# zhouyifan233/light-transport

Measured on AMD Instinct MI355X. Metric: photon_steps_per_sec, higher is better.
Workload: dtype f64

## Files before the change

include/lt.h:

```cpp
#ifndef LT_H_
#define LT_H_

#include <stddef.h>
#include <stdint.h>

#ifdef __cplusplus
extern "C" {
#endif

#define LT_ABI_VERSION 3

#define LT_OK 0
#define LT_E_INVALID (-1)
#define LT_E_STATE (-2)
#define LT_E_HIP (-3)
#define LT_E_NOMEM (-4)
#define LT_E_UNSUPPORTED (-5)

#define LT_TALLY_F32 0
#define LT_TALLY_F64 1
#define LT_TALLY_U64FX 2
#define LT_FX_SCALE 1099511627776.0

#define LT_QUANTITY_ABSORBED 0
#define LT_QUANTITY_FLUENCE 1

#define LT_SRC_PENCIL 0
#define LT_SRC_COSINE_QUAD 1

#define LT_FLAG_F32_WALK 1u

typedef struct lt_medium {
    double mu_a;
    double mu_s;
    double g;
    double n;
} lt_medium;

typedef struct lt_bvh_node {
    double lo[3];
    double hi[3];
    int32_t offset;
    int32_t n_prims;
    int32_t axis;
    int32_t pad_;
} lt_bvh_node;

typedef struct lt_counters {
    uint64_t photons;
    uint64_t steps;
    double w_absorbed;
    double w_lost_outside_grid;
    double w_escaped_top;
    double w_escaped_bottom;
    double w_escaped_mesh;
    double w_specular;
    double w_roulette_net;
    double w_capped;
} lt_counters;

typedef struct lt_ctx lt_ctx;

int lt_abi_version(void);
int lt_create(lt_ctx** out, int device_id);
int lt_destroy(lt_ctx* ctx);
const char* lt_last_error(const lt_ctx* ctx);

int lt_set_media(lt_ctx* ctx, const lt_medium* media, int n);
int lt_set_layers(lt_ctx* ctx, const double* z_bounds, const int32_t* medium_idx,
                  int n, double n_above, double n_below);
int lt_set_mesh(lt_ctx* ctx, const double* verts, const int32_t* med_front,
                const int32_t* med_back, int n_tris, const lt_bvh_node* nodes,
                int n_nodes);
int lt_build_bvh(const double* verts, int n_tris, int split_method, int32_t* order_out, lt_bvh_node* nodes_out,
                 int max_nodes, int* n_nodes_out);
int lt_set_grid(lt_ctx* ctx, int nx, int ny, int nz, const double origin[3],
                const double voxel[3], int tally_dtype);
int lt_set_source(lt_ctx* ctx, int type, const double pos[3], const double dir[3],
                  const double* extra, int start_medium);
int lt_set_max_steps(lt_ctx* ctx, uint32_t max_steps);
int lt_set_tuning(lt_ctx* ctx, const char* key, int64_t value);
int lt_set_tally_quantity(lt_ctx* ctx, int quantity);
int lt_set_launch_config(lt_ctx* ctx, int blocks_per_cu, int threads_per_block);

#define LT_MODE_ATOMIC 0
#define LT_MODE_LOG 1
#define LT_MODE_AUTO 2
int lt_set_tally_mode(lt_ctx* ctx, int mode, uint64_t log_bytes);
int lt_reserve_log(lt_ctx* ctx, uint64_t n_photons);
int lt_set_overlap(lt_ctx* ctx, int lanes);

int lt_launch(lt_ctx* ctx, uint64_t n_photons, uint64_t photon_offset, uint64_t seed,
              const double* rng_table, uint64_t table_steps, uint32_t flags);
int lt_sync(lt_ctx* ctx);
int lt_last_kernel_ms(lt_ctx* ctx, double* ms);
int lt_zero_tally(lt_ctx* ctx);
int lt_last_log_stages(lt_ctx* ctx, double ms_out[4], uint64_t* records, uint64_t* batches);
int lt_last_log_info(lt_ctx* ctx, uint64_t* records, uint64_t* overflow_records, uint64_t* batches, int* lanes);
int lt_last_log_hot_tiles(lt_ctx* ctx, uint32_t* hot_tiles, uint32_t* threshold);

int lt_read_grid(lt_ctx* ctx, void* host_out, size_t bytes);
int lt_read_grid_f64(lt_ctx* ctx, double* host_out, size_t n_voxels);
int lt_read_counters(lt_ctx* ctx, lt_counters* out);
int lt_grid_device_ptr(lt_ctx* ctx, void** ptr, size_t* bytes);
int lt_counters_device_ptr(lt_ctx* ctx, void** ptr, size_t* bytes);
void* lt_stream(lt_ctx* ctx);
int lt_reduce_grid(lt_ctx* ctx, void* nccl_comm, int root);


int lt_intersect_rays(lt_ctx* ctx, const double* origins, const double* dirs,
                      const double* tmax, size_t n, int use_bvh, int32_t* prim_out,
                      double* t_out);
int lt_triangle_intersect(lt_ctx* ctx, const double* origins, const double* dirs,
                          const double* tris, size_t n, double* t_out);
int lt_intersect_bounds(lt_ctx* ctx, const double* origins, const double* dirs,
                        const double* tmax, const double* boxes, size_t n,
                        int32_t* hit_out);
#define LT_FN_HG_PDF 0
#define LT_FN_HG_SAMPLE 1
#define LT_FN_ONB 2
#define LT_FN_DISK 3
#define LT_FN_COSINE_HEMI 4
#define LT_FN_REFLECT 5
#define LT_FN_BOUNDARY 6
#define LT_FN_SPIN 7
#define LT_FN_WALK_MATH 8
#define LT_FN_WALK_MATH_RAW 9
int lt_eval(lt_ctx* ctx, int fn, const double* in, size_t n, double* out);
int lt_rng_raw(lt_ctx* ctx, uint64_t seed, uint64_t photon_id, uint32_t count,
               uint32_t* out);

typedef struct lt_surface_material {
    double diffuse[3];
    double emission;
    double ior;
    double transmission;
    int32_t is_diffuse, is_mirror, is_light, pad_;
} lt_surface_material;

typedef struct lt_point_light {
    double source[3];
    double normal[3];
    double radiance[3];
    double total_area;
} lt_point_light;

int lt_set_surface_materials(lt_ctx* ctx, const lt_surface_material* mats, int n_tris);
int lt_set_lights(lt_ctx* ctx, const lt_point_light* lights, int n);
int lt_render_surface(lt_ctx* ctx, int width, int height, int samples, int max_depth,
                      const double camera[3], double f_distance, const double* xs,
                      const double* ys, double* rand_0, const double* rand_1,
                      const int32_t* light_choice, double* image);
int lt_render_surface_old(lt_ctx* ctx, int width, int height, int samples, int max_depth,
                          const double camera[3], double f_distance, const double* xs,
                          const double* ys, double* rand_0, const double* rand_1,
                          const int32_t* light_choice, int choices_per_sample, double* image);

#define LT_VERTEX_LIGHT 5
#define LT_VERTEX_REFLECTIVE 3
#define LT_VERTEX_TRANSMISSIVE 4
#define LT_VERTEX_VOLUME 7
typedef struct lt_vertex {
    double point[3];
    double direction[3];
    double g_norm[3];
    double throughput;
    double pdf_pos;
    double pdf_dir;
    int32_t kind;
    int32_t medium;
    uint32_t step;
    uint32_t pad_;
} lt_vertex;
int lt_set_vertex_capture(lt_ctx* ctx, uint32_t max_vertices_per_photon);
int lt_read_vertices(lt_ctx* ctx, lt_vertex* vertices_out, uint32_t* counts_out, uint64_t n_photons);

int lt_mesh_accel_info(lt_ctx* ctx, int* kind, int march_dims[3], uint64_t* march_entries, int clearance_dims[3]);

int lt_device_info(lt_ctx* ctx, char* name, size_t name_len, int* n_cus,
                   int* clock_mhz, size_t* hbm_bytes);

#ifdef __cplusplus
}
#endif
#endif
```

light_transport_amd/_lib.py:

```python
import ctypes as C
import os
import subprocess

import numpy as np

_HERE = os.path.dirname(os.path.abspath(__file__))
LIB_PATH = os.environ.get("LT_HIP_LIBRARY") or os.path.join(_HERE, "liblt_hip.so")

TALLY = {"f32": 0, "f64": 1, "u64fx": 2}
TALLY_NP = {0: np.float32, 1: np.float64, 2: np.uint64}
FX_SCALE = 2.0 ** 40
SRC_PENCIL, SRC_COSINE_QUAD = 0, 1
FLAG_F32_WALK = 1
FN = dict(HG_PDF=0, HG_SAMPLE=1, ONB=2, DISK=3, COSINE_HEMI=4, REFLECT=5, BOUNDARY=6, SPIN=7, WALK_MATH=8, WALK_MATH_RAW=9)
_FN_SHAPE = {0: (2, 1), 1: (2, 1), 2: (3, 6), 3: (2, 2), 4: (8, 4), 5: (6, 3), 6: (8, 5), 7: (5, 3), 8: (1, 5), 9: (1, 3)}

SYMBOLS = [
    "lt_abi_version", "lt_create", "lt_destroy", "lt_last_error", "lt_set_media", "lt_set_layers", "lt_set_mesh",
    "lt_set_grid", "lt_set_source", "lt_set_max_steps", "lt_set_launch_config", "lt_launch", "lt_sync",
    "lt_last_kernel_ms", "lt_zero_tally", "lt_read_grid", "lt_read_grid_f64", "lt_read_counters",
    "lt_grid_device_ptr", "lt_counters_device_ptr", "lt_stream", "lt_reduce_grid", "lt_intersect_rays",
    "lt_triangle_intersect", "lt_intersect_bounds", "lt_eval", "lt_rng_raw", "lt_device_info",
    "lt_set_surface_materials", "lt_set_lights", "lt_render_surface", "lt_set_vertex_capture", "lt_read_vertices",
    "lt_set_tally_mode", "lt_last_log_stages", "lt_reserve_log", "lt_render_surface_old", "lt_set_overlap", "lt_last_log_hot_tiles",
    "lt_last_log_info", "lt_set_tally_quantity", "lt_set_tuning", "lt_mesh_accel_info", "lt_build_bvh",
]

VERTEX_DTYPE = np.dtype([("point", "<f8", 3), ("direction", "<f8", 3), ("g_norm", "<f8", 3), ("throughput", "<f8"),
                         ("pdf_pos", "<f8"), ("pdf_dir", "<f8"), ("kind", "<i4"), ("medium", "<i4"), ("step", "<u4"),
                         ("pad_", "<u4")])
VERTEX_LIGHT, VERTEX_REFLECTIVE, VERTEX_TRANSMISSIVE, VERTEX_VOLUME = 5, 3, 4, 7


class LtError(RuntimeError):
    pass


NODE_DTYPE = np.dtype([("lo", "<f8", 3), ("hi", "<f8", 3), ("offset", "<i4"), ("n_prims", "<i4"), ("axis", "<i4"), ("pad_", "<i4")])


def build_bvh_arrays(verts, split_method=1):
    v = _f64(verts).reshape(-1, 3, 3)
    T = v.shape[0]
    order = np.empty(T, dtype=np.int32)
    nodes = np.zeros(max(2 * T, 1), dtype=NODE_DTYPE)
    nn = C.c_int(0)
    rc = lib().lt_build_bvh(_dp(v), C.c_int(T), C.c_int(int(split_method)), _ip(order), nodes.ctypes.data_as(C.c_void_p),
                            C.c_int(len(nodes)), C.byref(nn))
    if rc:
        raise LtError("lt_build_bvh failed (%d): needs >= 1 triangle with finite vertices and split_method 0 or 1" % rc)
    return order, nodes[:nn.value]


class Medium(C.Structure):
    _fields_ = [("mu_a", C.c_double), ("mu_s", C.c_double), ("g", C.c_double), ("n", C.c_double)]


class BvhNode(C.Structure):
    _fields_ = [("lo", C.c_double * 3), ("hi", C.c_double * 3), ("offset", C.c_int32),
                ("n_prims", C.c_int32), ("axis", C.c_int32), ("pad_", C.c_int32)]


class Counters(C.Structure):
    _fields_ = [("photons", C.c_uint64), ("steps", C.c_uint64)] + [
        (k, C.c_double) for k in ("w_absorbed", "w_lost_outside_grid", "w_escaped_top", "w_escaped_bottom",
                                  "w_escaped_mesh", "w_specular", "w_roulette_net", "w_capped")]

    def as_dict(self):
        return {k: getattr(self, k) for k, _ in self._fields_}


class SurfaceMaterial(C.Structure):
    _fields_ = [("diffuse", C.c_double * 3), ("emission", C.c_double), ("ior", C.c_double),
                ("transmission", C.c_double), ("is_diffuse", C.c_int32), ("is_mirror", C.c_int32),
                ("is_light", C.c_int32), ("pad_", C.c_int32)]


class PointLight(C.Structure):
    _fields_ = [("source", C.c_double * 3), ("normal", C.c_double * 3), ("radiance", C.c_double * 3),
                ("total_area", C.c_double)]


def pack_surface_materials(primitives):
    arr = (SurfaceMaterial * max(len(primitives), 1))()
    for i, p in enumerate(primitives):
        m = p.material
        arr[i].diffuse[:] = [float(x) for x in m.color.diffuse[:3]]
        arr[i].emission, arr[i].ior, arr[i].transmission = float(m.emission), float(m.ior), float(m.transmission)
        arr[i].is_diffuse, arr[i].is_mirror, arr[i].is_light = int(m.is_diffuse), int(m.is_mirror), int(p.is_light)
    return arr


def pack_lights(lights):
    arr = (PointLight * max(len(lights), 1))()
    for i, l in enumerate(lights):
        arr[i].source[:] = [float(x) for x in l.source[:3]]
        arr[i].normal[:] = [float(x) for x in l.normal[:3]]
        arr[i].radiance[:] = [float(l.material.emission * x) for x in l.material.color.diffuse[:3]]
        arr[i].total_area = float(l.total_area)
    return arr


_lib = None


def build(verbose=False):
    cmd = ["make", "-C", os.path.join(_HERE, "csrc")]
    if not verbose:
        cmd.append("-s")
    subprocess.check_call(cmd)
    return LIB_PATH


def lib():
    global _lib
    if _lib is None:
        if not os.path.exists(LIB_PATH):
            raise LtError("liblt_hip.so is not built (run light_transport_amd.build() or "
                          "`make -C light_transport_amd/csrc`); there is no CPU fallback")
        L = C.CDLL(LIB_PATH)
        L.lt_last_error.restype = C.c_char_p
        L.lt_last_error.argtypes = [C.c_void_p]
        L.lt_stream.restype = C.c_void_p
        L.lt_stream.argtypes = [C.c_void_p]
        _lib = L
    return _lib


def _dp(a):
    return a.ctypes.data_as(C.POINTER(C.c_double)) if a is not None else None


def _ip(a):
    return a.ctypes.data_as(C.POINTER(C.c_int32)) if a is not None else None


def _f64(a, shape=None):
    a = np.ascontiguousarray(a, dtype=np.float64)
    return a.reshape(shape) if shape is not None else a


class Context:

    def __init__(self, device_id=0):
        self._h = C.c_void_p()
        rc = lib().lt_create(C.byref(self._h), C.c_int(device_id))
        if rc != 0:
            msg = lib().lt_last_error(None)
            raise LtError("lt_create failed (%d): %s" % (rc, msg.decode() if msg else "?"))
        self.device_id = device_id
        self._grid_shape = None
        self._tally = None

    def _ck(self, rc, what):
        if rc != 0:
            msg = lib().lt_last_error(self._h)
            raise LtError("%s failed (%d): %s" % (what, rc, msg.decode() if msg else "?"))

    def close(self):
        if getattr(self, "_h", None) is not None and self._h.value:
            lib().lt_destroy(self._h)
            self._h = C.c_void_p()

    def __del__(self):
        try:
            self.close()
        except Exception:
            pass

    def __enter__(self):
        return self

    def __exit__(self, *a):
        self.close()

    def set_media(self, media):
        arr = (Medium * len(media))(*[Medium(*map(float, m)) for m in media])
        self._ck(lib().lt_set_media(self._h, arr, C.c_int(len(media))), "lt_set_media")

    def set_layers(self, z_bounds, medium_idx, n_above=1.0, n_below=1.0):
        zb = _f64(z_bounds)
        mi = np.ascontiguousarray(medium_idx, dtype=np.int32)
        if zb.size != mi.size + 1:
            raise LtError("set_layers: need len(z_bounds) == len(medium_idx) + 1")
        self._ck(lib().lt_set_layers(self._h, _dp(zb), _ip(mi), C.c_int(mi.size), C.c_double(n_above),
                                     C.c_double(n_below)), "lt_set_layers")

    def set_mesh(self, verts, med_front, med_back, nodes):
        v = _f64(verts).reshape(-1, 3, 3)
        mf = np.ascontiguousarray(med_front, dtype=np.int32)
        mb = np.ascontiguousarray(med_back, dtype=np.int32)
        if isinstance(nodes, np.ndarray) and nodes.dtype == NODE_DTYPE:
            arr = np.ascontiguousarray(nodes)
        else:
            n_ = len(nodes["offset"])
            arr = np.zeros(n_, dtype=NODE_DTYPE)
            arr["lo"] = np.asarray(nodes["lo"], dtype=np.float64).reshape(n_, 3); arr["hi"] = np.asarray(nodes["hi"], dtype=np.float64).reshape(n_, 3)
            arr["offset"] = nodes["offset"]; arr["n_prims"] = nodes["n_prims"]; arr["axis"] = nodes["axis"]
        n = len(arr)
        if mf.size != v.shape[0] or mb.size != v.shape[0]:
            raise LtError("set_mesh: medium arrays must have one entry per triangle")
        self._ck(lib().lt_set_mesh(self._h, _dp(v), _ip(mf), _ip(mb), C.c_int(v.shape[0]), arr.ctypes.data_as(C.c_void_p), C.c_int(n)),
                 "lt_set_mesh")

# ... 231 lines not shown
```

light_transport_amd/csrc/lt_api.cpp:

```cpp
#include <hip/hip_runtime_api.h>

#include <dlfcn.h>

#include <algorithm>
#include <cmath>
#include <cctype>
#include <cstdarg>
#include <cstdio>
#include <cstdlib>
#include <cstring>
#include <limits>
#include <mutex>
#include <new>
#include <string>
#include <vector>

#include "lt_internal.hpp"

using namespace ltk;

static const size_t kMeshLdsBudget = 64 * 1024;

namespace {

thread_local std::string g_create_error;

struct DevBuf {
    void* p = nullptr;
    size_t bytes = 0;
    void release() { if (p) { (void)hipFree(p); p = nullptr; bytes = 0; } }
    hipError_t ensure(size_t n)
    {
        if (n <= bytes && p) return hipSuccess;
        release();
        hipError_t e = hipMalloc(&p, n ? n : 16);
        if (e == hipSuccess) bytes = n ? n : 16;
        return e;
    }
};

}

constexpr int kMaxLanes = 3;
constexpr int kAutoLanes = 2;

struct LogLane {
    hipStream_t stream = nullptr;
    hipStream_t tail_stream = nullptr;
    hipEvent_t ev_bulk = nullptr, ev_tail = nullptr;
    hipEvent_t ev_done = nullptr;
    std::vector<hipEvent_t> evs;
    size_t ev_used = 0;
    DevBuf log_idx, log_val, tmp_idx, tmp_val, log_fill, meta, hist1, hist_unused, hist, bin_base, bin_cnt, tile_base, tile_cnt, cursor1,
        cursor2, items2, items_c, items_r, itab, head, pool, pool_n;
    size_t alloc_records = 0;
    int alloc_elem = 0;
    void release_log() { log_idx.release(); log_val.release(); tmp_idx.release(); tmp_val.release(); log_fill.release(); alloc_records = 0; }
    void release_all()
    {
        release_log(); meta.release(); hist1.release(); hist_unused.release(); hist.release(); bin_base.release(); bin_cnt.release(); tile_base.release();
        tile_cnt.release(); cursor1.release(); itab.release();
        cursor2.release(); items2.release(); items_c.release(); items_r.release(); head.release(); pool.release(); pool_n.release();
    }
};

struct lt_ctx {
    int device = 0;
    hipStream_t stream = nullptr;
    hipEvent_t ev0 = nullptr, ev1 = nullptr, ev_fork = nullptr;
    bool stages_valid = false;
    uint64_t last_records = 0, last_overflow = 0, last_batches = 0;
    int last_lanes = 1;
    bool log_stats_pending = false;
    uint64_t pending_photons = 0;
    std::string err;
    hipDeviceProp_t prop;

    std::vector<lt_medium> media;
    std::vector<double> z_bounds;
    std::vector<int32_t> layer_medium;
    double n_above = 1.0, n_below = 1.0;
    std::vector<double> verts;
    std::vector<int32_t> med_front, med_back;
    std::vector<lt_bvh_node> nodes;
    std::vector<lt_surface_material> surf_mats;
    std::vector<lt_point_light> lights;
    bool have_layers = false, have_mesh = false, have_grid = false, have_source = false;
    int nx = 0, ny = 0, nz = 0, tally = LT_TALLY_F32;
    double origin[3] = {0, 0, 0}, voxel[3] = {1, 1, 1};
    int src_type = LT_SRC_PENCIL, start_medium = 0;
    double src_pos[3] = {0, 0, 0}, src_dir[3] = {0, 0, 1}, src_extra[6] = {0, 0, 0, 0, 0, 0};
    uint32_t max_steps = 1000000;
    int quantity = LT_QUANTITY_ABSORBED;
    uint32_t max_vertices = 0, captured_max_vertices = 0;
    int tally_mode = 2;
    size_t log_budget = (size_t)16 << 30, default_log_budget = (size_t)16 << 30;
    double rec_per_photon = 0.0;
    int overlap_mode = 0;
    double auto_ms_per_photon[kMaxLanes] = {0.0, 0.0, 0.0};
    uint64_t auto_photons[kMaxLanes] = {0, 0, 0};
    int auto_pending = -1;
    uint64_t captured_photons = 0;
    int blocks_per_cu = 0, threads_per_block = 0;

    DevBuf d_media[2], d_zb[2], d_if[2], d_lm, d_tris[2], d_nodes[2];
    DevBuf d_grid, d_counters, d_head, d_table, d_scratch_in, d_scratch_out, d_scratch_aux;
    DevBuf d_mats, d_lights, d_r0, d_r1, d_lc, d_img, d_xy, d_vtx, d_vcnt, d_clear, d_job, d_gridx[kMaxLanes - 1];
    int cn[3] = {0, 0, 0};
    double corg[3] = {0, 0, 0}, ccell[3] = {1, 1, 1};
    bool have_clear = false;
    DevBuf d_mcell, d_mlist, d_mcoarse, d_links;
    MarchGrid mgrid;
    bool have_march = false, have_links = false;
    size_t march_entries = 0;
    LogLane lanes[kMaxLanes];
    DevBuf d_dmap, d_dmeta;
    bool dmap_valid = false, tile_cnt_ready = false, last_hot = false;
    uint32_t dmap_tiles = 0, dmap_bits2 = 0;
    bool tables_dirty = true, media_dirty = false;
    struct Knobs {
        long query_min = -1, log_bits2 = -1, log_hot = -1, overlap_walk_bpc = -1, diag_no_tally = -1, log_timing = -1,
             march_cells = -1, march_scale_milli = -1, no_march = -1, no_clearance = -1, no_near_lists = -1,
             clearance_cells = -1, march_info = -1, force_march = -1, tail_split = -1, part_alone = -1, serial_walks = -1, part_lds = -1,
             render_lds_tables = -1;
        std::string overlap_pattern;
    } knob;
    long* knob_by_name(const char* key)
    {
        static const struct { const char* k; long Knobs::*m; } tab[] = {
            {"query_min", &Knobs::query_min}, {"log_bits2", &Knobs::log_bits2}, {"log_hot", &Knobs::log_hot},
            {"overlap_walk_bpc", &Knobs::overlap_walk_bpc}, {"diag_no_tally", &Knobs::diag_no_tally}, {"log_timing", &Knobs::log_timing},
            {"march_cells", &Knobs::march_cells}, {"march_scale_milli", &Knobs::march_scale_milli}, {"no_march", &Knobs::no_march},
            {"no_clearance", &Knobs::no_clearance}, {"no_near_lists", &Knobs::no_near_lists}, {"clearance_cells", &Knobs::clearance_cells},
            {"march_info", &Knobs::march_info}, {"force_march", &Knobs::force_march}, {"tail_split", &Knobs::tail_split}, {"part_alone", &Knobs::part_alone}, {"serial_walks", &Knobs::serial_walks}, {"part_lds", &Knobs::part_lds},
            {"render_lds_tables", &Knobs::render_lds_tables}};
        for (const auto& t : tab) if (std::strcmp(key, t.k) == 0) return &(knob.*(t.m));
        return nullptr;
    }
    bool on(long v) const { return v > 0; }
    bool timed = false;

    int fail(int code, const char* fmt, ...)
    {
        char buf[512];
        va_list ap;
        va_start(ap, fmt);
        vsnprintf(buf, sizeof buf, fmt, ap);
        va_end(ap);
        err = buf;
        return code;
    }
    int hip(hipError_t e, const char* what)
    {
        if (e == hipSuccess) return LT_OK;
        return fail(LT_E_HIP, "%s: %s", what, hipGetErrorString(e));
    }
    size_t grid_elem() const { return tally == LT_TALLY_F32 ? 4 : 8; }
    size_t n_vox() const { return (size_t)nx * (size_t)ny * (size_t)nz; }
    void scene_changed() { rec_per_photon = 0.0; for (double& a : auto_ms_per_photon) a = 0.0; for (uint64_t& a : auto_photons) a = 0; auto_pending = -1; dmap_valid = tile_cnt_ready = false; }
};

static bool bvh_octant_links(const std::vector<lt_bvh_node>& nd, std::vector<int16_t>& out)
{
    const int n = (int)nd.size();
    if (n <= 0 || n > 32767) return false;
    out.assign((size_t)16 * n, (int16_t)n);
    for (int oct = 0; oct < 8; oct++) {
        int16_t* first = &out[(size_t)oct * 2 * n]; int16_t* after = first + n;
        std::vector<std::pair<int, int>> todo{{0, n}};
        while (!todo.empty()) {
            const auto [i, a] = todo.back(); todo.pop_back();
            after[i] = (int16_t)a;
            if (nd[(size_t)i].n_prims > 0) continue;
            const int c0 = i + 1, c1 = nd[(size_t)i].offset;
            const bool neg = (oct >> nd[(size_t)i].axis) & 1;
            const int near_ = neg ? c1 : c0, far_ = neg ? c0 : c1;
            first[i] = (int16_t)near_;
            todo.emplace_back(near_, far_); todo.emplace_back(far_, a);
        }
    }
    return true;
}

#define CHECK_CTX(c) do { if (!(c)) return LT_E_INVALID; } while (0)
#define HIP_TRY(c, call) do { hipError_t e_ = (call); if (e_ != hipSuccess) return (c)->hip(e_, #call); } while (0)
#define BIND(c) HIP_TRY(c, hipSetDevice((c)->device))

namespace {

template <typename R>
void fill_media(const std::vector<lt_medium>& in, int quantity, std::vector<MedD<R>>& out)
{
    out.resize(in.size());
    for (size_t i = 0; i < in.size(); i++) {
        const double mu_t = in[i].mu_a + in[i].mu_s;
        MedD<R>& m = out[i];
        m.mu_t = (R)mu_t;
        m.inv_mu_t = (R)(mu_t > 0 ? 1.0 / mu_t : 0.0);
        m.absorb = (R)(mu_t > 0 ? in[i].mu_a / mu_t : 0.0);
        m.g = (R)in[i].g;
        m.n = (R)in[i].n;
        const R g = m.g;
        m.one_m_g2 = (R)1 - g * g;
        m.one_p_g2 = (R)1 + g * g;
        m.inv_2g = g != 0 ? (R)1 / ((R)2 * g) : (R)0;
        m.dep = quantity == LT_QUANTITY_FLUENCE ? m.inv_mu_t : m.absorb;
        m.one_m_g = (R)1 - g; m.two_g = (R)2 * g;
        m.pad_ = 0;
    }
}

template <typename R>
void fill_tris(const std::vector<double>& v, const std::vector<int32_t>& mf, const std::vector<int32_t>& mb,
               std::vector<TriD<R>>& out)
{
    const size_t n = v.size() / 9;
    out.resize(n);
    for (size_t i = 0; i < n; i++) {
        const double* a = &v[9 * i];
        const double* b = a + 3;
        const double* c = a + 6;
        double e1[3], e2[3], nn[3];
        for (int k = 0; k < 3; k++) { e1[k] = b[k] - a[k]; e2[k] = c[k] - a[k]; }
        nn[0] = e1[1] * e2[2] - e1[2] * e2[1];
        nn[1] = e1[2] * e2[0] - e1[0] * e2[2];
        nn[2] = e1[0] * e2[1] - e1[1] * e2[0];
        const double l = std::sqrt(nn[0] * nn[0] + nn[1] * nn[1] + nn[2] * nn[2]);
        for (int k = 0; k < 3; k++) {
            out[i].a[k] = (R)a[k]; out[i].ab[k] = (R)e1[k]; out[i].ac[k] = (R)e2[k]; out[i].n[k] = (R)(nn[k] / l);
        }
        out[i].med_front = mf[i];
        out[i].med_back = mb[i];
    }
}

template <typename R>
void fill_nodes(const std::vector<lt_bvh_node>& in, std::vector<NodeD<R>>& out)
{
    out.resize(in.size());
    for (size_t i = 0; i < in.size(); i++) {
        for (int k = 0; k < 3; k++) {
            R lo = (R)in[i].lo[k], hi = (R)in[i].hi[k];
            if ((double)lo > in[i].lo[k]) lo = std::nextafter(lo, -std::numeric_limits<R>::infinity());
            if ((double)hi < in[i].hi[k]) hi = std::nextafter(hi, std::numeric_limits<R>::infinity());
            out[i].lo[k] = lo; out[i].hi[k] = hi;
        }
        out[i].offset = in[i].offset;
        out[i].n_prims = in[i].n_prims;
        out[i].axis = in[i].axis;
        out[i].skip = (int32_t)in.size();
    }
    for (size_t i = 0; i < in.size(); i++) {
        if (in[i].n_prims > 0) continue;
        out[i + 1].skip = in[i].offset;
        out[(size_t)in[i].offset].skip = out[i].skip;
    }
}

template <typename R>
void fill_ifaces(const lt_ctx* c, std::vector<IfD<R>>& out)
{
    const int n = (int)c->layer_medium.size();
    out.resize((size_t)n + 1);
    for (int k = 0; k <= n; k++) {
        auto index_of = [&](int layer) {
            const int32_t m = c->layer_medium[(size_t)layer];
            return m >= 0 && (size_t)m < c->media.size() ? c->media[(size_t)m].n : 1.0;
        };
        const R up = (R)(k == 0 ? c->n_above : index_of(k - 1));
        const R dn = (R)(k == n ? c->n_below : index_of(k));
        out[(size_t)k].n_up = up; out[(size_t)k].n_dn = dn;
        out[(size_t)k].nr_down = up / dn; out[(size_t)k].nr_up = dn / up;
    }
}

template <typename T>
int upload(lt_ctx* c, DevBuf& b, const std::vector<T>& h)
{
    HIP_TRY(c, b.ensure(h.size() * sizeof(T)));
    if (!h.empty()) HIP_TRY(c, hipMemcpyAsync(b.p, h.data(), h.size() * sizeof(T), hipMemcpyHostToDevice, c->stream));
    return LT_OK;
}

bool tri_box_overlap(const double bc[3], const double bh[3], const double* tri)
{
    double v[3][3];
    for (int i = 0; i < 3; i++) for (int k = 0; k < 3; k++) v[i][k] = tri[3 * i + k] - bc[k];
    for (int k = 0; k < 3; k++) {
        const double lo = std::min(v[0][k], std::min(v[1][k], v[2][k])), hi = std::max(v[0][k], std::max(v[1][k], v[2][k]));
        if (lo > bh[k] || hi < -bh[k]) return false;
    }
    const double e[3][3] = {{v[1][0] - v[0][0], v[1][1] - v[0][1], v[1][2] - v[0][2]},
                            {v[2][0] - v[1][0], v[2][1] - v[1][1], v[2][2] - v[1][2]},
                            {v[0][0] - v[2][0], v[0][1] - v[2][1], v[0][2] - v[2][2]}};
    for (int j = 0; j < 3; j++)
        for (int i = 0; i < 3; i++) {
            const int a = (i + 1) % 3, b = (i + 2) % 3;
            const double ax = -e[j][b], bx = e[j][a];
            const double p0 = ax * v[0][a] + bx * v[0][b], p1 = ax * v[1][a] + bx * v[1][b], p2 = ax * v[2][a] + bx * v[2][b];
            const double r = bh[a] * std::fabs(ax) + bh[b] * std::fabs(bx);
            if (std::min(p0, std::min(p1, p2)) > r || std::max(p0, std::max(p1, p2)) < -r) return false;
        }
    const double n[3] = {e[0][1] * e[1][2] - e[0][2] * e[1][1], e[0][2] * e[1][0] - e[0][0] * e[1][2], e[0][0] * e[1][1] - e[0][1] * e[1][0]};
    const double dn = n[0] * v[0][0] + n[1] * v[0][1] + n[2] * v[0][2];
    const double r = bh[0] * std::fabs(n[0]) + bh[1] * std::fabs(n[1]) + bh[2] * std::fabs(n[2]);
    return !(dn > r || dn < -r);
}

int build_march_grid(lt_ctx* c)
{
    c->have_march = false;
    const size_t nt = c->verts.size() / 9;
    double ext[3], longest = 0;
    for (int k = 0; k < 3; k++) { ext[k] = c->nodes[0].hi[k] - c->nodes[0].lo[k]; if (ext[k] > longest) longest = ext[k]; }
    if (!(longest > 0) || !std::isfinite(longest) || nt == 0) return LT_OK;
    std::vector<double> size(nt);
    for (size_t i = 0; i < nt; i++) {
        const double* a = &c->verts[9 * i];
        const double e1[3] = {a[3] - a[0], a[4] - a[1], a[5] - a[2]}, e2[3] = {a[6] - a[0], a[7] - a[1], a[8] - a[2]};
        const double nn[3] = {e1[1] * e2[2] - e1[2] * e2[1], e1[2] * e2[0] - e1[0] * e2[2], e1[0] * e2[1] - e1[1] * e2[0]};
        size[i] = std::sqrt(std::sqrt(nn[0] * nn[0] + nn[1] * nn[1] + nn[2] * nn[2]));
    }
    std::nth_element(size.begin(), size.begin() + nt / 2, size.end());
    double h = size[nt / 2];
    if (c->knob.march_scale_milli > 10 && c->knob.march_scale_milli < 100000) h *= 1e-3 * (double)c->knob.march_scale_milli;
    int per_axis = h > 0 ? (int)std::lround(longest / h) : 256;
    per_axis = per_axis < 32 ? 32 : (per_axis > 256 ? 256 : per_axis);
    if (c->knob.march_cells >= 4 && c->knob.march_cells <= 512) per_axis = (int)c->knob.march_cells;
    h = longest / (double)per_axis;
    MarchGrid& G = c->mgrid;
    int n[3];
    for (int k = 0; k < 3; k++) {
        n[k] = (int)std::ceil(ext[k] / h); if (n[k] < 1) n[k] = 1;
        G.h[k] = ext[k] > 0 ? ext[k] / n[k] : h;
        n[k] += 2;
        G.org[k] = c->nodes[0].lo[k] - G.h[k]; G.inv[k] = 1.0 / G.h[k];
    }
    G.nx = n[0]; G.ny = n[1]; G.nz = n[2];
    for (int k = 0; k < 3; k++) {
        G.fn[k] = (double)n[k]; G.fn32[k] = (float)n[k];
        G.org32[k] = (float)G.org[k]; G.inv32[k] = (float)G.inv[k]; G.h32[k] = (float)G.h[k];
    }
    const size_t cells = (size_t)n[0] * n[1] * n[2];
    const double hmin = std::min(G.h[0], std::min(G.h[1], G.h[2]));
    const double margin = std::max(1e-4 * hmin, 3e-5 * longest);
    G.nudge64 = 1e-9 * hmin; G.nudge32 = 4e-6 * longest;
    std::vector<uint32_t> count(cells, 0u);
    std::vector<std::pair<uint32_t, uint32_t>> pairs;
    pairs.reserve(nt * 8);
    for (size_t i = 0; i < nt; i++) {
        const double* a = &c->verts[9 * i];
        int lo[3], hi[3];
        for (int k = 0; k < 3; k++) {
            const double mn = std::min(a[k], std::min(a[3 + k], a[6 + k])) - margin, mx = std::max(a[k], std::max(a[3 + k], a[6 + k])) + margin;
            lo[k] = (int)std::floor((mn - G.org[k]) * G.inv[k]); hi[k] = (int)std::floor((mx - G.org[k]) * G.inv[k]);
            lo[k] = lo[k] < 0 ? 0 : lo[k]; hi[k] = hi[k] >= n[k] ? n[k] - 1 : hi[k];
        }
        const double bh[3] = {0.5 * G.h[0] + margin, 0.5 * G.h[1] + margin, 0.5 * G.h[2] + margin};
        for (int z = lo[2]; z <= hi[2]; z++)
            for (int y = lo[1]; y <= hi[1]; y++)
                for (int x = lo[0]; x <= hi[0]; x++) {
                    const double bc[3] = {G.org[0] + (x + 0.5) * G.h[0], G.org[1] + (y + 0.5) * G.h[1], G.org[2] + (z + 0.5) * G.h[2]};
                    if (!tri_box_overlap(bc, bh, a)) continue;
                    const uint32_t ci = (uint32_t)(((size_t)z * n[1] + y) * n[0] + x);
                    count[ci]++;
                    pairs.emplace_back(ci, (uint32_t)i);
                }
    }
    std::vector<uint2> rec(cells);
    size_t total = 0;
    for (size_t i = 0; i < cells; i++) {
        rec[i].x = count[i] < kMarchCountMask ? count[i] : kMarchCountMask;
        rec[i].y = (uint32_t)total;
        total += count[i];
    }
    if (total >= (1u << 26)) return LT_OK;
    std::vector<uint32_t> list(total ? total : 1, 0u), fill(cells, 0u);
    for (const auto& pr : pairs) list[rec[pr.first].y + fill[pr.first]++] = pr.second;
    c->march_entries = pairs.size();
    HIP_TRY(c, c->d_mcell.ensure(cells * sizeof(uint2)));
    HIP_TRY(c, c->d_mlist.ensure(list.size() * 4));
    const size_t nc = (size_t)((n[0] + 7) / 8) * ((n[1] + 7) / 8) * ((n[2] + 7) / 8);
    HIP_TRY(c, c->d_mcoarse.ensure(nc * sizeof(double)));
    HIP_TRY(c, hipMemcpyAsync(c->d_mcell.p, rec.data(), cells * sizeof(uint2), hipMemcpyHostToDevice, c->stream));
    HIP_TRY(c, hipMemcpyAsync(c->d_mlist.p, list.data(), list.size() * 4, hipMemcpyHostToDevice, c->stream));
    G.cell = (const uint2*)c->d_mcell.p; G.list = (const uint32_t*)c->d_mlist.p;
    HIP_TRY(c, launch_march_clearance(c->d_tris[0].p, c->d_nodes[0].p, (int)c->nodes.size(), G, (uint2*)c->d_mcell.p,
                                      (double*)c->d_mcoarse.p, c->stream));
    HIP_TRY(c, hipStreamSynchronize(c->stream));
    c->have_march = true;
    if (c->on(c->knob.march_info))
        std::fprintf(stderr, "[lt march] %zu triangles, grid %d x %d x %d (cell %.4g), %zu list entries (%.2f per triangle), %zu cells listed\n",
                     nt, n[0], n[1], n[2], h, pairs.size(), (double)pairs.size() / (double)nt,
                     (size_t)std::count_if(count.begin(), count.end(), [](uint32_t v) { return v != 0; }));
    return LT_OK;
}

int upload_tables(lt_ctx* c)
{
    if (!c->tables_dirty && !c->media_dirty) return LT_OK;
    int rc;
    std::vector<MedD<double>> m64; std::vector<MedD<float>> m32;
    std::vector<double> z64; std::vector<float> z32;
    std::vector<IfD<double>> i64; std::vector<IfD<float>> i32;
    std::vector<TriD<double>> t64; std::vector<TriD<float>> t32;
    std::vector<NodeD<double>> n64; std::vector<NodeD<float>> n32;
    std::vector<int16_t> links16;
    fill_media(c->media, c->quantity, m64); fill_media(c->media, c->quantity, m32);
    if ((rc = upload(c, c->d_media[0], m64))) return rc;
    if ((rc = upload(c, c->d_media[1], m32))) return rc;
    if (c->have_layers) {
        fill_ifaces(c, i64); fill_ifaces(c, i32);
        if ((rc = upload(c, c->d_if[0], i64))) return rc;
        if ((rc = upload(c, c->d_if[1], i32))) return rc;
    }
    if (!c->tables_dirty) {
        HIP_TRY(c, hipStreamSynchronize(c->stream));
        c->media_dirty = false;
        return LT_OK;
    }
    if (c->have_layers) {
        z64 = c->z_bounds;
        z32.assign(z64.begin(), z64.end());
        if ((rc = upload(c, c->d_zb[0], z64))) return rc;
        if ((rc = upload(c, c->d_zb[1], z32))) return rc;
        if ((rc = upload(c, c->d_lm, c->layer_medium))) return rc;
    }
    if (c->have_mesh) {
        fill_tris(c->verts, c->med_front, c->med_back, t64);
        fill_tris(c->verts, c->med_front, c->med_back, t32);
        fill_nodes(c->nodes, n64); fill_nodes(c->nodes, n32);
        if ((rc = upload(c, c->d_tris[0], t64))) return rc;
        if ((rc = upload(c, c->d_tris[1], t32))) return rc;
        if ((rc = upload(c, c->d_nodes[0], n64))) return rc;
        if ((rc = upload(c, c->d_nodes[1], n32))) return rc;
        c->have_links = bvh_octant_links(c->nodes, links16);
        if (c->have_links && (rc = upload(c, c->d_links, links16))) return rc;
        Variant vq; std::memset(&vq, 0, sizeof vq); vq.mesh = 1;
        const int nm = (int)c->media.size(), ntr = (int)t64.size(), nno = (int)n64.size();
        const bool lds64 = walk_lds_bytes(vq, nm, 0, ntr, nno) <= kMeshLdsBudget;
        vq.f32 = 1;
        const bool lds32 = walk_lds_bytes(vq, nm, 0, ntr, nno) <= kMeshLdsBudget;
        c->have_march = false;
        if ((!lds64 || c->on(c->knob.force_march)) && !c->on(c->knob.no_clearance) && !c->on(c->knob.no_march)) { if ((rc = build_march_grid(c))) return rc; }
        c->have_clear = false;
        if (!c->on(c->knob.no_clearance) && lds32) {
            if (t64.size() > 0xffff) return c->fail(LT_E_UNSUPPORTED, "lt_set_mesh: %zu triangles within the LDS budget cannot be (near-triangle ids are 16 bits)", t64.size());
            double ext[3], longest = 0;
            for (int k = 0; k < 3; k++) { ext[k] = c->nodes[0].hi[k] - c->nodes[0].lo[k]; if (ext[k] > longest) longest = ext[k]; }
            if (longest > 0 && std::isfinite(longest)) {
                int per_axis = (int)std::cbrt(2.0e9 / (double)(t64.empty() ? 1 : t64.size()));
                per_axis = per_axis < 32 ? 32 : (per_axis > 128 ? 128 : per_axis);
                if (c->knob.clearance_cells >= 8 && c->knob.clearance_cells <= 512) per_axis = (int)c->knob.clearance_cells;
                const double h = longest / (double)per_axis;
                for (int k = 0; k < 3; k++) {
                    c->cn[k] = (int)std::ceil(ext[k] / h); if (c->cn[k] < 1) c->cn[k] = 1;
                    c->ccell[k] = ext[k] > 0 ? ext[k] / c->cn[k] : h; c->corg[k] = c->nodes[0].lo[k];
                }
                const size_t cells = (size_t)c->cn[0] * c->cn[1] * c->cn[2];
                HIP_TRY(c, c->d_clear.ensure(cells * 16));
                HIP_TRY(c, launch_build_clearance(c->d_tris[0].p, (int)t64.size(), c->on(c->knob.no_near_lists) ? 0 : 1, c->d_clear.p,
                                                  c->cn[0], c->cn[1], c->cn[2], c->corg, c->ccell, c->stream));
                c->have_clear = true;
            }
        }
    }
    HIP_TRY(c, hipStreamSynchronize(c->stream));
    c->tables_dirty = false; c->media_dirty = false;
    return LT_OK;
}

int collect_log_stats(lt_ctx* c)
{
    if (!c->log_stats_pending) return LT_OK;
    unsigned long long h[2] = {0, 0};
    HIP_TRY(c, hipMemcpyAsync(h, c->d_job.p, sizeof h, hipMemcpyDeviceToHost, c->stream));
    HIP_TRY(c, hipStreamSynchronize(c->stream));
    c->log_stats_pending = false;
    c->last_records = h[0]; c->last_overflow = h[1];
    if (c->pending_photons > 0) c->rec_per_photon = (double)(h[0] + h[1]) / (double)c->pending_photons;
    if (c->auto_pending >= 0) {
        float f = 0;
        if (hipEventElapsedTime(&f, c->ev0, c->ev1) == hipSuccess && c->pending_photons > 0)
        {
            c->auto_ms_per_photon[c->auto_pending] = (double)f / (double)c->pending_photons;
            c->auto_photons[c->auto_pending] = c->pending_photons;
        }
        c->auto_pending = -1;
    }
    return LT_OK;
}

constexpr uint32_t kMaxLogTiles = 65536;
constexpr uint64_t kPilotPhotons = 16384;
constexpr uint64_t kOverlapMinPhotons = 1ull << 21;
constexpr uint64_t kTailSplitMinPerWave = 512;

struct LogGeom { uint32_t ntx, nty, ntz, n_tiles, bits2, nb1; };

LogGeom log_geom(const lt_ctx* c)
{
    LogGeom g;
    g.ntx = ((uint32_t)c->nx + 31u) >> kTileBX; g.nty = ((uint32_t)c->ny + 31u) >> kTileBY; g.ntz = ((uint32_t)c->nz + 15u) >> kTileBZ;
    g.n_tiles = g.ntx * g.nty * g.ntz;
    uint32_t b = 0;
    if (g.n_tiles > 1024) { b = 1; while ((1u << (2 * b)) < g.n_tiles && b < 7) b++; }
    if (c->knob.log_bits2 >= 0) b = c->knob.log_bits2 > 7 ? 7u : (uint32_t)c->knob.log_bits2;
    while ((g.n_tiles >> b) > 1024 && b < 7) b++;
    g.bits2 = b;
    g.nb1 = b ? (g.n_tiles + (1u << b) - 1) >> b : g.n_tiles;
    return g;
}

size_t log_slack_records() { return (size_t)kTileAlign * kMaxLogTiles + (size_t)kBinAlign * 1024 + 2 * (size_t)log_part_item(); }

struct LogPlan {
    int lanes = 1;
    uint32_t cap_chunks[kMaxLanes] = {0, 0, 0};
    std::vector<std::pair<int, uint64_t>> batches;
};

hipError_t ensure_lane(lt_ctx* c, LogLane& ln, size_t want, size_t limit, const LogGeom& G)
{
    hipError_t e;
    const size_t elem = c->grid_elem();
    if (ln.alloc_elem != (int)elem) { ln.release_log(); ln.alloc_elem = (int)elem; }
    if (want > ln.alloc_records) {
        size_t grown = want + want / 8;
        if (grown > limit) grown = limit;
        grown = (grown / kLogChunk) * kLogChunk;
        ln.release_log();
        const size_t n = grown + log_slack_records();
        if ((e = ln.log_idx.ensure(n * 4)) != hipSuccess) return e;
        if ((e = ln.tmp_idx.ensure(n * 4)) != hipSuccess) return e;
        if ((e = ln.log_val.ensure(n * elem)) != hipSuccess) return e;
        if ((e = ln.tmp_val.ensure(n * elem)) != hipSuccess) return e;
        if ((e = ln.log_fill.ensure((grown / kLogChunk) * 4)) != hipSuccess) return e;
        if ((e = ln.itab.ensure((grown / log_part_item() + 1024 + 16) * 16)) != hipSuccess) return e;
        ln.alloc_records = grown;
    }
    const size_t nt = G.n_tiles, nd = G.bits2 ? (size_t)log_max_digits() : G.n_tiles;
    if ((e = ln.meta.ensure(LM_WORDS * 4)) != hipSuccess) return e;
    if ((e = ln.head.ensure(sizeof(unsigned long long))) != hipSuccess) return e;
    if ((e = ln.hist.ensure(nt * kLogGroups * 4)) != hipSuccess) return e;
    if ((e = ln.hist1.ensure(nd * kLogGroups * 4)) != hipSuccess) return e;
    if (G.bits2 && (e = ln.hist_unused.ensure(nd * kLogGroups * 4)) != hipSuccess) return e;
    if ((e = ln.bin_base.ensure((nd + 1) * 4)) != hipSuccess) return e;
    if ((e = ln.bin_cnt.ensure((nd + 1) * 4)) != hipSuccess) return e;
    if ((e = ln.tile_base.ensure((nt + 1) * 4)) != hipSuccess) return e;
    if ((e = ln.tile_cnt.ensure((nt + 1) * 4)) != hipSuccess) return e;
    if ((e = ln.cursor1.ensure(nd * kLogGroups * 4)) != hipSuccess) return e;
    if ((e = ln.cursor2.ensure(nt * kLogGroups2 * 4)) != hipSuccess) return e;
    if ((e = ln.items2.ensure((nd + 1) * 4)) != hipSuccess) return e;
    if ((e = ln.items_c.ensure((nd + 1) * 4)) != hipSuccess) return e;
    return ln.items_r.ensure((nt + 1) * 4);
}

int plan_log(lt_ctx* c, uint64_t n, int lanes, LogPlan* plan)
{
    const LogGeom G = log_geom(c);
    const size_t rec_bytes = 4 + c->grid_elem();
    size_t per_lane = c->log_budget / (2 * rec_bytes) / (size_t)lanes;
    if (per_lane > 0xFF000000ull) per_lane = 0xFF000000ull;
    per_lane = (per_lane / kLogChunk) * kLogChunk;
    if (per_lane < 16 * (size_t)kLogChunk) {
        if (lanes > 1) return LT_E_NOMEM;
        return c->fail(LT_E_INVALID, "lt_launch: log budget too small (%zu bytes)", c->log_budget);
    }
    for (int l = 1; l < lanes; l++)
        if (c->d_gridx[l - 1].ensure(c->n_vox() * c->grid_elem()) != hipSuccess) { (void)hipGetLastError(); return LT_E_NOMEM; }
    const double rate = c->rec_per_photon > 0.0 ? c->rec_per_photon : 400.0;
    const uint64_t tail = lanes == 1 ? 0 : n / (uint64_t)(2 * lanes + 1);
    const uint64_t b_target = lanes == 1 ? n : (n - tail + (uint64_t)lanes - 1) / (uint64_t)lanes;
    double waves = 20.0 * (double)c->prop.multiProcessorCount / (double)lanes;
    const double launched = 4.0 * (double)((b_target + 255) / 256);
    if (launched < waves) waves = launched;
    const double wave_slack = (double)kLogChunk * waves;
    const double groups_used = launched / 4.0 < (double)kLogGroups ? (launched / 4.0 < 1.0 ? 1.0 : launched / 4.0) : (double)kLogGroups;
    const double need = (1.25 * rate * (double)b_target + 1048576.0) * ((double)kLogGroups / groups_used) + wave_slack;
    size_t want = need < (double)per_lane ? (size_t)need : per_lane;
    want = ((want + kLogChunk - 1) / kLogChunk) * kLogChunk;
    size_t cap_use = per_lane;
    for (int l = 0; l < lanes; l++) {
        if (ensure_lane(c, c->lanes[l], want, per_lane, G) != hipSuccess) {
            (void)hipGetLastError();
            for (int k = 0; k < kMaxLanes; k++) c->lanes[k].release_log();
            return LT_E_NOMEM;
        }
        const size_t use = c->lanes[l].alloc_records < per_lane ? c->lanes[l].alloc_records : per_lane;
        plan->cap_chunks[l] = (uint32_t)(use / kLogChunk);
        if (use < cap_use) cap_use = use;
    }
    double fit = 0.8 * ((double)cap_use - wave_slack) / rate;
    if (fit < 4096.0) fit = 4096.0;
    plan->lanes = lanes;
    plan->batches.clear();
    uint64_t left = n;
    if (lanes == 1) {
        while (left > 0) { const uint64_t b = (double)left > fit ? (uint64_t)fit : left; plan->batches.emplace_back(0, b); left -= b; }
    } else {
        int l = 0;
        if (const char* e = c->knob.overlap_pattern.empty() ? nullptr : c->knob.overlap_pattern.c_str()) {
            std::vector<double> wts; double sum = 0.0;
            for (const char* q = e; *q;) { char* end = nullptr; const double v_ = std::strtod(q, &end); if (end == q) break; if (v_ > 0) { wts.push_back(v_); sum += v_; } q = *end ? end + 1 : end; }
            for (size_t k = 0; k < wts.size() && left > 0 && sum > 0; k++) {
                uint64_t take = k + 1 == wts.size() ? left : (uint64_t)((double)n * wts[k] / sum);
                if (take < 1) take = 1;
                if (take > left) take = left;
                if ((double)take > fit) take = (uint64_t)fit;
                plan->batches.emplace_back(l, take);
                left -= take; l = (l + 1) % lanes;
            }
        }
        const uint64_t body = left > tail ? left - tail : left;
        const uint64_t cap_b = (double)b_target > fit ? (uint64_t)fit : b_target;
        uint64_t rounds = (body + cap_b * (uint64_t)lanes - 1) / (cap_b * (uint64_t)lanes);
        if (rounds < 1) rounds = 1;
        const uint64_t full = (body + rounds * (uint64_t)lanes - 1) / (rounds * (uint64_t)lanes);
        for (uint64_t k = 0, done_b = 0; k < rounds * (uint64_t)lanes && done_b < body; k++) {
            const uint64_t take = full < body - done_b ? full : body - done_b;
            plan->batches.emplace_back(l, take);
            done_b += take; left -= take; l = (l + 1) % lanes;
        }
        while (left > 0) {
            const uint64_t take = (double)left > fit ? (uint64_t)fit : left;
            plan->batches.emplace_back(l, take);
            left -= take; l = (l + 1) % lanes;
        }
    }
    return LT_OK;
}

int choose_lanes(lt_ctx* c, uint64_t n)
{
    c->auto_pending = -1;
    if (c->overlap_mode == 1) return 1;
    if (c->overlap_mode >= 2) return n >= 8192 ? c->overlap_mode : 1;
    if (c->blocks_per_cu > 0 || n < kOverlapMinPhotons) return 1;
    for (int k = kAutoLanes - 1; k >= 0; k--) {
        const bool stale = c->auto_photons[k] != 0 && (n > 2 * c->auto_photons[k] || c->auto_photons[k] > 2 * n);
        if (c->auto_ms_per_photon[k] <= 0.0 || stale) { c->auto_pending = k; return k + 1; }
    }
    int best = 0;
    for (int k = 1; k < kAutoLanes; k++) if (c->auto_ms_per_photon[k] < c->auto_ms_per_photon[best]) best = k;
    return best + 1;
}

struct LogRun {
    lt_ctx* c; WalkParams P; Variant v; LaunchCfg cfg; LogGeom G;
};

struct WalkGate {
    std::mutex mu;
    hipEvent_t ring[64] = {};
    unsigned next = 0;
    hipEvent_t last = nullptr;
};
WalkGate& walk_gate(int device)
{
    static WalkGate gates[16];
    return gates[device & 15];
}

hipError_t lane_event(LogLane& ln, hipStream_t s)
{
    if (ln.ev_used == ln.evs.size()) {
        hipEvent_t ev;
        hipError_t e = hipEventCreate(&ev);
        if (e != hipSuccess) return e;
        ln.evs.push_back(ev);
    }
    return hipEventRecord(ln.evs[ln.ev_used++], s);
}

int run_log_plan(LogRun& R, const LogPlan& plan, uint64_t offset, int* n_batches)
{
    lt_ctx* c = R.c;
    const LogGeom& G = R.G;
    const bool hot = G.bits2 != 0 && c->dmap_valid;
    const uint32_t n_hist = G.bits2 ? G.nb1 : G.n_tiles;
    LaunchCfg cfg = R.cfg;
    cfg.lds_bytes = walk_lds_bytes(R.v, R.P.n_media, R.P.n_layers, R.P.n_tris, R.P.n_nodes, n_hist);
    const int resident = walk_max_blocks_per_cu(R.v, cfg.threads, cfg.lds_bytes);
    if (resident <= 0) return c->fail(LT_E_HIP, "lt_launch: log-mode kernel not resident");
    int per_cu = c->blocks_per_cu > 0 ? c->blocks_per_cu : (plan.lanes >= 2 ? (resident + 1) / 2 : resident);
    if (plan.lanes >= 2 && c->knob.overlap_walk_bpc >= 1 && c->knob.overlap_walk_bpc <= 8) per_cu = (int)c->knob.overlap_walk_bpc;
    const unsigned long long cap = (unsigned long long)per_cu * (unsigned long long)c->prop.multiProcessorCount;
    if (plan.lanes >= 2) {
        const size_t gb = c->n_vox() * c->grid_elem();
        HIP_TRY(c, hipEventRecord(c->ev_fork, c->stream));
        for (int l = 1; l < plan.lanes; l++) {
            if (!c->lanes[l].stream) HIP_TRY(c, hipStreamCreateWithFlags(&c->lanes[l].stream, hipStreamNonBlocking));
            HIP_TRY(c, hipStreamWaitEvent(c->lanes[l].stream, c->ev_fork, 0));
            HIP_TRY(c, hipMemsetAsync(c->d_gridx[l - 1].p, 0, gb, c->lanes[l].stream));
        }
    }
    for (const auto& bt : plan.batches) {
        LogLane& ln = c->lanes[bt.first];
        hipStream_t s = ln.stream;
        uint32_t* meta = (uint32_t*)ln.meta.p;
        WalkParams P = R.P;
        P.n_photons = bt.second; P.photon_offset = offset;
        if (bt.first >= 1) P.grid = c->d_gridx[bt.first - 1].p;
        P.head = (unsigned long long*)ln.head.p;
        P.log_idx = (uint32_t*)ln.log_idx.p; P.log_val = ln.log_val.p; P.log_fill = (uint32_t*)ln.log_fill.p;
        P.log_next = meta + LM_NEXT; P.log_overflow = meta + LM_OVERFLOW; P.log_cap_chunks = plan.cap_chunks[bt.first];
        P.log_hist = (uint32_t*)(hot ? ln.hist_unused.p : (G.bits2 ? ln.hist1.p : ln.hist.p)); P.log_n_hist = n_hist; P.log_hist_shift = kTileShift + G.bits2;
        P.log_ntx = G.ntx; P.log_nty = G.nty;
        const unsigned long long want = (bt.second + (unsigned long long)cfg.threads - 1) / (unsigned long long)cfg.threads;
        cfg.blocks = (int)(want < cap ? want : cap);
        if (cfg.blocks < 1) cfg.blocks = 1;

        LogReduceParams L;
        std::memset(&L, 0, sizeof L);
        L.log_idx = P.log_idx; L.log_val = P.log_val; L.log_fill = P.log_fill;
        L.tmp_idx = (uint32_t*)ln.tmp_idx.p; L.tmp_val = ln.tmp_val.p;
        L.hist1 = (uint32_t*)ln.hist1.p; L.hist = (uint32_t*)ln.hist.p;
        L.bin_base = (uint32_t*)ln.bin_base.p; L.bin_cnt = (uint32_t*)ln.bin_cnt.p;
        L.tile_base = (uint32_t*)ln.tile_base.p; L.tile_cnt = (uint32_t*)ln.tile_cnt.p;
        L.cursor1 = (uint32_t*)ln.cursor1.p; L.cursor2 = (uint32_t*)ln.cursor2.p;
        L.items2 = (uint32_t*)ln.items2.p; L.items_c = (uint32_t*)ln.items_c.p; L.items_r = (uint32_t*)ln.items_r.p;
        L.itab = (uint32_t*)ln.itab.p;
        L.meta = meta; L.job = (unsigned long long*)c->d_job.p; L.cap_chunks = P.log_cap_chunks;
        L.n_tiles = G.n_tiles; L.bits2 = G.bits2;
        L.grid = bt.first >= 1 ? c->d_gridx[bt.first - 1].p : c->d_grid.p; L.n_vox = c->n_vox(); L.tally = c->tally;
        L.nx = (uint32_t)c->nx; L.ny = (uint32_t)c->ny; L.nz = (uint32_t)c->nz; L.ntx = G.ntx; L.nty = G.nty;
        L.flush_atomic = 0;
        if (hot) { L.dmap = (const uint16_t*)c->d_dmap.p; L.dmeta = (const uint32_t*)c->d_dmeta.p; }

        HIP_TRY(c, hipMemsetAsync(ln.head.p, 0, sizeof(unsigned long long), s));
        HIP_TRY(c, hipMemsetAsync(meta, 0, LM_WORDS * 4, s));
        HIP_TRY(c, hipMemsetAsync(ln.hist.p, 0, (size_t)G.n_tiles * (G.bits2 ? kLogGroups2 : kLogGroups) * 4, s));
        HIP_TRY(c, hipMemsetAsync(ln.log_fill.p, 0, (size_t)P.log_cap_chunks * 4, s));
        if (G.bits2) HIP_TRY(c, hipMemsetAsync(ln.hist1.p, 0, (size_t)(hot ? log_max_digits() : G.nb1) * kLogGroups * 4, s));
        const bool last_batch = &bt == &plan.batches.back();
        const uint64_t waves_launched = (uint64_t)cfg.blocks * (uint64_t)(cfg.threads / 64);
        const bool big_enough = c->knob.tail_split >= 2 || bt.second >= kTailSplitMinPerWave * waves_launched;
        const bool split = R.v.mesh <= 1 && !R.v.table && !R.v.capture && c->knob.tail_split != 0 && big_enough &&
                           ((plan.lanes == 1 && (c->blocks_per_cu == 0 || c->knob.serial_walks > 0) && (!R.v.f32 || c->knob.tail_split >= 2)) ||
                            (plan.lanes > 1 && last_batch));
        L.alone = (plan.lanes == 1 && c->blocks_per_cu == 0 && !split) ? 1 : 0;
        if (c->knob.part_alone == 0 || c->knob.part_alone == 1) L.alone = (int)c->knob.part_alone;
        L.lds_part = c->knob.part_lds > 0 ? (int)(c->knob.part_lds & 7) : 0;
        Variant vw = R.v;
        if (split) {
            const size_t cap = (size_t)cfg.blocks * (size_t)(cfg.threads / 64) * kDumpPoolLanes;
            P.dump_max = c->knob.tail_split > 1 ? (uint32_t)std::min<long>(c->knob.tail_split, (long)kDumpPoolLanes) : kDumpMaxLanes;
            HIP_TRY(c, ln.pool.ensure(cap * (R.v.f32 ? sizeof(SurvD<float>) : sizeof(SurvD<double>))));
            HIP_TRY(c, ln.pool_n.ensure(4));
            if (!ln.tail_stream) HIP_TRY(c, hipStreamCreateWithFlags(&ln.tail_stream, hipStreamNonBlocking));
            if (!ln.ev_bulk) HIP_TRY(c, hipEventCreateWithFlags(&ln.ev_bulk, hipEventDisableTiming));
            if (!ln.ev_tail) HIP_TRY(c, hipEventCreateWithFlags(&ln.ev_tail, hipEventDisableTiming));
            HIP_TRY(c, hipMemsetAsync(ln.pool_n.p, 0, 4, s));
            P.pool = ln.pool.p; P.pool_n = (uint32_t*)ln.pool_n.p; P.pool_cap = (uint32_t)cap;
            vw.phase = 1;
        }
        const bool train = c->knob.serial_walks > 0;
        if (train) {
            WalkGate& g = walk_gate(c->device);
            std::lock_guard<std::mutex> lk(g.mu);
            if (g.last) HIP_TRY(c, hipStreamWaitEvent(s, g.last, 0));
        }
        HIP_TRY(c, lane_event(ln, s));
        HIP_TRY(c, launch_walk(P, vw, cfg, s));
        HIP_TRY(c, lane_event(ln, s));
        if (split) {
            HIP_TRY(c, hipEventRecord(ln.ev_bulk, s));
            HIP_TRY(c, hipStreamWaitEvent(ln.tail_stream, ln.ev_bulk, 0));
            WalkParams Pt = P;
            Pt.log_idx = nullptr; Pt.log_val = nullptr; Pt.log_n_hist = 0;
            Variant vt = R.v; vt.phase = 2;
            LaunchCfg ct = cfg;
            ct.lds_bytes = walk_lds_bytes(vt, P.n_media, P.n_layers, P.n_tris, P.n_nodes, 0);
            ct.blocks = (int)((P.pool_cap / 64u + (unsigned)(cfg.threads / 64) - 1) / (unsigned)(cfg.threads / 64));
            if (ct.blocks < 1) ct.blocks = 1;
            HIP_TRY(c, launch_walk(Pt, vt, ct, ln.tail_stream));
            HIP_TRY(c, hipEventRecord(ln.ev_tail, ln.tail_stream));
        }
        if (hot) HIP_TRY(c, launch_log_count1(L, s));
        HIP_TRY(c, G.bits2 ? launch_log_scan_bins(L, s) : launch_log_scan_tiles(L, s));
        if (train) {
            WalkGate& g = walk_gate(c->device);
            std::lock_guard<std::mutex> lk(g.mu);
            hipEvent_t& ev = g.ring[g.next++ & 63u];
            if (!ev) HIP_TRY(c, hipEventCreateWithFlags(&ev, hipEventDisableTiming));
            HIP_TRY(c, hipEventRecord(ev, s));
            g.last = ev;
        }
        HIP_TRY(c, lane_event(ln, s));
        HIP_TRY(c, launch_log_part1(L, s));
        LogReduceParams Lr = L;
        if (G.bits2 == 0) { Lr.log_idx = L.tmp_idx; Lr.log_val = L.tmp_val; }
        else HIP_TRY(c, launch_log_part2(L, s));
        HIP_TRY(c, lane_event(ln, s));
        if (split) Lr.flush_atomic = 1;
        HIP_TRY(c, launch_log_reduce(Lr, s));
        HIP_TRY(c, lane_event(ln, s));
        if (split) HIP_TRY(c, hipStreamWaitEvent(s, ln.ev_tail, 0));
        if (bt.first == 0 && G.bits2) c->tile_cnt_ready = true;
        offset += bt.second;
        (*n_batches)++;
    }
    for (int l = 1; l < plan.lanes; l++) {
        HIP_TRY(c, hipEventRecord(c->lanes[l].ev_done, c->lanes[l].stream));
        HIP_TRY(c, hipStreamWaitEvent(c->stream, c->lanes[l].ev_done, 0));
        HIP_TRY(c, launch_grid_add(c->d_grid.p, c->d_gridx[l - 1].p, c->tally, c->n_vox(), c->stream));
    }
    return LT_OK;
}

bool bvh_is_valid(const std::vector<lt_bvh_node>& n, int n_tris, int* max_depth)
{
    std::vector<std::pair<int, int>> todo{{0, 0}};
    std::vector<char> seen(n.size(), 0);
    size_t visited = 0;
    *max_depth = 0;
    while (!todo.empty()) {
        const auto [idx, depth] = todo.back(); todo.pop_back();
        if (idx < 0 || idx >= (int)n.size() || seen[idx]) return false;
        seen[idx] = 1; visited++;
        if (depth > *max_depth) *max_depth = depth;
        const lt_bvh_node& nd = n[idx];
        if (nd.n_prims > 0) { if (nd.offset < 0 || nd.offset + nd.n_prims > n_tris) return false; continue; }
        if (nd.axis < 0 || nd.axis > 2 || nd.offset <= idx + 1) return false;
        todo.emplace_back(nd.offset, depth + 1); todo.emplace_back(idx + 1, depth + 1);
    }
    return visited == n.size();
}

}

extern "C" {

int lt_abi_version(void) { return LT_ABI_VERSION; }

const char* lt_last_error(const lt_ctx* ctx) { return ctx ? ctx->err.c_str() : g_create_error.c_str(); }

int lt_create(lt_ctx** out, int device_id)
{
    if (!out) return LT_E_INVALID;
    *out = nullptr;
    int n_dev = 0;
    hipError_t e = hipGetDeviceCount(&n_dev);
    if (e != hipSuccess || n_dev <= 0) {
        g_create_error = std::string("no HIP device available (") + (e != hipSuccess ? hipGetErrorString(e) : "0 devices") +
                         "); this library has no CPU fallback";
        return LT_E_HIP;
    }
    if (device_id < 0 || device_id >= n_dev) { g_create_error = "device_id out of range"; return LT_E_INVALID; }
    lt_ctx* c = new (std::nothrow) lt_ctx();
    if (!c) { g_create_error = "out of host memory"; return LT_E_NOMEM; }
    c->device = device_id;
    {
        static const char* const names[] = {"query_min", "log_bits2", "log_hot", "overlap_walk_bpc", "diag_no_tally", "log_timing", "march_cells",
                                            "march_scale_milli", "no_march", "no_clearance", "no_near_lists", "clearance_cells", "march_info", "force_march", "tail_split", "part_alone", "serial_walks", "part_lds",
                                            "render_lds_tables"};
        for (const char* k : names) {
            std::string name = "LT_";
            for (const char* q = k; *q; q++) name += (char)std::toupper((unsigned char)*q);
            if (const char* v = std::getenv(name.c_str())) *c->knob_by_name(k) = std::atol(v);
        }
        if (const char* v = std::getenv("LT_OVERLAP_PATTERN")) c->knob.overlap_pattern = v;
    }
    e = hipSetDevice(device_id);
    if (e == hipSuccess) e = hipGetDeviceProperties(&c->prop, device_id);
    if (e == hipSuccess && std::strncmp(c->prop.gcnArchName, "gfx950", 6) != 0) {
        g_create_error = std::string("device arch ") + c->prop.gcnArchName + " is not gfx950: kernels are built for MI355X only";
        delete c;
        return LT_E_UNSUPPORTED;
    }
    if (e == hipSuccess) {
        size_t quarter = c->prop.totalGlobalMem / 4;
        c->log_budget = c->default_log_budget = quarter < ((size_t)64 << 30) ? quarter : ((size_t)64 << 30);
    }
    if (e == hipSuccess) e = hipStreamCreateWithFlags(&c->stream, hipStreamNonBlocking);
    c->lanes[0].stream = c->stream;
    if (e == hipSuccess) e = hipEventCreate(&c->ev0);
    if (e == hipSuccess) e = hipEventCreate(&c->ev1);
    if (e == hipSuccess) e = hipEventCreateWithFlags(&c->ev_fork, hipEventDisableTiming);
    for (int k = 0; k < kMaxLanes && e == hipSuccess; k++) e = hipEventCreateWithFlags(&c->lanes[k].ev_done, hipEventDisableTiming);
    if (e == hipSuccess) e = c->d_job.ensure(2 * sizeof(unsigned long long));
    if (e == hipSuccess) e = c->d_counters.ensure(sizeof(DevCounters));
    if (e == hipSuccess) e = c->d_head.ensure(sizeof(unsigned long long));
    if (e == hipSuccess) e = hipMemsetAsync(c->d_counters.p, 0, sizeof(DevCounters), c->stream);
    if (e != hipSuccess) {
        g_create_error = std::string("lt_create: ") + hipGetErrorString(e);
        delete c;
        return LT_E_HIP;
    }
    *out = c;
    return LT_OK;
}

int lt_destroy(lt_ctx* c)
{
    if (!c) return LT_OK;
    (void)hipSetDevice(c->device);
    if (c->stream) (void)hipStreamSynchronize(c->stream);
    for (int i = 0; i < 2; i++) { c->d_media[i].release(); c->d_zb[i].release(); c->d_if[i].release(); c->d_tris[i].release(); c->d_nodes[i].release(); }
    c->d_lm.release(); c->d_grid.release(); c->d_counters.release(); c->d_head.release(); c->d_table.release();
    c->d_scratch_in.release(); c->d_scratch_out.release(); c->d_scratch_aux.release();
    c->d_mats.release(); c->d_lights.release(); c->d_r0.release(); c->d_r1.release(); c->d_lc.release();
    c->d_img.release(); c->d_xy.release(); c->d_vtx.release(); c->d_vcnt.release(); c->d_clear.release();
    c->d_job.release(); c->d_dmap.release(); c->d_dmeta.release();
    c->d_mcell.release(); c->d_mlist.release(); c->d_mcoarse.release(); c->d_links.release();
    for (int k = 1; k < kMaxLanes; k++) { c->d_gridx[k - 1].release(); if (c->lanes[k].stream) (void)hipStreamSynchronize(c->lanes[k].stream); }
    for (int k = 0; k < kMaxLanes; k++) {
        c->lanes[k].release_all();
        for (hipEvent_t ev : c->lanes[k].evs) (void)hipEventDestroy(ev);
        if (c->lanes[k].ev_done) (void)hipEventDestroy(c->lanes[k].ev_done);
    }
    if (c->ev0) (void)hipEventDestroy(c->ev0);
    if (c->ev1) (void)hipEventDestroy(c->ev1);
    if (c->ev_fork) (void)hipEventDestroy(c->ev_fork);
    for (int k = 0; k < kMaxLanes; k++) {
        if (c->lanes[k].tail_stream) { (void)hipStreamSynchronize(c->lanes[k].tail_stream); (void)hipStreamDestroy(c->lanes[k].tail_stream); }
        if (c->lanes[k].ev_bulk) (void)hipEventDestroy(c->lanes[k].ev_bulk);
        if (c->lanes[k].ev_tail) (void)hipEventDestroy(c->lanes[k].ev_tail);
    }
    for (int k = 1; k < kMaxLanes; k++) if (c->lanes[k].stream) (void)hipStreamDestroy(c->lanes[k].stream);
    if (c->stream) (void)hipStreamDestroy(c->stream);
    delete c;
    return LT_OK;
}

int lt_set_media(lt_ctx* c, const lt_medium* media, int n)
{
    CHECK_CTX(c);
    if (!media || n <= 0 || n > kMaxMedia) return c->fail(LT_E_INVALID, "lt_set_media: need 1..%d media", kMaxMedia);
    for (int i = 0; i < n; i++) {
        const lt_medium& m = media[i];
        if (!(m.mu_a >= 0) || !(m.mu_s >= 0) || !(m.g > -1 && m.g < 1) || !(m.n > 0) || !std::isfinite(m.mu_a + m.mu_s))
            return c->fail(LT_E_INVALID, "lt_set_media: medium %d out of range (mu_a,mu_s >= 0, |g| < 1, n > 0)", i);
    }
    c->media.assign(media, media + n);
    c->scene_changed();
    c->tables_dirty = true;
    return LT_OK;
}

int lt_set_layers(lt_ctx* c, const double* z_bounds, const int32_t* medium_idx, int n, double n_above, double n_below)
{
    CHECK_CTX(c);
    if (!z_bounds || !medium_idx || n <= 0 || n > kMaxLayers)
        return c->fail(LT_E_INVALID, "lt_set_layers: need 1..%d layers", kMaxLayers);
    if (!std::isfinite(z_bounds[0])) return c->fail(LT_E_INVALID, "lt_set_layers: z_bounds[0] must be finite");
    for (int i = 0; i < n; i++) {
        if (!(z_bounds[i + 1] > z_bounds[i])) return c->fail(LT_E_INVALID, "lt_set_layers: z_bounds must ascend");
        if (medium_idx[i] < 0) return c->fail(LT_E_INVALID, "lt_set_layers: negative medium index");
    }
    if (!(n_above > 0) || !(n_below > 0)) return c->fail(LT_E_INVALID, "lt_set_layers: ambient indices must be > 0");
    c->z_bounds.assign(z_bounds, z_bounds + n + 1);
    c->layer_medium.assign(medium_idx, medium_idx + n);
    c->n_above = n_above; c->n_below = n_below;
    c->have_layers = true; c->have_mesh = false;
    c->scene_changed();
    c->tables_dirty = true;
    return LT_OK;
}

int lt_set_mesh(lt_ctx* c, const double* verts, const int32_t* med_front, const int32_t* med_back, int n_tris,
                const lt_bvh_node* nodes, int n_nodes)
{
    CHECK_CTX(c);
    if (!verts || !med_front || !med_back || n_tris <= 0 || !nodes || n_nodes <= 0)
        return c->fail(LT_E_INVALID, "lt_set_mesh: empty mesh or BVH");
    for (size_t i = 0; i < (size_t)n_tris * 9; i++)
        if (!std::isfinite(verts[i])) return c->fail(LT_E_INVALID, "lt_set_mesh: non-finite vertex");
    std::vector<lt_bvh_node> nn(nodes, nodes + n_nodes);
    int depth = 0;
    if (!bvh_is_valid(nn, n_tris, &depth))
        return c->fail(LT_E_INVALID, "lt_set_mesh: BVH is not a valid pre-order tree over %d triangles", n_tris);
    size_t covered = 0;
    for (const auto& nd : nn) if (nd.n_prims > 0) covered += (size_t)nd.n_prims;
    if (covered != (size_t)n_tris) return c->fail(LT_E_INVALID, "lt_set_mesh: leaves cover %zu of %d triangles", covered, n_tris);
    c->verts.assign(verts, verts + (size_t)n_tris * 9);
    c->med_front.assign(med_front, med_front + n_tris);
    c->med_back.assign(med_back, med_back + n_tris);
    c->nodes.swap(nn);
    c->have_mesh = true; c->have_layers = false;
    c->surf_mats.clear();
    c->scene_changed();
    c->tables_dirty = true;
    return LT_OK;
}

int lt_set_grid(lt_ctx* c, int nx, int ny, int nz, const double origin[3], const double voxel[3], int tally_dtype)
{
    CHECK_CTX(c);
    if (nx <= 0 || ny <= 0 || nz <= 0 || !origin || !voxel) return c->fail(LT_E_INVALID, "lt_set_grid: bad shape");
    if (tally_dtype < LT_TALLY_F32 || tally_dtype > LT_TALLY_U64FX) return c->fail(LT_E_INVALID, "lt_set_grid: bad tally dtype");
    for (int k = 0; k < 3; k++)
        if (!(voxel[k] > 0) || !std::isfinite(origin[k])) return c->fail(LT_E_INVALID, "lt_set_grid: bad origin/voxel");
    if ((double)nx * ny * nz > 2147483647.0) return c->fail(LT_E_UNSUPPORTED, "lt_set_grid: more than 2^31-1 voxels");
    BIND(c);
    c->nx = nx; c->ny = ny; c->nz = nz; c->tally = tally_dtype;
    for (int k = 0; k < 3; k++) { c->origin[k] = origin[k]; c->voxel[k] = voxel[k]; }
    HIP_TRY(c, c->d_grid.ensure(c->n_vox() * c->grid_elem()));
    c->have_grid = true;
    c->scene_changed();
    return lt_zero_tally(c);
}

int lt_set_source(lt_ctx* c, int type, const double pos[3], const double dir[3], const double* extra, int start_medium)
{
    CHECK_CTX(c);
    if (!pos || !dir || (type != LT_SRC_PENCIL && type != LT_SRC_COSINE_QUAD)) return c->fail(LT_E_INVALID, "lt_set_source: bad arguments");
    const double l = std::sqrt(dir[0] * dir[0] + dir[1] * dir[1] + dir[2] * dir[2]);
    if (!(l > 0) || !std::isfinite(l)) return c->fail(LT_E_INVALID, "lt_set_source: zero direction");
    if (type == LT_SRC_COSINE_QUAD && !extra) return c->fail(LT_E_INVALID, "lt_set_source: quad source needs extra[6]");
    c->src_type = type; c->start_medium = start_medium;
    for (int k = 0; k < 3; k++) { c->src_pos[k] = pos[k]; c->src_dir[k] = dir[k] / l; }
    for (int k = 0; k < 6; k++) c->src_extra[k] = extra ? extra[k] : 0.0;
    c->have_source = true;
    c->scene_changed();
    return LT_OK;
}

int lt_set_max_steps(lt_ctx* c, uint32_t max_steps)
{
    CHECK_CTX(c);
    if (max_steps == 0) return c->fail(LT_E_INVALID, "lt_set_max_steps: must be > 0");
    c->max_steps = max_steps;
    return LT_OK;
}

int lt_set_tuning(lt_ctx* c, const char* key, int64_t value)
{
    CHECK_CTX(c);
    long* k = key ? c->knob_by_name(key) : nullptr;
    if (!k) return c->fail(LT_E_INVALID, "lt_set_tuning: unknown key '%s'", key ? key : "(null)");
    *k = value < 0 ? -1 : (long)value;
    if (!std::strcmp(key, "log_hot") || !std::strcmp(key, "log_bits2")) { c->dmap_valid = false; }
    return LT_OK;
}

int lt_set_tally_quantity(lt_ctx* c, int quantity)
{
    CHECK_CTX(c);
    if (quantity != LT_QUANTITY_ABSORBED && quantity != LT_QUANTITY_FLUENCE)
        return c->fail(LT_E_INVALID, "lt_set_tally_quantity: LT_QUANTITY_ABSORBED or LT_QUANTITY_FLUENCE");
    if (quantity != c->quantity) { c->quantity = quantity; c->media_dirty = true; }
    return LT_OK;
}

int lt_set_launch_config(lt_ctx* c, int blocks_per_cu, int threads_per_block)
{
    CHECK_CTX(c);
    if (blocks_per_cu < 0 || threads_per_block < 0 || threads_per_block > 256 || (threads_per_block % 64) != 0)
        return c->fail(LT_E_INVALID, "lt_set_launch_config: threads must be a multiple of 64, <= 256");
    c->blocks_per_cu = blocks_per_cu; c->threads_per_block = threads_per_block;
    return LT_OK;
}

int lt_zero_tally(lt_ctx* c)
{
    CHECK_CTX(c);
    BIND(c);
    if (c->have_grid) HIP_TRY(c, hipMemsetAsync(c->d_grid.p, 0, c->n_vox() * c->grid_elem(), c->stream));
    HIP_TRY(c, hipMemsetAsync(c->d_counters.p, 0, sizeof(DevCounters), c->stream));
    return LT_OK;
}

int lt_launch(lt_ctx* c, uint64_t n_photons, uint64_t photon_offset, uint64_t seed, const double* rng_table,
              uint64_t table_steps, uint32_t flags)
{
    CHECK_CTX(c);
    if (c->media.empty()) return c->fail(LT_E_STATE, "lt_launch: lt_set_media first");
    if (!c->have_layers && !c->have_mesh) return c->fail(LT_E_STATE, "lt_launch: lt_set_layers or lt_set_mesh first");
    if (!c->have_grid) return c->fail(LT_E_STATE, "lt_launch: lt_set_grid first");
    if (!c->have_source) return c->fail(LT_E_STATE, "lt_launch: lt_set_source first");
    const int n_media = (int)c->media.size();
    if (c->have_layers) {
        for (int32_t m : c->layer_medium) if (m >= n_media) return c->fail(LT_E_INVALID, "lt_launch: layer medium index %d >= %d media", m, n_media);
    } else {
        for (size_t i = 0; i < c->med_front.size(); i++)
            if (c->med_front[i] >= n_media || c->med_back[i] >= n_media || c->med_front[i] < -1 || c->med_back[i] < -1)
                return c->fail(LT_E_INVALID, "lt_launch: triangle %zu medium index out of range", i);
        if (c->start_medium < 0 || c->start_medium >= n_media) return c->fail(LT_E_INVALID, "lt_launch: start_medium out of range");
    }
    Variant v;
    v.f32 = (flags & LT_FLAG_F32_WALK) ? 1 : 0;
    v.mesh = c->have_mesh ? 1 : 0;
    v.table = rng_table ? 1 : 0;
    v.tally = c->tally;
    v.capture = c->max_vertices > 0 ? 1 : 0;
    v.phase = 0;
    if (v.capture && (v.f32 || v.table)) return c->fail(LT_E_UNSUPPORTED, "lt_launch: vertex capture runs the f64 walk with the XORWOW generator");
    if (c->on(c->knob.diag_no_tally)) v.tally = 3;
    if (v.table && v.f32) return c->fail(LT_E_UNSUPPORTED, "lt_launch: table RNG runs the f64 walk only");
    if (v.table && v.tally == LT_TALLY_F32) return c->fail(LT_E_UNSUPPORTED, "lt_launch: table RNG needs an f64 or u64fx tally");
    if (v.table && table_steps == 0) return c->fail(LT_E_INVALID, "lt_launch: table_steps == 0");
    BIND(c);
    int rc = upload_tables(c);
    if (rc) return rc;
    if (n_photons == 0) { c->timed = false; return LT_OK; }

    if (v.table) {
        const size_t bytes = (size_t)n_photons * (size_t)table_steps * 4 * sizeof(double);
        HIP_TRY(c, c->d_table.ensure(bytes));
        HIP_TRY(c, hipMemcpyAsync(c->d_table.p, rng_table, bytes, hipMemcpyHostToDevice, c->stream));
        HIP_TRY(c, hipStreamSynchronize(c->stream));
    }

    WalkParams P;
    std::memset(&P, 0, sizeof P);
    P.head = (unsigned long long*)c->d_head.p;
    P.n_photons = n_photons; P.photon_offset = photon_offset; P.seed = seed;
    const int pi = v.f32 ? 1 : 0;
    P.media = c->d_media[pi].p; P.zb = c->d_zb[pi].p; P.ifaces = c->d_if[pi].p; P.layer_medium = (const int32_t*)c->d_lm.p;
    P.tris = c->d_tris[pi].p; P.nodes = c->d_nodes[pi].p; P.links = c->have_mesh && c->have_links ? (const int16_t*)c->d_links.p : nullptr;
    P.n_media = n_media;
    P.n_layers = c->have_layers ? (int)c->layer_medium.size() : 0;
    P.n_tris = c->have_mesh ? (int)c->med_front.size() : 0;
    P.n_nodes = c->have_mesh ? (int)c->nodes.size() : 0;
    P.n_above = c->n_above; P.n_below = c->n_below;
    P.grid = c->d_grid.p; P.nx = c->nx; P.ny = c->ny; P.nz = c->nz; P.tally = c->tally;
    for (int k = 0; k < 3; k++) {
        P.origin[k] = c->origin[k]; P.inv_voxel[k] = 1.0 / c->voxel[k];
        P.src_pos[k] = c->src_pos[k]; P.src_dir[k] = c->src_dir[k];
        P.src_e1[k] = c->src_extra[k]; P.src_e2[k] = c->src_extra[3 + k];
    }
    P.fdim[0] = (double)c->nx; P.fdim[1] = (double)c->ny; P.fdim[2] = (double)c->nz;
    for (int k = 0; k < 3; k++) { P.f32.origin[k] = (float)P.origin[k]; P.f32.inv_voxel[k] = (float)P.inv_voxel[k]; P.f32.fdim[k] = (float)P.fdim[k]; }
    P.src_type = c->src_type; P.start_medium = c->start_medium;
    P.table = (const double*)c->d_table.p; P.table_steps = table_steps;
    P.max_steps = c->max_steps;
    P.counters = (DevCounters*)c->d_counters.p;
    if (c->knob.query_min >= 1 && c->knob.query_min <= 64) P.query_min = (unsigned)c->knob.query_min;
    if (c->have_mesh && c->have_clear) {
        P.clear = (const uint4*)c->d_clear.p; P.cnx = c->cn[0]; P.cny = c->cn[1]; P.cnz = c->cn[2];
        for (int k = 0; k < 3; k++) {
            P.corg[k] = c->corg[k]; P.cinv[k] = 1.0 / c->ccell[k]; P.cdim[k] = (double)c->cn[k];
            P.f32.corg[k] = (float)P.corg[k]; P.f32.cinv[k] = (float)P.cinv[k]; P.f32.cdim[k] = (float)P.cdim[k];
        }
    }
    if (c->have_mesh && c->have_march) P.mg = c->mgrid;
    c->captured_photons = 0;
    if (c->max_vertices > 0) {
        const size_t vb = (size_t)n_photons * c->max_vertices * sizeof(lt_vertex);
        if (vb > ((size_t)64 << 30)) return c->fail(LT_E_NOMEM, "lt_launch: vertex capture needs %zu bytes (> 64 GiB)", vb);
        HIP_TRY(c, c->d_vtx.ensure(vb));
        HIP_TRY(c, c->d_vcnt.ensure((size_t)n_photons * sizeof(uint32_t)));
        HIP_TRY(c, hipMemsetAsync(c->d_vcnt.p, 0, (size_t)n_photons * sizeof(uint32_t), c->stream));
        P.vertices = (lt_vertex*)c->d_vtx.p; P.vertex_counts = (uint32_t*)c->d_vcnt.p; P.max_vertices = c->max_vertices;
        c->captured_photons = n_photons; c->captured_max_vertices = c->max_vertices;
    }

    LaunchCfg cfg;
    cfg.threads = c->threads_per_block > 0 ? c->threads_per_block : 256;
    cfg.lds_bytes = walk_lds_bytes(v, P.n_media, P.n_layers, P.n_tris, P.n_nodes);
    if (v.mesh && (cfg.lds_bytes > kMeshLdsBudget || (c->on(c->knob.force_march) && c->have_march && !v.table))) {
        if (v.table) return c->fail(LT_E_UNSUPPORTED, "lt_launch: table RNG with a mesh beyond the LDS budget");
        v.mesh = c->have_march ? 3 : 2;
        cfg.lds_bytes = walk_lds_bytes(v, P.n_media, P.n_layers, P.n_tris, P.n_nodes);
    }
    int resident = walk_max_blocks_per_cu(v, cfg.threads, cfg.lds_bytes);
    if (resident <= 0) return c->fail(LT_E_HIP, "lt_launch: kernel variant not resident (occupancy query returned %d)", resident);
    int per_cu = c->blocks_per_cu > 0 ? c->blocks_per_cu : resident;
    unsigned long long want = (n_photons + (unsigned long long)cfg.threads - 1) / (unsigned long long)cfg.threads;
    unsigned long long cap = (unsigned long long)per_cu * (unsigned long long)c->prop.multiProcessorCount;
    cfg.blocks = (int)(want < cap ? want : cap);
    if (cfg.blocks < 1) cfg.blocks = 1;

    const int mode = c->tally_mode == 2 ? 1 : c->tally_mode;
    { int rc3 = collect_log_stats(c); if (rc3) return rc3; }
    LogGeom G = log_geom(c);
    bool use_log = mode == 1 && !v.table && c->max_vertices == 0 && G.n_tiles <= kMaxLogTiles && !c->on(c->knob.diag_no_tally);
    if (use_log) {
        LogRun R;
        R.c = c; R.P = P; R.v = v; R.cfg = cfg; R.G = G;
        if (c->dmap_valid && (c->dmap_tiles != G.n_tiles || c->dmap_bits2 != G.bits2)) c->dmap_valid = c->tile_cnt_ready = false;
        c->stages_valid = false;
        for (LogLane& ln : c->lanes) ln.ev_used = 0;
        HIP_TRY(c, hipMemsetAsync(c->d_job.p, 0, 2 * sizeof(unsigned long long), c->stream));
        uint64_t done = 0;
        int n_batches = 0;
        if (c->rec_per_photon <= 0.0 && n_photons > kPilotPhotons) {
            LogPlan pilot;
            rc = plan_log(c, kPilotPhotons, 1, &pilot);
            if (rc == LT_OK) rc = run_log_plan(R, pilot, photon_offset, &n_batches);
            if (rc == LT_E_NOMEM) { use_log = false; rc = LT_OK; }
            else if (rc) return rc;
            else {
                c->log_stats_pending = true; c->pending_photons = kPilotPhotons; c->auto_pending = -1;
                if ((rc = collect_log_stats(c))) return rc;
                done = kPilotPhotons;
            }
        }
        if (use_log && G.bits2 && !c->dmap_valid && c->tile_cnt_ready && G.n_tiles <= kMaxHotTiles && G.nb1 < log_max_digits()) {
            uint32_t max_hot = log_max_digits() - G.nb1;
            if (c->knob.log_hot >= 0 && (uint32_t)c->knob.log_hot < max_hot) max_hot = (uint32_t)c->knob.log_hot;
            if (max_hot > 0) {
                HIP_TRY(c, c->d_dmap.ensure(((size_t)G.n_tiles + 2) * sizeof(uint16_t)));
                HIP_TRY(c, c->d_dmeta.ensure(4 * sizeof(uint32_t)));
                HIP_TRY(c, launch_log_plan((const uint32_t*)c->lanes[0].tile_cnt.p, G.n_tiles, G.bits2, max_hot, (uint16_t*)c->d_dmap.p,
                                           (uint32_t*)c->d_dmeta.p, c->stream));
                c->dmap_valid = true; c->dmap_tiles = G.n_tiles; c->dmap_bits2 = G.bits2;
            }
        }
        if (use_log) {
            int lanes = choose_lanes(c, n_photons - done);
            LogPlan plan;
            rc = plan_log(c, n_photons - done, lanes, &plan);
            while (rc == LT_E_NOMEM && lanes > 1) {
                lanes--; rc = plan_log(c, n_photons - done, lanes, &plan);
                if (c->auto_pending >= 0) c->auto_pending = lanes - 1;
            }
            if (rc == LT_E_NOMEM) { use_log = false; rc = LT_OK; }
            else if (rc) return rc;
            else {
                HIP_TRY(c, hipEventRecord(c->ev0, c->stream));
                if ((rc = run_log_plan(R, plan, photon_offset + done, &n_batches))) return rc;
                HIP_TRY(c, hipEventRecord(c->ev1, c->stream));
                c->stages_valid = true; c->last_batches = (uint64_t)n_batches; c->last_lanes = plan.lanes;
                c->last_hot = G.bits2 != 0 && c->dmap_valid;
                c->log_stats_pending = true; c->pending_photons = n_photons;
                if (c->auto_pending >= 0 && done > 0) c->auto_pending = -1;
                c->timed = true;
                if (c->on(c->knob.log_timing)) {
                    double ms[4]; uint64_t rec = 0, bat = 0;
                    if (lt_last_log_stages(c, ms, &rec, &bat) == LT_OK)
                        std::fprintf(stderr, "[lt log] %llu photons, %d lane(s), %llu batches, %llu records (%.1f / photon), %llu to atomics; "
                                     "stage sums ms: walk %.2f scan %.2f partition %.2f reduce %.2f\n", (unsigned long long)n_photons,
                                     plan.lanes, (unsigned long long)bat, (unsigned long long)rec, (double)rec / (double)n_photons,
                                     (unsigned long long)c->last_overflow, ms[0], ms[1], ms[2], ms[3]);
                }
                return LT_OK;
            }
        }
        P.n_photons = n_photons - done; P.photon_offset = photon_offset + done;
        want = (P.n_photons + (unsigned long long)cfg.threads - 1) / (unsigned long long)cfg.threads;
        cfg.blocks = (int)(want < cap ? want : cap);
        if (cfg.blocks < 1) cfg.blocks = 1;
    }

    c->stages_valid = false;
    HIP_TRY(c, hipMemsetAsync(c->d_head.p, 0, sizeof(unsigned long long), c->stream));
    HIP_TRY(c, hipEventRecord(c->ev0, c->stream));
    HIP_TRY(c, launch_walk(P, v, cfg, c->stream));
    HIP_TRY(c, hipEventRecord(c->ev1, c->stream));
    c->timed = true;
    return LT_OK;
}

int lt_reserve_log(lt_ctx* c, uint64_t n_photons)
{
    CHECK_CTX(c);
    if (!c->have_grid) return c->fail(LT_E_STATE, "lt_reserve_log: lt_set_grid first");
    BIND(c);
    LogPlan plan;
    int lanes = c->overlap_mode == 1 ? 1 : (c->overlap_mode >= 2 ? c->overlap_mode : ((c->blocks_per_cu == 0 && n_photons >= kOverlapMinPhotons) ? kAutoLanes : 1));
    int rc = plan_log(c, n_photons, lanes, &plan);
    if (rc == LT_E_NOMEM) return c->fail(LT_E_NOMEM, "lt_reserve_log: not enough device memory for the deposit log");
    return rc;
}

int lt_set_tally_mode(lt_ctx* c, int mode, uint64_t log_bytes)
{
    CHECK_CTX(c);
    if (mode < 0 || mode > 2) return c->fail(LT_E_INVALID, "lt_set_tally_mode: mode must be LT_MODE_ATOMIC, LT_MODE_LOG or LT_MODE_AUTO");
    c->tally_mode = mode;
    c->log_budget = log_bytes ? (size_t)log_bytes : c->default_log_budget;
// ... 459 lines not shown
```

light_transport_amd/csrc/lt_internal.hpp:

```cpp
#pragma once
#include <hip/hip_runtime_api.h>
#include <stdint.h>

#include "../../include/lt.h"

namespace ltk {

template <typename R>
struct MedD {
    R mu_t, inv_mu_t, absorb, g;
    R n, one_m_g2, one_p_g2, inv_2g;
    R dep;
    R one_m_g, two_g;
    R pad_;
};

template <typename R>
struct IfD {
    R n_up, n_dn;
    R nr_down, nr_up;
};

template <typename R>
struct TriD {
    R a[3], ab[3], ac[3], n[3];
    int32_t med_front, med_back;
};

template <typename R>
struct NodeD {
    R lo[3], hi[3];
    int32_t offset, n_prims, axis;
    int32_t skip;
};

struct DevCounters {
    unsigned long long photons, steps;
    double w[8];
};
enum { CW_ABSORBED = 0, CW_LOST, CW_ESC_TOP, CW_ESC_BOT, CW_ESC_MESH, CW_SPECULAR, CW_ROULETTE, CW_CAPPED };

constexpr int kMaxMedia = 32;
constexpr uint32_t kLogChunk = 8192;
constexpr uint32_t kTileShift = 14;
constexpr uint32_t kTileSize = 1u << kTileShift;
constexpr uint32_t kTileBX = 5, kTileBY = 5, kTileBZ = 4;
constexpr uint32_t kLogGroups = 16;
constexpr uint32_t kLogGroups2 = 8;
constexpr int kMaxLayers = 64;

constexpr uint32_t kMarchCountMask = 63u;
struct MarchGrid {
    const uint2* cell;
    const uint32_t* list;
    int nx, ny, nz;
    double org[3], inv[3], h[3];
    double fn[3];
    float org32[3], inv32[3], h32[3], fn32[3];
    double nudge64, nudge32;
};

template <typename R>
struct SurvD {
    R p[3], u[3], w, sleft;
    unsigned long long pid;
    int32_t cur;
    uint32_t step;
    uint32_t rng[6];
    uint32_t held[3];
    uint32_t q_pend;
};
constexpr uint32_t kDumpMaxLanes = 32;
constexpr uint32_t kDumpPoolLanes = 48;

struct WalkParams {
    unsigned long long* head;
    unsigned long long n_photons, photon_offset, seed;
    const void* media;
    const void* zb;
    const void* ifaces;
    const int32_t* layer_medium;
    const void* tris;
    const void* nodes;
    const int16_t* links;
    int n_media, n_layers, n_tris, n_nodes;
    double n_above, n_below;
    void* grid;
    int nx, ny, nz, tally;
    double origin[3], inv_voxel[3];
    double fdim[3];
    double cdim[3];
    struct { float origin[3], inv_voxel[3], fdim[3], corg[3], cinv[3], cdim[3]; } f32;
    int src_type, start_medium;
    double src_pos[3], src_dir[3], src_e1[3], src_e2[3];
    const double* table;
    unsigned long long table_steps;
    unsigned max_steps;
    unsigned query_min;
    DevCounters* counters;
    uint32_t* log_idx;
    void* log_val;
    uint32_t* log_fill;
    uint32_t* log_next;
    uint32_t log_cap_chunks;
    uint32_t* log_hist;
    uint32_t log_n_hist, log_hist_shift, log_ntx, log_nty;
    uint32_t* log_overflow;
    const uint4* clear;
    int cnx, cny, cnz;
    double corg[3], cinv[3];
    MarchGrid mg;
    void* pool;
    uint32_t* pool_n;
    uint32_t pool_cap;
    uint32_t dump_max;
    lt_vertex* vertices;
    uint32_t* vertex_counts;
    unsigned max_vertices;
};

struct LaunchCfg {
    int blocks, threads;
    size_t lds_bytes;
};

struct Variant {
    int f32;
    int mesh;
    int table;
    int tally;
    int capture;
    int phase;
};

hipError_t launch_walk(const WalkParams& P, const Variant& v, const LaunchCfg& cfg, hipStream_t s);
size_t walk_lds_bytes(const Variant& v, int n_media, int n_layers, int n_tris, int n_nodes, unsigned n_hist = 0);
int walk_max_blocks_per_cu(const Variant& v, int threads, size_t lds_bytes);

struct RenderParams {
    const void* tris;
    const void* nodes;
    const lt_surface_material* mats;
    const lt_point_light* lights;
    const int16_t* links;
    int n_tris, n_nodes, n_lights;
    int W, H, S, D;
    double cam[3], f_distance;
    const double* xs;
    const double* ys;
    double* rand_0;
    const double* rand_1;
    const int32_t* light_choice;
    double* image;
    int variant;
    int choices;
    int lds_tables;
};
constexpr int kRenderOldMaxDepth = 24;
hipError_t launch_march_clearance(const void* tris_f64, const void* nodes_f64, int n_nodes, const MarchGrid& G, uint2* cells,
                                  double* coarse, hipStream_t s);
hipError_t launch_build_clearance(const void* tris_f64, int n_tris, int near_lists, void* clear_records, int nx, int ny, int nz,
                                  const double org[3], const double cell[3], hipStream_t s);
hipError_t launch_render_surface(const RenderParams& P, hipStream_t s);

enum { LM_NEXT = 0,
       LM_OVERFLOW = 16,
       LM_RECORDS,
       LM_ITEMS2,
       LM_ITEMS_R,
       LM_SLICE,
       LM_ITEMS_C,
       LM_WORK,
       LM_WORDS = 24 };
static_assert(kLogGroups == 16, "LM_NEXT holds one counter per group");
constexpr uint32_t kTileAlign = 8, kBinAlign = 8;

struct LogReduceParams {
    const uint32_t* log_idx; const void* log_val; const uint32_t* log_fill;
    uint32_t* tmp_idx; void* tmp_val;
    uint32_t* hist1;
    uint32_t* hist;
    uint32_t* bin_base; uint32_t* bin_cnt;
    uint32_t* tile_base; uint32_t* tile_cnt;
    uint32_t* cursor1;
    uint32_t* cursor2;
    uint32_t* items2;
    uint32_t* items_c;
    uint32_t* itab;
    uint32_t* items_r;
    uint32_t* meta;
    unsigned long long* job;
    uint32_t cap_chunks;
    uint32_t n_tiles, bits2;
    void* grid; size_t n_vox; int tally;
    uint32_t nx, ny, nz, ntx, nty;
    const uint16_t* dmap; const uint32_t* dmeta;
    int alone;
    int flush_atomic;
    int lds_part;
};
hipError_t launch_log_scan_bins(const LogReduceParams& L, hipStream_t s);
hipError_t launch_log_count1(const LogReduceParams& L, hipStream_t s);
hipError_t launch_log_plan(const uint32_t* tile_cnt, uint32_t n_tiles, uint32_t bits2, uint32_t max_hot, uint16_t* dmap,
                           uint32_t* dmeta, hipStream_t s);
uint32_t log_max_digits();
constexpr uint32_t kMaxHotTiles = 8192;
hipError_t launch_log_scan_tiles(const LogReduceParams& L, hipStream_t s);
hipError_t launch_log_part1(const LogReduceParams& L, hipStream_t s);
hipError_t launch_log_part2(const LogReduceParams& L, hipStream_t s);
hipError_t launch_log_reduce(const LogReduceParams& L, hipStream_t s);
uint32_t log_part_item();

hipError_t launch_intersect_rays(const void* tris, const void* nodes, int n_tris, int n_nodes,
                                 const double* o, const double* d, const double* tmax, size_t n,
                                 int use_bvh, const MarchGrid* G, const int16_t* links, int32_t* prim, double* t, hipStream_t s);
hipError_t launch_triangle_intersect(const double* o, const double* d, const double* tris, size_t n,
                                     double* t, hipStream_t s);
hipError_t launch_intersect_bounds(const double* o, const double* d, const double* tmax,
                                   const double* boxes, size_t n, int32_t* hit, hipStream_t s);
hipError_t launch_eval(int fn, const double* in, size_t n, double* out, hipStream_t s);
hipError_t launch_rng_raw(unsigned long long seed, unsigned long long photon_id, unsigned count,
                          uint32_t* out, hipStream_t s);
hipError_t launch_grid_to_f64(const void* grid, int tally, size_t n, double* out, hipStream_t s);
hipError_t launch_grid_add(void* dst, const void* src, int tally, size_t n, hipStream_t s);

}
```

light_transport_amd/csrc/lt_kernels.hip:

```cpp
#include <hip/hip_runtime.h>

#define ROCRAND_DETAIL_BM_NOT_IN_STATE
#include <rocrand/rocrand_xorwow.h>
#include <rocrand/rocrand_uniform.h>

#include "lt_internal.hpp"

static_assert(sizeof(rocrand_state_xorwow) == 6 * sizeof(uint32_t), "rocrand_state_xorwow is not {d, x[5]}: SurvD::rng and the tail-split hand-over assume it");

namespace ltk {

#define LT_DEV __device__ __forceinline__
#define LT_PV(name, k) (sizeof(R) == 8 ? (R)P.name[k] : (R)P.f32.name[k])
#define LT_GV(name, k) (sizeof(R) == 8 ? (R)G.name[k] : (R)G.name##32[k])

#ifdef LT_K_IN_SGPR
LT_DEV double fma_k(double a, double b, double k) { double r; asm("v_fma_f64 %0, %1, %2, %3" : "=v"(r) : "v"(a), "v"(b), "s"(k)); return r; }
LT_DEV double fma_mk(double a, double k, double c) { return __builtin_fma(a, k, c); }
LT_DEV double mul_k(double a, double k) { return a * k; }
LT_DEV double fma_kk(double x, double k) { double r; asm("v_fma_f64 %0, %1, %2, %2" : "=v"(r) : "v"(x), "s"(k)); return r; }
#else
template <unsigned long long BITS> LT_DEV double fma_kb(double a, double b)
{
    double r;
// ... 31 lines not shown
{
    double r = __builtin_amdgcn_rcp(b);
    r = __builtin_fma(__builtin_fma(-b, r, 1.0), r, r);
    const double q = a * r;
    return __builtin_fma(__builtin_fma(-b, q, a), r, q);
}
LT_DEV double sqrt_core(double x, double y)
{
    double g = x * y, h = 0.5 * y;
    const double r = __builtin_fma(-h, g, 0.5);
    g = __builtin_fma(g, r, g); h = __builtin_fma(h, r, h);
    const double d = __builtin_fma(-g, g, x);
    return __builtin_fma(d, h, g);
}
LT_DEV double sqrt01(double x)
{
    const double xc = __builtin_fmax(x, 0.0);
    return sqrt_core(xc, __builtin_amdgcn_rsq(__builtin_fmax(xc, 1e-300)));
}
LT_DEV double sqrt_pos(double x) { return sqrt_core(x, __builtin_amdgcn_rsq(x)); }
LT_DEV double rsqrt_pos(double x)
{
    double y = __builtin_amdgcn_rsq(x);
    double e = __builtin_fma(-(x * y), y, 1.0);
    y = __builtin_fma(0.5 * y, e, y);
    e = __builtin_fma(-(x * y), y, 1.0);
    return __builtin_fma(0.5 * y, e, y);
}
__device__ const double kWalkMathTab[(97 + 64) * 2] = {
    0x1.5555555555555p-7, -0x1.269621134db92p-2, 0x1.51d07eae2f815p-7, -0x1.1bf99635a6b95p-2, 0x1.4e5e0a72f0539p-7, -0x1.1178e8227e47cp-2,
    0x1.4afd6a052bf5bp-7, -0x1.07138604d5862p-2, 0x1.47ae147ae147bp-7, -0x1.f991c6cb3b379p-3, 0x1.446f86562d9fbp-7, -0x1.e530effe71012p-3,
    0x1.4141414141414p-7, -0x1.d1037f2655e7bp-3, 0x1.3e22cbce4a902p-7, -0x1.bd087383bd8adp-3, 0x1.3b13b13b13b14p-7, -0x1.a93ed3c8ad9e3p-3,
    0x1.3813813813814p-7, -0x1.95a5adcf7017fp-3, 0x1.3521cfb2b78c1p-7, -0x1.823c16551a3c2p-3, 0x1.323e34a2b10bfp-7, -0x1.6f0128b756abcp-3,
    0x1.2f684bda12f68p-7, -0x1.5bf406b543db2p-3, 0x1.2c9fb4d812ca0p-7, -0x1.4913d8333b561p-3, 0x1.29e4129e4129ep-7, -0x1.365fcb0159016p-3,
    0x1.27350b8812735p-7, -0x1.23d712a49c202p-3, 0x1.2492492492492p-7, -0x1.1178e8227e47cp-3, 0x1.21fb78121fb78p-7, -0x1.fe89139dbd566p-4,
    0x1.1f7047dc11f70p-7, -0x1.da727638446a2p-4, 0x1.1cf06ada2811dp-7, -0x1.b6ac88dad5b1cp-4, 0x1.1a7b9611a7b96p-7, -0x1.9335e5d594989p-4,
    0x1.1811811811812p-7, -0x1.700d30aeac0e1p-4, 0x1.15b1e5f75270dp-7, -0x1.4d3115d207eacp-4, 0x1.135c81135c811p-7, -0x1.2aa04a44717a5p-4,
    0x1.1111111111111p-7, -0x1.08598b59e3a07p-4, 0x1.0ecf56be69c90p-7, -0x1.ccb73cdddb2ccp-5, 0x1.0c9714fbcda3bp-7, -0x1.894aa149fb343p-5,
    0x1.0a6810a6810a7p-7, -0x1.466aed42de3eap-5, 0x1.0842108421084p-7, -0x1.0415d89e74444p-5, 0x1.0624dd2f1a9fcp-7, -0x1.8492528c8cabfp-6,
    0x1.0410410410410p-7, -0x1.0205658935847p-6, 0x1.0204081020408p-7, -0x1.010157588de71p-7, 0x1.0000000000000p-7, 0x0.0p+0,
    0x1.fc07f01fc07f0p-8, 0x1.fe02a6b106789p-8, 0x1.f81f81f81f820p-8, 0x1.fc0a8b0fc03e4p-7, 0x1.f44659e4a4271p-8, 0x1.7b91b07d5b11bp-6,
    0x1.f07c1f07c1f08p-8, 0x1.f829b0e783300p-6, 0x1.ecc07b301ecc0p-8, 0x1.39e87b9febd60p-5, 0x1.e9131abf0b767p-8, 0x1.77458f632dcfcp-5,
    0x1.e573ac901e574p-8, 0x1.b42dd711971bfp-5, 0x1.e1e1e1e1e1e1ep-8, 0x1.f0a30c01162a6p-5, 0x1.de5d6e3f8868ap-8, 0x1.16536eea37ae1p-4,
    0x1.dae6076b981dbp-8, 0x1.341d7961bd1d1p-4, 0x1.d77b654b82c34p-8, 0x1.51b073f06183fp-4, 0x1.d41d41d41d41dp-8, 0x1.6f0d28ae56b4cp-4,
    0x1.d0cb58f6ec074p-8, 0x1.8c345d6319b21p-4, 0x1.cd85689039b0bp-8, 0x1.a926d3a4ad563p-4, 0x1.ca4b3055ee191p-8, 0x1.c5e548f5bc743p-4,
    0x1.c71c71c71c71cp-8, 0x1.e27076e2af2e6p-4, 0x1.c3f8f01c3f8f0p-8, 0x1.fec9131dbeabbp-4, 0x1.c0e070381c0e0p-8, 0x1.0d77e7cd08e59p-3,
    0x1.bdd2b899406f7p-8, 0x1.1b72ad52f67a0p-3, 0x1.bacf914c1bad0p-8, 0x1.29552f81ff523p-3, 0x1.b7d6c3dda338bp-8, 0x1.371fc201e8f74p-3,
    0x1.b4e81b4e81b4fp-8, 0x1.44d2b6ccb7d1ep-3, 0x1.b2036406c80d9p-8, 0x1.526e5e3a1b438p-3, 0x1.af286bca1af28p-8, 0x1.5ff3070a793d4p-3,
    0x1.ac5701ac5701bp-8, 0x1.6d60fe719d21dp-3, 0x1.a98ef606a63bep-8, 0x1.7ab890210d909p-3, 0x1.a6d01a6d01a6dp-8, 0x1.87fa06520c911p-3,
    0x1.a41a41a41a41ap-8, 0x1.9525a9cf456b4p-3, 0x1.a16d3f97a4b02p-8, 0x1.a23bc1fe2b563p-3, 0x1.9ec8e951033d9p-8, 0x1.af3c94e80bff3p-3,
    0x1.9c2d14ee4a102p-8, 0x1.bc286742d8cd6p-3, 0x1.999999999999ap-8, 0x1.c8ff7c79a9a22p-3, 0x1.970e4f80cb872p-8, 0x1.d5c216b4fbb91p-3,
    0x1.948b0fcd6e9e0p-8, 0x1.e27076e2af2e6p-3, 0x1.920fb49d0e229p-8, 0x1.ef0adcbdc5936p-3, 0x1.8f9c18f9c18fap-8, 0x1.fb9186d5e3e2bp-3,
    0x1.8d3018d3018d3p-8, 0x1.0402594b4d041p-2, 0x1.8acb90f6bf3aap-8, 0x1.0a324e27390e3p-2, 0x1.886e5f0abb04ap-8, 0x1.1058bf9ae4ad5p-2,
    0x1.8618618618618p-8, 0x1.1675cababa60ep-2, 0x1.83c977ab2beddp-8, 0x1.1c898c16999fbp-2, 0x1.8181818181818p-8, 0x1.22941fbcf7966p-2,
    0x1.7f405fd017f40p-8, 0x1.2895a13de86a3p-2, 0x1.7d05f417d05f4p-8, 0x1.2e8e2bae11d31p-2, 0x1.7ad2208e0ecc3p-8, 0x1.347dd9a987d55p-2,
    0x1.78a4c8178a4c8p-8, 0x1.3a64c556945eap-2, 0x1.767dce434a9b1p-8, 0x1.404308686a7e4p-2, 0x1.745d1745d1746p-8, 0x1.4618bc21c5ec2p-2,
    0x1.724287f46debcp-8, 0x1.4be5f957778a1p-2, 0x1.702e05c0b8170p-8, 0x1.51aad872df82dp-2, 0x1.6e1f76b4337c7p-8, 0x1.5767717455a6cp-2,
    0x1.6c16c16c16c17p-8, 0x1.5d1bdbf5809cap-2, 0x1.6a13cd1537290p-8, 0x1.62c82f2b9c795p-2, 0x1.6816816816817p-8, 0x1.686c81e9b14afp-2,
    0x1.661ec6a5122f9p-8, 0x1.6e08eaa2ba1e4p-2, 0x1.642c8590b2164p-8, 0x1.739d7f6bbd007p-2, 0x1.623fa77016240p-8, 0x1.792a55fdd47a2p-2,
    0x1.6058160581606p-8, 0x1.7eaf83b82afc3p-2, 0x1.5e75bb8d015e7p-8, 0x1.842d1da1e8b17p-2, 0x1.5c9882b931057p-8, 0x1.89a3386c1425bp-2,
    0x1.5ac056b015ac0p-8, 0x1.8f11e873662c7p-2, 0x1.58ed2308158edp-8, 0x1.947941c2116fbp-2, 0x1.571ed3c506b3ap-8, 0x1.99d958117e08bp-2,
    0x1.5555555555555p-8, 0x1.9f323ecbf984cp-2,
    0x0.0p+0, 0x1.0000000000000p+0, 0x1.917a6bc29b42cp-4, 0x1.fd88da3d12526p-1, 0x1.8f8b83c69a60bp-3, 0x1.f6297cff75cb0p-1,
    0x1.294062ed59f06p-2, 0x1.e9f4156c62ddap-1, 0x1.87de2a6aea963p-2, 0x1.d906bcf328d46p-1, 0x1.e2b5d3806f63bp-2, 0x1.c38b2f180bdb1p-1,
    0x1.1c73b39ae68c8p-1, 0x1.a9b66290ea1a3p-1, 0x1.44cf325091dd6p-1, 0x1.8bc806b151741p-1, 0x1.6a09e667f3bcdp-1, 0x1.6a09e667f3bcdp-1,
    0x1.8bc806b151741p-1, 0x1.44cf325091dd6p-1, 0x1.a9b66290ea1a3p-1, 0x1.1c73b39ae68c8p-1, 0x1.c38b2f180bdb1p-1, 0x1.e2b5d3806f63bp-2,
    0x1.d906bcf328d46p-1, 0x1.87de2a6aea963p-2, 0x1.e9f4156c62ddap-1, 0x1.294062ed59f06p-2, 0x1.f6297cff75cb0p-1, 0x1.8f8b83c69a60bp-3,
    0x1.fd88da3d12526p-1, 0x1.917a6bc29b42cp-4, 0x1.0000000000000p+0, 0x0.0p+0, 0x1.fd88da3d12526p-1, -0x1.917a6bc29b42cp-4,
    0x1.f6297cff75cb0p-1, -0x1.8f8b83c69a60bp-3, 0x1.e9f4156c62ddap-1, -0x1.294062ed59f06p-2, 0x1.d906bcf328d46p-1, -0x1.87de2a6aea963p-2,
    0x1.c38b2f180bdb1p-1, -0x1.e2b5d3806f63bp-2, 0x1.a9b66290ea1a3p-1, -0x1.1c73b39ae68c8p-1, 0x1.8bc806b151741p-1, -0x1.44cf325091dd6p-1,
    0x1.6a09e667f3bcdp-1, -0x1.6a09e667f3bcdp-1, 0x1.44cf325091dd6p-1, -0x1.8bc806b151741p-1, 0x1.1c73b39ae68c8p-1, -0x1.a9b66290ea1a3p-1,
    0x1.e2b5d3806f63bp-2, -0x1.c38b2f180bdb1p-1, 0x1.87de2a6aea963p-2, -0x1.d906bcf328d46p-1, 0x1.294062ed59f06p-2, -0x1.e9f4156c62ddap-1,
    0x1.8f8b83c69a60bp-3, -0x1.f6297cff75cb0p-1, 0x1.917a6bc29b42cp-4, -0x1.fd88da3d12526p-1, 0x0.0p+0, -0x1.0000000000000p+0,
    -0x1.917a6bc29b42cp-4, -0x1.fd88da3d12526p-1, -0x1.8f8b83c69a60bp-3, -0x1.f6297cff75cb0p-1, -0x1.294062ed59f06p-2, -0x1.e9f4156c62ddap-1,
    -0x1.87de2a6aea963p-2, -0x1.d906bcf328d46p-1, -0x1.e2b5d3806f63bp-2, -0x1.c38b2f180bdb1p-1, -0x1.1c73b39ae68c8p-1, -0x1.a9b66290ea1a3p-1,
    -0x1.44cf325091dd6p-1, -0x1.8bc806b151741p-1, -0x1.6a09e667f3bcdp-1, -0x1.6a09e667f3bcdp-1, -0x1.8bc806b151741p-1, -0x1.44cf325091dd6p-1,
    -0x1.a9b66290ea1a3p-1, -0x1.1c73b39ae68c8p-1, -0x1.c38b2f180bdb1p-1, -0x1.e2b5d3806f63bp-2, -0x1.d906bcf328d46p-1, -0x1.87de2a6aea963p-2,
    -0x1.e9f4156c62ddap-1, -0x1.294062ed59f06p-2, -0x1.f6297cff75cb0p-1, -0x1.8f8b83c69a60bp-3, -0x1.fd88da3d12526p-1, -0x1.917a6bc29b42cp-4,
    -0x1.0000000000000p+0, 0x0.0p+0, -0x1.fd88da3d12526p-1, 0x1.917a6bc29b42cp-4, -0x1.f6297cff75cb0p-1, 0x1.8f8b83c69a60bp-3,
    -0x1.e9f4156c62ddap-1, 0x1.294062ed59f06p-2, -0x1.d906bcf328d46p-1, 0x1.87de2a6aea963p-2, -0x1.c38b2f180bdb1p-1, 0x1.e2b5d3806f63bp-2,
    -0x1.a9b66290ea1a3p-1, 0x1.1c73b39ae68c8p-1, -0x1.8bc806b151741p-1, 0x1.44cf325091dd6p-1, -0x1.6a09e667f3bcdp-1, 0x1.6a09e667f3bcdp-1,
    -0x1.44cf325091dd6p-1, 0x1.8bc806b151741p-1, -0x1.1c73b39ae68c8p-1, 0x1.a9b66290ea1a3p-1, -0x1.e2b5d3806f63bp-2, 0x1.c38b2f180bdb1p-1,
    -0x1.87de2a6aea963p-2, 0x1.d906bcf328d46p-1, -0x1.294062ed59f06p-2, 0x1.e9f4156c62ddap-1, -0x1.8f8b83c69a60bp-3, 0x1.f6297cff75cb0p-1,
    -0x1.917a6bc29b42cp-4, 0x1.fd88da3d12526p-1
};
constexpr int kLnTabEntries = 97, kScTabEntries = 64;
constexpr size_t kWalkMathTabBytes = sizeof(double) * 2 * (kLnTabEntries + kScTabEntries);
LT_DEV double neg_log_tab(double x, const double* T)
{
    int e = __builtin_amdgcn_frexp_exp(x);
    double m = __builtin_amdgcn_frexp_mant(x);
    if (m < 0.75) { m += m; e -= 1; }
    const double t = m * 128.0;
    const double qf = __builtin_rint(t);
    const double d = t - qf;
    const double2 Tj = *reinterpret_cast<const double2*>(T + 2 * ((int)qf - 96));
    const double r = d * Tj.x;
    double p = 1.0 / 7.0;
    p = fma_k(p, r, -1.0 / 6.0); p = fma_k(p, r, 1.0 / 5.0); p = fma_k(p, r, -0.25); p = fma_k(p, r, 1.0 / 3.0);
    p = __builtin_fma(p, r, -0.5);
    const double lnm = Tj.y + __builtin_fma(r * r, p, r);
    const double de = (double)e;
    return -fma_mk(de, 6.93147180369123816490e-01, fma_mk(de, 1.90821492927058770002e-10, lnm));
}
LT_DEV void sincos_turn_tab(double xi, const double* T, double* sn, double* cs)
{
    const double t = 64.0 * xi;
    const double qf = __builtin_rint(t);
    const double a = mul_k(t - qf, 9.8174770424681038702e-02);
    const double z = a * a;
    double ps = -1.9841269841269841270e-04;
    ps = fma_k(ps, z, 8.3333333333333333333e-03);
    ps = fma_k(ps, z, -1.6666666666666666667e-01);
    const double sd = __builtin_fma(a * z, ps, a);
    double pc = 2.4801587301587301587e-05;
    pc = fma_k(pc, z, -1.3888888888888888889e-03);
    pc = fma_k(pc, z, 4.1666666666666666667e-02);
    pc = __builtin_fma(pc, z, -0.5);
    const double cd = __builtin_fma(pc, z, 1.0);
    const double2 Ti = *reinterpret_cast<const double2*>(T + 2 * (kLnTabEntries + ((int)qf & (kScTabEntries - 1))));
    *sn = __builtin_fma(Ti.x, cd, Ti.y * sd);
    *cs = __builtin_fma(Ti.y, cd, -(Ti.x * sd));
}

LT_DEV void sincos_small_f64(double x, double* sn, double* cs)
{
    const double kf = __builtin_rint(x * 0.63661977236758134308);
    double a = __builtin_fma(-kf, 1.57079632679489655800e+00, x);
    a = __builtin_fma(-kf, 6.12323399573676603587e-17, a);
    const double z = a * a;
    double ps = -7.6471637318198164759e-13;
    ps = fma_k(ps, z, 1.6059043836821614599e-10);
    ps = fma_k(ps, z, -2.5052108385441718775e-08);
    ps = fma_k(ps, z, 2.7557319223985890653e-06);
    ps = fma_k(ps, z, -1.9841269841269841270e-04);
    ps = fma_k(ps, z, 8.3333333333333333333e-03);
    ps = fma_k(ps, z, -1.6666666666666666667e-01);
    const double s = __builtin_fma(a * z, ps, a);
    double pc = 4.7794773323873852974e-14;
    pc = fma_k(pc, z, -1.1470745597729724714e-11);
    pc = fma_k(pc, z, 2.0876756987868098979e-09);
    pc = fma_k(pc, z, -2.7557319223985890653e-07);
    pc = fma_k(pc, z, 2.4801587301587301587e-05);
    pc = fma_k(pc, z, -1.3888888888888888889e-03);
    pc = fma_k(pc, z, 4.1666666666666666667e-02);
    pc = __builtin_fma(pc, z, -0.5);
    const double c = __builtin_fma(pc, z, 1.0);
    const int q = (int)kf & 3;
    const double s1 = (q & 1) ? c : s, c1 = (q & 1) ? s : c;
    *sn = (q & 2) ? -s1 : s1;
    *cs = ((q + 1) & 2) ? -c1 : c1;
}

LT_DEV double neg_log_raw(unsigned k, const double* T)
{
    const unsigned n = k + 1u;
    const int lz = __clz((int)n);
    const unsigned nm = n << (lz & 31);
    const unsigned hi = nm >= 0xC0000000u ? 1u : 0u;
    const unsigned sh = 24u + hi;
    const unsigned j = ((nm >> (sh - 1u)) + 1u) >> 1;
    const int dint = (int)(nm - (j << sh));
    const double d = __builtin_ldexp((double)dint, -(int)sh);
    const double2 Tj = *reinterpret_cast<const double2*>(T + 2 * ((int)j - 96));
    const double r = d * Tj.x;
    double p = 1.0 / 7.0;
    p = fma_k(p, r, -1.0 / 6.0); p = fma_k(p, r, 1.0 / 5.0); p = fma_k(p, r, -0.25); p = fma_k(p, r, 1.0 / 3.0);
    p = __builtin_fma(p, r, -0.5);
    const double lnm = Tj.y + __builtin_fma(r * r, p, r);
    const double de = (double)((int)hi - 1 - lz);
    const double v = -fma_mk(de, 6.93147180369123816490e-01, fma_mk(de, 1.90821492927058770002e-10, lnm));
    return n == 0u ? 0.0 : v;
}
LT_DEV void sincos_turn_raw(unsigned k, const double* T, double* sn, double* cs)
{
    const unsigned n = k + 1u;
    const unsigned iq = ((n >> 25) + 1u) >> 1;
    const int drem = (int)(n - (iq << 26));
    const double a = mul_k((double)drem, 1.4629180792671596e-09);
    const double z = a * a;
    double ps = -1.9841269841269841270e-04;
    ps = fma_k(ps, z, 8.3333333333333333333e-03);
    ps = fma_k(ps, z, -1.6666666666666666667e-01);
    const double sd = __builtin_fma(a * z, ps, a);
    double pc = 2.4801587301587301587e-05;
    pc = fma_k(pc, z, -1.3888888888888888889e-03);
    pc = fma_k(pc, z, 4.1666666666666666667e-02);
    pc = __builtin_fma(pc, z, -0.5);
    const double cd = __builtin_fma(pc, z, 1.0);
    const double2 Ti = *reinterpret_cast<const double2*>(T + 2 * (kLnTabEntries + (int)(iq & (unsigned)(kScTabEntries - 1))));
    *sn = __builtin_fma(Ti.x, cd, Ti.y * sd);
    *cs = __builtin_fma(Ti.y, cd, -(Ti.x * sd));
}
template <typename R> struct Mx;
template <> struct Mx<double> {
    static LT_DEV double log(double x) { return ::log(x); }
    static LT_DEV double sqrt(double x) { return ::sqrt(x); }
    static LT_DEV double abs(double x) { return ::fabs(x); }
    static LT_DEV double clamp_unit(double c) { return __builtin_fmax(__builtin_fmin(c, 1.0), -1.0); }
    static LT_DEV double sin(double x) { return ::sin(x); }
    static LT_DEV double cos(double x) { return ::cos(x); }
    static LT_DEV double neg_log(double xi, const double* T) { return neg_log_tab(xi, T); }
    static LT_DEV double sqrt_unit(double x) { return sqrt01(x); }
    static LT_DEV double max0(double x) { return __builtin_fmax(x, 0.0); }
    static LT_DEV unsigned sign_word(double x) { return (unsigned)__double2hiint(x); }
    static LT_DEV double max_tiny(double x) { return __builtin_fmax(x, 1e-300); }
    static LT_DEV double sqrt_pos(double x) { return ltk::sqrt_pos(x); }
    static LT_DEV double rsqrt_pos(double x) { return ltk::rsqrt_pos(x); }
    static LT_DEV double quot(double a, double b) { return fast_div(a, b); }
    static LT_DEV double rcp48(double d) { double r = __builtin_amdgcn_rcp(d); return __builtin_fma(__builtin_fma(-d, r, 1.0), r, r); }
    static LT_DEV void sincos_turn(double xi, const double* T, double* s, double* c) { sincos_turn_tab(xi, T, s, c); }
    static LT_DEV double inf() { return __builtin_huge_val(); }
    static LT_DEV double uniform(rocrand_state_xorwow* st)
    {
        const unsigned v1 = rocrand(st), v2 = rocrand(st);
        return fma_kk((double)(((unsigned long long)(v2 >> 11) << 32) | v1), 1.1102230246251565404e-16);
    }
    static LT_DEV double uniform32(rocrand_state_xorwow* st) { return fma_kk((double)rocrand(st), 2.3283064365386962891e-10); }
};
template <> struct Mx<float> {
    static LT_DEV float log(float x) { return ::logf(x); }
    static LT_DEV float sqrt(float x) { return ::sqrtf(x); }
    static LT_DEV float abs(float x) { return ::fabsf(x); }
    static LT_DEV float clamp_unit(float c) { return __builtin_fmaxf(__builtin_fminf(c, 1.0f), -1.0f); }
    static LT_DEV float sin(float x) { return ::sinf(x); }
    static LT_DEV float cos(float x) { return ::cosf(x); }
    static LT_DEV float neg_log(float xi, const double*) { return -::logf(xi); }
    static LT_DEV float sqrt_unit(float x) { return ::sqrtf(__builtin_fmaxf(x, 0.0f)); }
    static LT_DEV float max0(float x) { return __builtin_fmaxf(x, 0.0f); }
    static LT_DEV unsigned sign_word(float x) { return __float_as_uint(x); }
    static LT_DEV float max_tiny(float x) { return __builtin_fmaxf(x, 1e-30f); }
    static LT_DEV float sqrt_pos(float x) { return ::sqrtf(x); }
    static LT_DEV float rsqrt_pos(float x) { return 1.0f / ::sqrtf(x); }
    static LT_DEV float quot(float a, float b) { return a / b; }
    static LT_DEV float rcp48(float d) { return 1.0f / d; }
    static LT_DEV void sincos_turn(float xi, const double*, float* s, float* c) { ::sincospif(2.0f * xi, s, c); }
    static LT_DEV float inf() { return __builtin_huge_valf(); }
    static LT_DEV float uniform(rocrand_state_xorwow* st) { return rocrand_uniform(st); }
    static LT_DEV float uniform32(rocrand_state_xorwow* st) { return rocrand_uniform(st); }
};

template <typename R> LT_DEV R dot3(const R* a, const R* b) { return a[0] * b[0] + a[1] * b[1] + a[2] * b[2]; }
template <typename R> LT_DEV void cross3(const R* a, const R* b, R* o)
{
    o[0] = a[1] * b[2] - a[2] * b[1];
    o[1] = a[2] * b[0] - a[0] * b[2];
    o[2] = a[0] * b[1] - a[1] * b[0];
}
template <typename R> LT_DEV void normalize3(R* v)
{
    R l = Mx<R>::sqrt(v[0] * v[0] + v[1] * v[1] + v[2] * v[2]);
    v[0] /= l; v[1] /= l; v[2] /= l;
}

template <typename R>
LT_DEV R tri_hit(const R* o, const R* d, const TriD<R>* T)
{
    const R eps = (R)1e-7;
    const R nan = (R)__builtin_nanf("");
    R n[3] = {T->n[0], T->n[1], T->n[2]};
    R ddn = dot3(d, n);
    if (Mx<R>::abs(ddn) <= eps) return nan;
    R ab[3] = {T->ab[0], T->ab[1], T->ab[2]};
    R ac[3] = {T->ac[0], T->ac[1], T->ac[2]};
    R pvec[3], qvec[3], tvec[3];
    cross3(d, ac, pvec);
    R det = dot3(ab, pvec);
    if (-eps < det && det < eps) return nan;
    R inv_det = (R)1 / det;
    tvec[0] = o[0] - T->a[0]; tvec[1] = o[1] - T->a[1]; tvec[2] = o[2] - T->a[2];
    R u = dot3(tvec, pvec) * inv_det;
    if (u < 0 || u > 1) return nan;
    cross3(tvec, ab, qvec);
    R v = dot3(d, qvec) * inv_det;
    if (v < 0 || u + v > 1) return nan;
    R t = dot3(ac, qvec) * inv_det;
    return (t > eps) ? t : nan;
}

template <typename R> LT_DEV R box_widen()
{
    const R eps = (R)5.9604644775390625e-08;
    return (R)1 + (R)2 * (((R)3 * eps) / ((R)1 - (R)3 * eps));
}

template <typename R>
LT_DEV bool box_hit(const R* lo, const R* hi, const R* o, const R* inv_d, R tmax)
{
    R t0 = 0, t1 = tmax;
    const R widen = box_widen<R>();
#pragma unroll
    for (int i = 0; i < 3; i++) {
        R tn = (lo[i] - o[i]) * inv_d[i];
        R tf = (hi[i] - o[i]) * inv_d[i];
        if (tn > tf) { R s = tn; tn = tf; tf = s; }
        tf *= widen;
        t0 = tn > t0 ? tn : t0;
        t1 = tf < t1 ? tf : t1;
        if (t0 > t1) return false;
    }
    return true;
}

template <typename R>
LT_DEV void consider(const TriD<R>* tris, int i, const R* o, const R* d, int& bi, R& bt)
{
    R t = tri_hit(o, d, &tris[i]);
    if (t == t && t > (R)1e-6) {
        if (t < bt || (t == bt && bi >= 0 && i < bi)) { bt = t; bi = i; }
    }
}

template <typename R>
LT_DEV void nearest_bvh(const TriD<R>* tris, const NodeD<R>* nodes, int n_nodes, const R* o,
                        const R* d, R tmax, int& prim, R& t_out)
{
    int bi = -1; R bt = tmax;
    const R inv_d[3] = {(R)1 / d[0], (R)1 / d[1], (R)1 / d[2]};
    const R slack = box_widen<R>();
    int cur = 0;
    while (cur < n_nodes) {
        const NodeD<R>* nd = &nodes[cur];
        const R lo[3] = {nd->lo[0], nd->lo[1], nd->lo[2]};
        const R hi[3] = {nd->hi[0], nd->hi[1], nd->hi[2]};
        const int np = nd->n_prims, off = nd->offset, skip = nd->skip;
        if (box_hit(lo, hi, o, inv_d, bt * slack)) {
            if (np > 0) {
                for (int k = 0; k < np; k++) consider(tris, off + k, o, d, bi, bt);
                cur = skip;
            } else {
                cur = cur + 1;
            }
        } else {
            cur = skip;
        }
    }
    prim = bi; t_out = bi >= 0 ? bt : Mx<R>::inf();
}

template <typename R>
LT_DEV void nearest_bvh_ordered(const TriD<R>* tris, const NodeD<R>* nodes, int n_nodes, const int16_t* links, const R* o,
                                const R* d, R tmax, int& prim, R& t_out, bool ANY = false)
{
    int bi = -1; R bt = tmax;
    const R inv_d[3] = {(R)1 / d[0], (R)1 / d[1], (R)1 / d[2]};
    const R slack = box_widen<R>();
// ... 230 lines not shown
    const R inf = Mx<R>::inf(), tol = (R)1e-4;
    const R hx = LT_GV(h, 0), hy = LT_GV(h, 1), hz = LT_GV(h, 2);
    const R nudge = sizeof(R) == 8 ? (R)G.nudge64 : (R)G.nudge32;
    unsigned n = 0, lst = 0;
    R tex = inf, bt = inf; float clr = 0.0f;
    bool m = marching;
    if (m) {
        bt = march_unbits(W->slot_t[lane]);
        if (!(tcur < bt)) m = false;
    }
    if (m) {
        const R px = W->ray[0][lane], py = W->ray[1][lane], pz = W->ray[2][lane];
        const R ux = W->ray[3][lane], uy = W->ray[4][lane], uz = W->ray[5][lane];
        const R fx = (px + tcur * ux - LT_GV(org, 0)) * LT_GV(inv, 0), fy = (py + tcur * uy - LT_GV(org, 1)) * LT_GV(inv, 1),
                fz = (pz + tcur * uz - LT_GV(org, 2)) * LT_GV(inv, 2);
        if (!(fx >= -tol && fx <= LT_GV(fn, 0) + tol && fy >= -tol && fy <= LT_GV(fn, 1) + tol && fz >= -tol && fz <= LT_GV(fn, 2) + tol) ||
            (ux > 0 ? fx >= LT_GV(fn, 0) : (ux < 0 && fx <= 0)) || (uy > 0 ? fy >= LT_GV(fn, 1) : (uy < 0 && fy <= 0)) ||
            (uz > 0 ? fz >= LT_GV(fn, 2) : (uz < 0 && fz <= 0))) m = false;
        else {
            int cx = (int)__builtin_floor(fx), cy = (int)__builtin_floor(fy), cz = (int)__builtin_floor(fz);
            cx = cx < 0 ? 0 : (cx >= G.nx ? G.nx - 1 : cx);
            cy = cy < 0 ? 0 : (cy >= G.ny ? G.ny - 1 : cy);
            cz = cz < 0 ? 0 : (cz >= G.nz ? G.nz - 1 : cz);
            const uint2 rec = G.cell[((size_t)cz * G.ny + cy) * G.nx + cx];
            n = rec.x & kMarchCountMask; lst = rec.y; clr = __uint_as_float(rec.x & ~kMarchCountMask);
            if (n == kMarchCountMask) { heavy = true; m = false; n = 0; }
            const R ix = W->ray[6][lane], iy = W->ray[7][lane], iz = W->ray[8][lane];
            const R ex = ix < inf && ix > -inf ? (LT_GV(org, 0) + (R)(cx + (ux > 0 ? 1 : 0)) * hx - px) * ix : inf;
            const R ey = iy < inf && iy > -inf ? (LT_GV(org, 1) + (R)(cy + (uy > 0 ? 1 : 0)) * hy - py) * iy : inf;
            const R ez = iz < inf && iz > -inf ? (LT_GV(org, 2) + (R)(cz + (uz > 0 ? 1 : 0)) * hz - pz) * iz : inf;
            tex = ex < ey ? (ex < ez ? ex : ez) : (ey < ez ? ey : ez);
        }
    }
    if (!m) marching = false;
    unsigned excl = 0, total_ = 0;
#pragma unroll
    for (unsigned b = 0; b < 6; b++) {
        const unsigned long long mb = __ballot((n >> b) & 1u);
        excl += __builtin_amdgcn_mbcnt_hi((unsigned)(mb >> 32), __builtin_amdgcn_mbcnt_lo((unsigned)mb, 0u)) << b;
        total_ += (unsigned)__popcll(mb) << b;
    }
    const unsigned incl = excl + n, cap = kMarchQ - qn;
    const bool blocked = incl > cap;
    const unsigned long long bm = __ballot(blocked);
    const unsigned pushed = bm ? (unsigned)__builtin_amdgcn_readlane((int)excl, __ffsll((long long)bm) - 1) : total_;
    if (!blocked) for (unsigned k = 0; k < n; k++) W->q_item[qn + excl + k] = (lane << 26) | (lst + k);
    qn += pushed;
    if (m && !blocked) {
        if (n) dirty = true;
        const R jump_min = (R)1.5 * (hx < hy ? (hx < hz ? hx : hz) : (hy < hz ? hy : hz));
        if (!(tex < bt)) marching = false;
        else {
            R tn = (R)clr > jump_min ? tex + (R)clr : tex + nudge;
            const R floor_ = tcur + nudge;
            tcur = tn > floor_ ? tn : floor_;
            if (!(tcur < bt)) marching = false;
        }
    }
    return bm != 0ull;
}

template <typename R>
LT_DEV void march_drain(const TriD<R>* tris, const MarchGrid& G, MarchWave<R>* W, unsigned& qn)
{
    typedef typename MarchBits<R>::type UB;
    const unsigned lane = threadIdx.x & 63u;
    __builtin_amdgcn_fence(__ATOMIC_RELEASE, "wavefront");
    for (unsigned j0 = 0; j0 < qn; j0 += 64u) {
        const unsigned j = j0 + lane;
        UB tb = ~(UB)0;
        if (j < qn) {
            const unsigned item = W->q_item[j], src = item >> 26;
            const int id = (int)G.list[item & 0x3ffffffu];
            const R o[3] = {W->ray[0][src], W->ray[1][src], W->ray[2][src]};
            const R d[3] = {W->ray[3][src], W->ray[4][src], W->ray[5][src]};
            const R t = tri_hit(o, d, &tris[id]);
            if (t == t && t > (R)1e-6) {
                tb = march_bits(t);
                const UB old = __hip_atomic_fetch_min(&W->slot_t[src], tb, __ATOMIC_RELAXED, __HIP_MEMORY_SCOPE_WORKGROUP);
                if (tb < old) W->slot_i[src] = kMarchNone;
            }
        }
        W->q_t[j] = tb;
    }
    __builtin_amdgcn_fence(__ATOMIC_ACQ_REL, "wavefront");
    for (unsigned j0 = 0; j0 < qn; j0 += 64u) {
        const unsigned j = j0 + lane;
        if (j < qn) {
            const UB tb = W->q_t[j];
            const unsigned item = W->q_item[j], src = item >> 26;
            if (tb != ~(UB)0 && tb == W->slot_t[src])
                (void)__hip_atomic_fetch_min(&W->slot_i[src], G.list[item & 0x3ffffffu], __ATOMIC_RELAXED, __HIP_MEMORY_SCOPE_WORKGROUP);
        }
    }
    __builtin_amdgcn_fence(__ATOMIC_ACQ_REL, "wavefront");
    qn = 0;
}

template <typename R>
LT_DEV void march_result(const TriD<R>* tris, const NodeD<R>* nodes, int n_nodes, const int16_t* links, MarchWave<R>* W, bool use_bvh, R px, R py, R pz,
                         R ux, R uy, R uz, R tmax, int& prim, R& t_out)
{
    const unsigned lane = threadIdx.x & 63u;
    prim = -1; t_out = Mx<R>::inf();
    if (use_bvh) {
        const R o[3] = {px, py, pz}, d[3] = {ux, uy, uz};
        nearest_bvh_walk(tris, nodes, n_nodes, links, o, d, tmax, prim, t_out);
    } else {
        const typename MarchBits<R>::type b = W->slot_t[lane];
        if (b < march_bits(tmax)) { prim = (int)W->slot_i[lane]; t_out = march_unbits(b); }
    }
}

template <typename R>
LT_DEV void march_service(const TriD<R>* tris, const NodeD<R>* nodes, int n_nodes, const MarchGrid& G, MarchWave<R>* W,
                          bool want, R px, R py, R pz, R ux, R uy, R uz, R tmax, R t0, int& prim, R& t_out)
{
    bool marching = false, heavy = false, dirty = false, outside = false;
    R tcur = t0 > 0 ? t0 : (R)0;
    if (want) { outside = !march_enter(G, W, px, py, pz, ux, uy, uz, tmax); marching = !outside; }
    unsigned qn = 0;
    while (__any(marching) || qn > 0) {
        bool full = false;
        if (__any(marching)) full = march_round(G, W, marching, heavy, dirty, tcur, qn);
        if (qn > 0 && (full || qn >= 64u || !__any(marching))) march_drain(tris, G, W, qn);
    }
    if (want) march_result(tris, nodes, n_nodes, (const int16_t*)nullptr, W, outside || heavy, px, py, pz, ux, uy, uz, tmax, prim, t_out);
    else { prim = -1; t_out = Mx<R>::inf(); }
}

template <typename R> LT_DEV R hg_pdf(R cos_t, R g)
{
    R denom = (R)1 + g * g + (R)2 * g * cos_t;
    return (R)0.07957747154594767 * ((R)1 - g * g) / (denom * Mx<R>::sqrt(denom));
}

template <typename R> LT_DEV R hg_sample(R xi, R g, R one_m_g2, R one_p_g2, R inv_2g)
{
    R c;
    if (g == 0) c = (R)2 * xi - (R)1;
    else {
        R t = Mx<R>::quot(one_m_g2, (R)1 - g + (R)2 * g * xi);
        c = (one_p_g2 - t * t) * inv_2g;
    }
    return Mx<R>::clamp_unit(c);
}

template <typename R> LT_DEV R hg_sample_walk(R xi, const MedD<R>* M)
{
    if (M->g == 0) return (R)2 * xi - (R)1;
    const R t = Mx<R>::quot(M->one_m_g2, M->two_g * xi + M->one_m_g);
    return (M->one_p_g2 - t * t) * M->inv_2g;
}

template <typename R> LT_DEV void onb(const R* n, R* v2, R* v3)
{
    if (Mx<R>::abs(n[0]) > Mx<R>::abs(n[1])) {
        R l = Mx<R>::sqrt(n[0] * n[0] + n[2] * n[2]);
        v2[0] = -n[2] / l; v2[1] = 0; v2[2] = n[0] / l;
    } else {
        R l = Mx<R>::sqrt(n[1] * n[1] + n[2] * n[2]);
        v2[0] = 0; v2[1] = n[2] / l; v2[2] = -n[1] / l;
    }
    cross3(n, v2, v3);
}

template <typename R, bool LEAN = false> LT_DEV void disk(R u0, R u1, R* d)
{
    R ox = (R)2 * u0 - (R)1, oy = (R)2 * u1 - (R)1;
    if (ox == 0 && oy == 0) { d[0] = 0; d[1] = 0; return; }
    R r, theta;
    if (Mx<R>::abs(ox) > Mx<R>::abs(oy)) { r = ox; theta = (R)0.7853981633974483 * (oy / ox); }
    else { r = oy; theta = (R)1.5707963267948966 - (R)0.7853981633974483 * (ox / oy); }
    if constexpr (LEAN && sizeof(R) == 8) {
        double sn, cs;
        sincos_small_f64(theta, &sn, &cs);
        d[0] = r * cs; d[1] = r * sn;
    } else {
        d[0] = r * Mx<R>::cos(theta); d[1] = r * Mx<R>::sin(theta);
    }
}

template <typename R> LT_DEV void cosine_hemi_frame(const R* n, const R* v2, const R* v3, const R* wi_in, R u0, R u1, R* out)
{
    R wiz = -wi_in[2];
    R d[2]; disk(u0, u1, d);
    R zz = (R)1 - d[0] * d[0] - d[1] * d[1];
    R z = Mx<R>::sqrt(zz > 0 ? zz : (R)0);
    R oz = z;
    if (wiz < 0) oz = -oz;
    R pdf = (wiz * oz > 0) ? Mx<R>::abs(z) * (R)0.3183098861837907 : (R)0;
#pragma unroll
    for (int k = 0; k < 3; k++) out[k] = d[0] * v2[k] + d[1] * v3[k] + oz * n[k];
    out[3] = pdf;
}
template <typename R, bool LEAN = false> LT_DEV void cosine_hemi(const R* n, const R* wi_in, R u0, R u1, R* out)
{
    R wiz = -wi_in[2];
    R d[2]; disk<R, LEAN>(u0, u1, d);
    R zz = (R)1 - d[0] * d[0] - d[1] * d[1];
    R z = Mx<R>::sqrt(zz > 0 ? zz : (R)0);
    R oz = z;
    R v2[3], v3[3]; onb(n, v2, v3);
    if (wiz < 0) oz = -oz;
    R pdf = (wiz * oz > 0) ? Mx<R>::abs(z) * (R)0.3183098861837907 : (R)0;
#pragma unroll
    for (int k = 0; k < 3; k++) out[k] = d[0] * v2[k] + d[1] * v3[k] + oz * n[k];
    out[3] = pdf;
}

template <typename R> LT_DEV void reflect(const R* v, const R* n, R* o)
{
    R k = (R)2 * dot3(v, n);
    o[0] = v[0] - k * n[0]; o[1] = v[1] - k * n[1]; o[2] = v[2] - k * n[2];
    normalize3(o);
}

template <typename R> LT_DEV void reflect_walk(const R* v, const R* n, R* o)
{
    R k = (R)2 * dot3(v, n);
    o[0] = v[0] - k * n[0]; o[1] = v[1] - k * n[1]; o[2] = v[2] - k * n[2];
    const R inv = Mx<R>::rsqrt_pos(o[0] * o[0] + o[1] * o[1] + o[2] * o[2]);
    o[0] *= inv; o[1] *= inv; o[2] *= inv;
}

template <typename R> LT_DEV R boundary(const R* d, const R* nf, R n1, R n2, R* cos_t_out, R* refr)
{
    R cos_i = -dot3(d, nf);
    if (n1 == n2) {
        *cos_t_out = cos_i; refr[0] = d[0]; refr[1] = d[1]; refr[2] = d[2];
        return 0;
    }
    R Nr = Mx<R>::quot(n1, n2);
    R rad = (R)1 - Nr * Nr * ((R)1 - cos_i * cos_i);
    if (rad <= 0) { *cos_t_out = 0; refr[0] = refr[1] = refr[2] = 0; return 1; }
    R cos_t = Mx<R>::sqrt_pos(rad);
    R a = n1 * cos_i, b = n2 * cos_t, c = n1 * cos_t, e = n2 * cos_i;
    const R sab = a + b, sce = c + e;
    const R rr = Mx<R>::rcp48(sab * sce);
    R rs = (a - b) * sce * rr, rp = (c - e) * sab * rr;
    R k = Nr * cos_i - cos_t;
    refr[0] = d[0] * Nr + nf[0] * k;
    refr[1] = d[1] * Nr + nf[1] * k;
    refr[2] = d[2] * Nr + nf[2] * k;
    const R inv = Mx<R>::rsqrt_pos(refr[0] * refr[0] + refr[1] * refr[1] + refr[2] * refr[2]);
    refr[0] *= inv; refr[1] *= inv; refr[2] *= inv;
    *cos_t_out = cos_t;
    return (R)0.5 * (rs * rs + rp * rp);
}

template <typename R> LT_DEV R boundary_planar(R uz, R n1, R n2, R Nr, R* cos_t_out)
{
    const R cos_i = Mx<R>::abs(uz);
    if (n1 == n2) { *cos_t_out = cos_i; return 0; }
    const R rad = (R)1 - Nr * Nr * ((R)1 - cos_i * cos_i);
    if (rad <= 0) { *cos_t_out = 0; return 1; }
    const R cos_t = Mx<R>::sqrt_pos(rad);
    const R a = n1 * cos_i, b = n2 * cos_t, c = n1 * cos_t, e = n2 * cos_i;
    const R sab = a + b, sce = c + e;
    const R r = Mx<R>::rcp48(sab * sce);
    const R rs = (a - b) * sce * r, rp = (c - e) * sab * r;
    *cos_t_out = cos_t;
    return (R)0.5 * (rs * rs + rp * rp);
}

template <typename R, bool TABLE> LT_DEV void spin(R* u, R ct, typename HeldU<R, TABLE>::type xi_phi, const double* T)
{
    const R st2 = Mx<R>::max0((R)1 - ct * ct);
    R sp, cp; HeldU<R, TABLE>::sincos_turn(xi_phi, T, &sp, &cp);
    R ux = u[0], uy = u[1], uz = u[2];
    if (Mx<R>::abs(uz) > (R)0.99999) {
        const R st = Mx<R>::sqrt_unit(st2);
        u[0] = st * cp; u[1] = st * sp; u[2] = uz >= 0 ? ct : -ct;
    } else {
        const R t2 = (R)1 - uz * uz;
        const R a = st2 * Mx<R>::rsqrt_pos(Mx<R>::max_tiny(st2 * t2));
        const R sc = a * cp, ss = a * sp;
        const R k = uz * sc + ct;
        u[0] = ux * k - uy * ss;
        u[1] = uy * k + ux * ss;
        u[2] = uz * ct - sc * t2;
    }
}

LT_DEV unsigned long long mix64(unsigned long long z)
{
    z = (z ^ (z >> 30)) * 0xBF58476D1CE4E5B9ull;
    z = (z ^ (z >> 27)) * 0x94D049BB133111EBull;
    return z ^ (z >> 31);
}
LT_DEV unsigned long long mix_seed(unsigned long long seed, unsigned long long photon_id)
{
    return mix64(mix64(seed + 0x9E3779B97F4A7C15ull) ^ ((photon_id + 1ull) * 0x9E3779B97F4A7C15ull));
}

constexpr int kRngWarmup = 8;
LT_DEV void photon_stream(unsigned long long seed, unsigned long long photon_id, rocrand_state_xorwow* st)
{
    rocrand_init(mix_seed(seed, photon_id), 0ull, 0ull, st);
#pragma unroll
    for (int k = 0; k < kRngWarmup; k++) (void)rocrand(st);
}

template <int TALLY> struct TallyT { typedef double type; };
template <> struct TallyT<LT_TALLY_F32> { typedef float type; };
template <> struct TallyT<LT_TALLY_U64FX> { typedef unsigned long long type; };
#define LT_TALLY_NONE 3

template <int TALLY, typename R> LT_DEV typename TallyT<TALLY>::type tally_quantum(R dw)
{
    if constexpr (TALLY == LT_TALLY_U64FX) return (unsigned long long)((double)dw * LT_FX_SCALE + 0.5);
    else return (typename TallyT<TALLY>::type)dw;
}

template <int TALLY> LT_DEV void tally_add(void* grid, unsigned idx, typename TallyT<TALLY>::type v)
{
    if constexpr (TALLY == LT_TALLY_NONE) { asm volatile("" ::"v"(idx), "v"(v)); }
    else
        __hip_atomic_fetch_add(reinterpret_cast<typename TallyT<TALLY>::type*>(grid) + idx, v, __ATOMIC_RELAXED,
                               __HIP_MEMORY_SCOPE_AGENT);
}

LT_DEV size_t align16(size_t x) { return (x + 15) & ~(size_t)15; }

template <typename R> struct LdsLayout {
    size_t off_cnt, off_frame, off_media, off_zb, off_if, off_lm, off_tris, off_nodes, off_links, off_hist, off_march, off_math, total;
    __host__ __device__ LdsLayout(int n_media, int n_layers, int n_tris, int n_nodes, unsigned n_hist = 0, size_t march_bytes = 0)
    {
        auto al = [](size_t x) { return (x + 15) & ~(size_t)15; };
        size_t o = 0;
        off_cnt = o;   o = al(o + 8 * sizeof(double));
        off_frame = o; o = al(o + 15 * sizeof(R));
        off_media = o; o = al(o + (size_t)n_media * sizeof(MedD<R>));
        off_zb = o;    o = al(o + (size_t)(n_layers + 1) * sizeof(R));
        off_if = o;    o = al(o + (size_t)(n_layers > 0 ? n_layers + 1 : 0) * sizeof(IfD<R>));
        off_lm = o;    o = al(o + (size_t)(n_layers > 0 ? n_layers : 1) * sizeof(int32_t));
        off_tris = o;  o = al(o + (size_t)n_tris * sizeof(TriD<R>));
        off_nodes = o; o = al(o + (size_t)n_nodes * sizeof(NodeD<R>));
        off_links = o; o = al(o + (size_t)n_nodes * 16 * sizeof(int16_t));
        off_hist = o;  o = al(o + (size_t)n_hist * sizeof(uint32_t));
        off_march = o; o = al(o + march_bytes);
        off_math = o;  o = al(o + (sizeof(R) == 8 ? kWalkMathTabBytes : 0));
        total = o;
    }
};

LT_DEV void lds_copy(void* dst, const void* src, size_t bytes)
{
    uint32_t* d = reinterpret_cast<uint32_t*>(dst);
    const uint32_t* s = reinterpret_cast<const uint32_t*>(src);
    for (size_t i = threadIdx.x; i < bytes / 4; i += blockDim.x) d[i] = s[i];
}

LT_DEV unsigned long long readlane64(unsigned long long v, int lane)
{
    unsigned lo = __builtin_amdgcn_readlane((unsigned)v, lane);
    unsigned hi = __builtin_amdgcn_readlane((unsigned)(v >> 32), lane);
    return ((unsigned long long)hi << 32) | lo;
}

template <typename T> LT_DEV T wave_sum(T v)
{
#pragma unroll
    for (int off = 32; off > 0; off >>= 1) v += __shfl_down(v, off, 64);
    return v;
}

template <typename R>
LT_DEV void record_vertex(const WalkParams& P, unsigned long long rel, unsigned& nv, R px, R py, R pz, R ux, R uy,
                          R uz, R w, int kind, int medium, unsigned step, R gx, R gy, R gz, R pdf_pos, R pdf_dir)
{
    if (nv < P.max_vertices) {
        lt_vertex* v = P.vertices + rel * (unsigned long long)P.max_vertices + nv;
        v->point[0] = (double)px; v->point[1] = (double)py; v->point[2] = (double)pz;
        v->direction[0] = (double)ux; v->direction[1] = (double)uy; v->direction[2] = (double)uz;
        v->g_norm[0] = (double)gx; v->g_norm[1] = (double)gy; v->g_norm[2] = (double)gz;
        v->throughput = (double)w; v->pdf_pos = (double)pdf_pos; v->pdf_dir = (double)pdf_dir;
        v->kind = kind; v->medium = medium; v->step = step; v->pad_ = 0;
        nv++;
        P.vertex_counts[rel] = nv;
    }
}

constexpr unsigned kLogExhausted = 0xfffffffeu;
template <int TALLY>
LT_DEV void emit_deposit(const WalkParams& P, bool has, unsigned idx, typename TallyT<TALLY>::type val,
                         unsigned& lg_cur, unsigned& lg_end, unsigned& lg_chunk, uint32_t* s_hist)
{
    typedef typename TallyT<TALLY>::type TV;
    if (P.log_idx == nullptr) {
        if (has) tally_add<TALLY>(P.grid, idx, val);
        return;
    }
    const unsigned long long m = __ballot(has);
    if (m == 0ull) return;
    const unsigned cnt = (unsigned)__popcll(m);
    if (lg_chunk != kLogExhausted && lg_end - lg_cur < cnt) {
        const int lane = threadIdx.x & 63;
        const unsigned grp = blockIdx.x & (kLogGroups - 1);
        if (lg_chunk < kLogExhausted && lane == 0) P.log_fill[lg_chunk] = lg_cur - lg_chunk * kLogChunk;
        unsigned c = 0;
        if (lane == 0) c = __hip_atomic_fetch_add(P.log_next + grp, 1u, __ATOMIC_RELAXED, __HIP_MEMORY_SCOPE_AGENT);
        c = grp + kLogGroups * __builtin_amdgcn_readfirstlane(c);
        if (c < P.log_cap_chunks) { lg_chunk = c; lg_cur = c * kLogChunk; lg_end = lg_cur + kLogChunk; }
        else { lg_chunk = kLogExhausted; lg_cur = lg_end = 0; }
    }
    if (lg_chunk == kLogExhausted) {
        if ((threadIdx.x & 63) == 0) __hip_atomic_fetch_add(P.log_overflow, cnt, __ATOMIC_RELAXED, __HIP_MEMORY_SCOPE_AGENT);
        if (has) {
            unsigned ntx = P.log_ntx, nty = P.log_nty;
            asm volatile("" : "+s"(ntx), "+s"(nty));
            const unsigned tile = idx >> kTileShift, tx = tile % ntx, ty = (tile / ntx) % nty,
                           tz = tile / (ntx * nty);
            const unsigned vx = (tx << kTileBX) | (idx & 31u), vy = (ty << kTileBY) | ((idx >> 5) & 31u),
                           vz = (tz << kTileBZ) | ((idx >> 10) & 15u);
            tally_add<TALLY>(P.grid, (vz * (unsigned)P.ny + vy) * (unsigned)P.nx + vx, val);
        }
        return;
    }
    if (has) {
        const unsigned rank = __builtin_amdgcn_mbcnt_hi((unsigned)(m >> 32), __builtin_amdgcn_mbcnt_lo((unsigned)m, 0u));
        P.log_idx[lg_cur + rank] = idx;
        reinterpret_cast<TV*>(P.log_val)[lg_cur + rank] = val;
        atomicAdd(&s_hist[idx >> P.log_hist_shift], 1u);
    }
    lg_cur += cnt;
}

constexpr unsigned kPacket = 64;
#ifndef LT_REFILL_MIN
#define LT_REFILL_MIN 4
#endif
constexpr unsigned kRefillMin = LT_REFILL_MIN;
#ifndef LT_QUERY_MIN
#define LT_QUERY_MIN 8
#endif
constexpr unsigned kQueryMin = LT_QUERY_MIN;
constexpr unsigned kQueryMinGlobal = 48;
#ifndef LT_QUERY_MAX_AGE
#define LT_QUERY_MAX_AGE 8
#endif
constexpr unsigned kQueryMaxAge = LT_QUERY_MAX_AGE;
#ifndef LT_MARCH_DRAIN_MIN
#define LT_MARCH_DRAIN_MIN 8
#endif
constexpr unsigned kMarchDrainMin = LT_MARCH_DRAIN_MIN;

#ifndef LT_F64_WAVES
#define LT_F64_WAVES 4
#endif
#ifndef LT_F64_GLOBAL_WAVES
#define LT_F64_GLOBAL_WAVES 3
#endif
#ifndef LT_F64_SLAB_WAVES
#define LT_F64_SLAB_WAVES 4
#endif
#ifndef LT_F32_WAVES
#define LT_F32_WAVES 5
#endif
#ifndef LT_INV_MODE_SLAB
#define LT_INV_MODE_SLAB 1
#endif
#ifndef LT_INV_MODE_MESH
#define LT_INV_MODE_MESH 2
#endif
#ifndef LT_INV_MODE_MARCH
#define LT_INV_MODE_MARCH 2
#endif
#define LT_INV_MODE LT_INV_MODE_SLAB
#define LT_WALK_NAME walk_kernel
#define LT_WALK_BATCH 0
#include "lt_walk_kernel.inc"
#undef LT_WALK_NAME
#undef LT_WALK_BATCH
#undef LT_INV_MODE
#define LT_INV_MODE LT_INV_MODE_MESH
#define LT_WALK_NAME walk_kernel_q
#define LT_WALK_BATCH 1
#include "lt_walk_kernel.inc"
#undef LT_WALK_NAME
#undef LT_WALK_BATCH
#undef LT_INV_MODE
#define LT_INV_MODE LT_INV_MODE_MARCH
#define LT_WALK_NAME walk_kernel_m
#define LT_WALK_BATCH 2
#include "lt_walk_kernel.inc"
#undef LT_WALK_NAME
#undef LT_WALK_BATCH
#undef LT_INV_MODE
// ... 824 lines not shown
```

light_transport_amd/csrc/lt_walk_kernel.inc:

```
#ifndef LT_MED
#define LT_MED(i) reinterpret_cast<const MedD<R>*>(reinterpret_cast<const unsigned char*>(s_med) + __umul24((unsigned)(i), (unsigned)sizeof(MedD<R>)))
#endif
#if LT_WALK_BATCH != 2
template <typename R, int GEOM, bool TABLE, int TALLY, bool CAPTURE, int PHASE = 0>
#else
template <typename R, int GEOM, bool TABLE, int TALLY, bool CAPTURE>
#endif
#if LT_WALK_BATCH == 0 && defined(LT_SLAB_VGPR_CAP)
__attribute__((amdgpu_num_vgpr(LT_SLAB_VGPR_CAP)))
#endif
__global__ void __launch_bounds__(256, (sizeof(R) == 8 ? (GEOM == 0 ? LT_F64_SLAB_WAVES : (GEOM == 2 ? LT_F64_GLOBAL_WAVES : LT_F64_WAVES)) : (GEOM == 0 ? LT_F32_WAVES : 4))) LT_WALK_NAME(const WalkParams P)
{
    constexpr bool MESH = GEOM != 0;
#if LT_WALK_BATCH == 2
    constexpr int PHASE = 0;
#endif
#if LT_WALK_PRIO
    __builtin_amdgcn_s_setprio(LT_WALK_PRIO);
#endif
    extern __shared__ __attribute__((aligned(16))) unsigned char lds_raw[];
    const LdsLayout<R> L(P.n_media, P.n_layers, GEOM == 1 ? P.n_tris : 0, GEOM == 1 ? P.n_nodes : 0,
                         P.log_idx ? P.log_n_hist : 0u, LT_WALK_BATCH == 2 ? 4 * sizeof(MarchWave<R>) : 0);
    uint32_t* s_hist = reinterpret_cast<uint32_t*>(lds_raw + L.off_hist);
    if (P.log_idx) for (unsigned t = threadIdx.x; t < P.log_n_hist; t += blockDim.x) s_hist[t] = 0;
    double* s_cnt = reinterpret_cast<double*>(lds_raw + L.off_cnt);
    const MedD<R>* s_med = reinterpret_cast<const MedD<R>*>(lds_raw + L.off_media);
    const R* s_zb = reinterpret_cast<const R*>(lds_raw + L.off_zb);
    const int32_t* s_lm = reinterpret_cast<const int32_t*>(lds_raw + L.off_lm);
    const IfD<R>* s_if = reinterpret_cast<const IfD<R>*>(lds_raw + L.off_if);
    const TriD<R>* s_tris = GEOM == 2 ? reinterpret_cast<const TriD<R>*>(P.tris)
                                      : reinterpret_cast<const TriD<R>*>(lds_raw + L.off_tris);
    const NodeD<R>* s_nodes = GEOM == 2 ? reinterpret_cast<const NodeD<R>*>(P.nodes)
                                        : reinterpret_cast<const NodeD<R>*>(lds_raw + L.off_nodes);

    const int16_t* s_links = !MESH || !P.links ? nullptr
                             : (GEOM == 1 ? reinterpret_cast<const int16_t*>(lds_raw + L.off_links) : P.links);
    if (threadIdx.x < 8) s_cnt[threadIdx.x] = 0.0;
    R* s_frame = reinterpret_cast<R*>(lds_raw + L.off_frame);
    if (threadIdx.x == 64 % blockDim.x && P.src_type == LT_SRC_COSINE_QUAD) {
        const R nrm[3] = {(R)P.src_dir[0], (R)P.src_dir[1], (R)P.src_dir[2]};
        R v2[3], v3[3];
        onb(nrm, v2, v3);
#pragma unroll
        for (int k = 0; k < 3; k++) { s_frame[k] = v2[k]; s_frame[3 + k] = v3[k]; }
    }
#if LT_INV_MODE == 2
    const R* s_inv = s_frame + 6;
    if (threadIdx.x == 128 % blockDim.x) {
#pragma unroll
        for (int k = 0; k < 3; k++) { s_frame[6 + k] = LT_PV(origin, k); s_frame[9 + k] = LT_PV(inv_voxel, k); s_frame[12 + k] = LT_PV(fdim, k); }
    }
#endif
    const double* s_math = reinterpret_cast<const double*>(lds_raw + L.off_math);
    if constexpr (sizeof(R) == 8) lds_copy(lds_raw + L.off_math, kWalkMathTab, kWalkMathTabBytes);
    lds_copy(lds_raw + L.off_media, P.media, (size_t)P.n_media * sizeof(MedD<R>));
    if constexpr (!MESH) {
        lds_copy(lds_raw + L.off_zb, P.zb, (size_t)(P.n_layers + 1) * sizeof(R));
        lds_copy(lds_raw + L.off_lm, P.layer_medium, (size_t)P.n_layers * sizeof(int32_t));
        lds_copy(lds_raw + L.off_if, P.ifaces, (size_t)(P.n_layers + 1) * sizeof(IfD<R>));
    } else if constexpr (GEOM == 1) {
        lds_copy(lds_raw + L.off_tris, P.tris, (size_t)P.n_tris * sizeof(TriD<R>));
        lds_copy(lds_raw + L.off_nodes, P.nodes, (size_t)P.n_nodes * sizeof(NodeD<R>));
        if (P.links) lds_copy(lds_raw + L.off_links, P.links, (size_t)P.n_nodes * 16 * sizeof(int16_t));
    }
    __syncthreads();

    const R eps = (R)1e-6;
    const R inf = Mx<R>::inf();
    const int lane = threadIdx.x & 63;

    bool alive = false;
    R px = 0, py = 0, pz = 0, ux = 0, uy = 0, uz = 1, w = 0, sleft = 0;
    int cur = 0;
    unsigned step = 0, max_steps = P.max_steps, nv = 0;
    unsigned long long pid = 0, grp = 0;
    rocrand_state_xorwow rng;
    double acc_abs = 0.0, acc_lost = 0.0;
    unsigned long long acc_steps = 0;
    typedef typename TallyT<TALLY>::type TV;
    constexpr unsigned kNoVoxel = 0xffffffffu;
    unsigned pend_idx = kNoVoxel;
    TV pend_val = 0;
    unsigned lg_cur = 0, lg_end = 0, lg_chunk = kNoVoxel;
    unsigned long long pk_next = 0, pk_end = 0;
    bool q_done = false;
    bool dumped = false;
#if LT_WALK_BATCH
    bool q_pend = false;
#if LT_WALK_BATCH == 1
    typename HeldU<R, TABLE>::type q_u1 = 0, q_u2 = 0, q_u3 = 0;
#endif
#if LT_WALK_BATCH == 2
    R q_tc = 0;
    bool q_march = false, q_dirty = false, q_bvh = false;
    unsigned mq_n = 0;
    MarchWave<R>* const mw = reinterpret_cast<MarchWave<R>*>(lds_raw + L.off_march) + (threadIdx.x >> 6);
#endif
#if defined(LT_DIAG_MESH)
    unsigned long long dg_iter = 0, dg_alive = 0, dg_prep = 0, dg_wait = 0, dg_trav_it = 0, dg_trav = 0, dg_go = 0, dg_bnd_it = 0, dg_bnd = 0,
                       dg_int_it = 0, dg_int = 0, dg_refill_it = 0, dg_refill = 0, dg_bvh_it = 0, dg_bvh = 0, dg_l4_it = 0, dg_l4 = 0;
    unsigned long long dg_clk_srv = 0, dg_clk_bnd = 0, dg_clk_all = clock64();
    unsigned long long dgm_clk[4] = {0, 0, 0, 0};
#endif
#endif

#if LT_WALK_BATCH == 1
    const unsigned query_min = P.query_min ? P.query_min : (GEOM == 2 ? kQueryMinGlobal : kQueryMin);
    unsigned q_age = 0;
#elif LT_WALK_BATCH == 2
    const unsigned drain_min = P.query_min ? P.query_min : kMarchDrainMin;
#endif
#if LT_INV_MODE == 2
#define gx0 s_inv[0]
#define gy0 s_inv[1]
#define gz0 s_inv[2]
#define ivx s_inv[3]
#define ivy s_inv[4]
#define ivz s_inv[5]
#define fnx s_inv[6]
#define fny s_inv[7]
#define fnz s_inv[8]
#else
    R gx0 = LT_PV(origin, 0), gy0 = LT_PV(origin, 1), gz0 = LT_PV(origin, 2);
    R ivx = LT_PV(inv_voxel, 0), ivy = LT_PV(inv_voxel, 1), ivz = LT_PV(inv_voxel, 2);
    [[maybe_unused]] const R fnx = LT_PV(fdim, 0), fny = LT_PV(fdim, 1), fnz = LT_PV(fdim, 2);
#if LT_INV_MODE == 1
    asm volatile("" : "+v"(gx0), "+v"(gy0), "+v"(gz0), "+v"(ivx), "+v"(ivy), "+v"(ivz));
#endif
#endif

    if constexpr (PHASE == 2) {
        q_done = true;
        const unsigned have = *P.pool_n < P.pool_cap ? *P.pool_n : P.pool_cap;
        const unsigned e = (blockIdx.x * (blockDim.x >> 6) + (threadIdx.x >> 6)) * 64u + (unsigned)lane;
        if (e < have) {
            const SurvD<R>& S = reinterpret_cast<const SurvD<R>*>(P.pool)[e];
            px = S.p[0]; py = S.p[1]; pz = S.p[2]; ux = S.u[0]; uy = S.u[1]; uz = S.u[2]; w = S.w; sleft = S.sleft;
            cur = S.cur; step = S.step;
            __builtin_memcpy(&rng, S.rng, sizeof S.rng);
            alive = true;
#if LT_WALK_BATCH == 1
            if constexpr (!TABLE) {
                q_pend = S.q_pend != 0u;
                q_u1 = __builtin_bit_cast(typename HeldU<R, TABLE>::type, S.held[0]);
                q_u2 = __builtin_bit_cast(typename HeldU<R, TABLE>::type, S.held[1]);
                q_u3 = __builtin_bit_cast(typename HeldU<R, TABLE>::type, S.held[2]);
            }
#endif
        }
    }
    for (;;) {
        unsigned long long need = __ballot(!alive);
        if (need != 0ull && !(q_done && pk_next >= pk_end) &&
            ((unsigned)__popcll(need) >= kRefillMin || need == __ballot(true))) {
            const unsigned cnt = (unsigned)__popcll(need);
#if LT_WALK_BATCH && defined(LT_DIAG_MESH)
            dg_refill_it++; dg_refill += cnt;
#endif
            const unsigned rank = __builtin_amdgcn_mbcnt_hi((unsigned)(need >> 32),
                                      __builtin_amdgcn_mbcnt_lo((unsigned)need, 0u));
            const unsigned long long avail = pk_end - pk_next;
            unsigned long long nlo = 0, nhi = 0;
            if (cnt > avail && !q_done) {
                const int leader = __ffsll((long long)need) - 1;
                unsigned long long base = 0;
                if (lane == leader)
                    base = __hip_atomic_fetch_add(P.head, (unsigned long long)kPacket, __ATOMIC_RELAXED,
                                                  __HIP_MEMORY_SCOPE_AGENT);
                base = readlane64(base, leader);
                nlo = base < P.n_photons ? base : P.n_photons;
                nhi = base + kPacket < P.n_photons ? base + kPacket : P.n_photons;
                if (nhi >= P.n_photons) q_done = true;
            }
            bool got = false;
            unsigned long long id = 0;
            if (!alive) {
                if (rank < avail) { id = pk_next + rank; got = true; }
                else if (rank - avail < nhi - nlo) { id = nlo + (rank - avail); got = true; }
            }
            if (cnt <= avail) pk_next += cnt;
            else {
                unsigned long long used = cnt - avail;
                if (used > nhi - nlo) used = nhi - nlo;
                pk_next = nlo + used; pk_end = nhi;
            }

            if (got) {
                pid = P.photon_offset + id;
                alive = true; w = 1; sleft = 0; step = 0; grp = 0;
                R e_pdf_dir = 1;
                max_steps = P.max_steps;
                if constexpr (!TABLE) photon_stream(P.seed, pid, &rng);
                if (P.src_type == LT_SRC_COSINE_QUAD) {
                    R u4[4];
                    if constexpr (TABLE) {
                        const double* t = P.table + (id * P.table_steps + grp) * 4;
#pragma unroll
                        for (int k = 0; k < 4; k++) u4[k] = (R)(1.0 - t[k]);
                    } else {
#pragma unroll
                        for (int k = 0; k < 4; k++) u4[k] = Mx<R>::uniform32(&rng);
                    }
                    grp++;
                    R nrm[3] = {(R)P.src_dir[0], (R)P.src_dir[1], (R)P.src_dir[2]};
                    R wi[3] = {-nrm[0], -nrm[1], -nrm[2]};
                    R o4[4];
                    {
                        const R v2[3] = {s_frame[0], s_frame[1], s_frame[2]}, v3[3] = {s_frame[3], s_frame[4], s_frame[5]};
                        cosine_hemi_frame(nrm, v2, v3, wi, u4[2], u4[3], o4);
                    }
                    e_pdf_dir = Mx<R>::abs(o4[0] * nrm[0] + o4[1] * nrm[1] + o4[2] * nrm[2]) * (R)0.3183098861837907;
                    ux = o4[0]; uy = o4[1]; uz = o4[2];
// ... 187 lines not shown
                float clr = -1.0f;
                unsigned rec_y = 0u, rec_z = 0xffffffffu;
                if constexpr (GEOM == 2) {
                    if (P.mg.cell) clr = march_clearance<R>(P.mg, px, py, pz);
                } else if constexpr (MESH) {
                    if (P.clear) {
                        const R cx = (px - LT_PV(corg, 0)) * LT_PV(cinv, 0), cy = (py - LT_PV(corg, 1)) * LT_PV(cinv, 1),
                                cz = (pz - LT_PV(corg, 2)) * LT_PV(cinv, 2);
                        if (cx >= 0 && cx < LT_PV(cdim, 0) && cy >= 0 && cy < LT_PV(cdim, 1) && cz >= 0 && cz < LT_PV(cdim, 2)) {
                            const uint4 rec = P.clear[((size_t)(int)cz * P.cny + (int)cy) * P.cnx + (int)cx];
                            clr = __uint_as_float(rec.x); rec_y = rec.y; rec_z = rec.z;
                        }
                    }
                }
                typename HeldU<R, TABLE>::type x0, h1, h2, h3;
                if constexpr (TABLE) {
                    const double* t = P.table + ((pid - P.photon_offset) * P.table_steps + grp) * 4;
                    x0 = (R)(1.0 - t[0]); h1 = (R)(1.0 - t[1]); h2 = (R)(1.0 - t[2]); h3 = (R)(1.0 - t[3]);
                } else if constexpr (sizeof(R) == 8) {
                    x0 = rocrand(&rng); h1 = rocrand(&rng); h2 = rocrand(&rng); h3 = rocrand(&rng);
                } else {
                    x0 = Mx<R>::uniform32(&rng); h1 = Mx<R>::uniform32(&rng); h2 = Mx<R>::uniform32(&rng); h3 = HeldU<R, TABLE>::draw(&rng);
                }
                u1 = HeldU<R, TABLE>::get(h1); x2 = h2; x3 = h3;
                grp++;
                const MedD<R>* Mq = LT_MED(MESH ? cur : s_lm[cur]);
                if (sleft == 0) sleft = HeldU<R, TABLE>::neg_log(x0, s_math);
                s = (Mq->mu_t > 0) ? sleft * Mq->inv_mu_t : inf;

                if constexpr (!MESH) {
                    if (uz != 0) {
                        const R dz = (uz > 0 ? s_zb[cur + 1] : s_zb[cur]) - pz;
                        const R guard = sizeof(R) == 8 ? (R)(1.0 + 1e-12) : (R)(1.0 + 1e-5);
                        const bool near = !(Mx<R>::abs(dz) > s * Mx<R>::abs(uz) * guard);
                        if (__any(near)) {
                            R den = uz;
                            asm volatile("" : "+v"(den));
                            if (near) tb = dz / den;
                        }
                    }
                    go = true;
                } else {
                    if (!(s < (R)clr)) {
                        bool need = true;
                        if constexpr (GEOM == 1) {
                            const float c2 = (float)__builtin_bit_cast(_Float16, (unsigned short)(rec_y & 0xffffu));
                            if (s < (R)c2) {
                                const unsigned i0 = rec_z & 0xffffu, i1 = rec_z >> 16;
                                need = (i0 != 0xffffu && plane_within_reach(&s_tris[i0], px, py, pz, ux, uy, uz, s)) ||
                                       (i1 != 0xffffu && plane_within_reach(&s_tris[i1], px, py, pz, ux, uy, uz, s));
                            }
                        }
                        if (need) { q_pend = true; q_u1 = h1; q_u2 = h2; q_u3 = h3; }
                        else go = true;
                    } else go = true;
                }
            }
        }
        if constexpr (MESH) {
            const unsigned long long wq = __ballot(q_pend);
#if defined(LT_DIAG_MESH)
            if (wq != 0ull && ((unsigned)__popcll(wq) >= query_min || q_age + 1 > kQueryMaxAge || !__any(go))) { dg_trav_it++; dg_trav += __popcll(wq); }
            else dg_wait += __popcll(wq);
#endif
            if (wq != 0ull) q_age++;
            if (wq != 0ull && ((unsigned)__popcll(wq) >= query_min || q_age > kQueryMaxAge || !__any(go))) {
                q_age = 0;
#if defined(LT_DIAG_MESH)
                const long long dg_t0 = clock64();
#endif
                if (q_pend) {
                    {
                        const MedD<R>* Mq = LT_MED(MESH ? cur : s_lm[cur]);
                        s = (Mq->mu_t > 0) ? sleft * Mq->inv_mu_t : inf;
                    }
                    u1 = HeldU<R, TABLE>::get(q_u1); x2 = q_u2; x3 = q_u3;
                    R o[3] = {px, py, pz}, d[3] = {ux, uy, uz}, th;
                    if constexpr (GEOM == 2) {
                        nearest_bvh_walk(s_tris, s_nodes, P.n_nodes, s_links, o, d, s, hit_tri, th);
                    } else {
                    uint4 rec = make_uint4(0u, 0u, 0xffffffffu, 0xffffffffu);
                    if (P.clear) {
                        const R cx = (px - LT_PV(corg, 0)) * LT_PV(cinv, 0), cy = (py - LT_PV(corg, 1)) * LT_PV(cinv, 1),
                                cz = (pz - LT_PV(corg, 2)) * LT_PV(cinv, 2);
                        if (cx >= 0 && cx < LT_PV(cdim, 0) && cy >= 0 && cy < LT_PV(cdim, 1) && cz >= 0 && cz < LT_PV(cdim, 2))
                            rec = P.clear[((size_t)(int)cz * P.cny + (int)cy) * P.cnx + (int)cx];
                    }
#if defined(LT_DIAG_MESH)
                    {
                        const float c2_ = (float)__builtin_bit_cast(_Float16, (unsigned short)(rec.y & 0xffffu));
                        const float c4_ = (float)__builtin_bit_cast(_Float16, (unsigned short)(rec.y >> 16));
                        const unsigned long long fb = __ballot(!(s < (R)c4_)), f4 = __ballot(!(s < (R)c2_) && s < (R)c4_);
                        if (fb) { dg_bvh_it++; dg_bvh += __popcll(fb); }
                        if (f4) { dg_l4_it++; dg_l4 += __popcll(f4); }
                    }
#endif
                    nearest_listed(s_tris, s_nodes, P.n_nodes, s_links, rec, o, d, s, hit_tri, th);
                    }
                    if (hit_tri >= 0) tb = th;
                    q_pend = false; go = true;
                }
#if defined(LT_DIAG_MESH)
                dg_clk_srv += clock64() - dg_t0;
#endif
            }
        }
#if defined(LT_DIAG_MESH)
        {
            const unsigned long long gm = __ballot(go), bm = __ballot(go && hit_tri >= 0);
            dg_go += __popcll(gm);
            if (bm) { dg_bnd_it++; dg_bnd += __popcll(bm); }
            if (gm & ~bm) { dg_int_it++; dg_int += __popcll(gm & ~bm); }
        }
#endif
#if defined(LT_DIAG_MESH)
        const long long dg_t1 = clock64();
#endif
        if (go) {
            {
                const MedD<R>* Mp = LT_MED(MESH ? cur : s_lm[cur]);
                const R mu_t = Mp->mu_t;
#else
        unsigned f_idx = kNoVoxel;
        TV f_val = 0;
        if (alive) {
            if (step >= max_steps) {
                atomicAdd(&s_cnt[CW_CAPPED], (double)w); alive = false;
            } else {
                step++;
                acc_steps++;
                float clr = -1.0f;
                if constexpr (GEOM == 2) {
                    if (P.mg.cell) clr = march_clearance<R>(P.mg, px, py, pz);
                } else if constexpr (MESH) {
                    if (P.clear) {
                        const R cx = (px - LT_PV(corg, 0)) * LT_PV(cinv, 0), cy = (py - LT_PV(corg, 1)) * LT_PV(cinv, 1),
                                cz = (pz - LT_PV(corg, 2)) * LT_PV(cinv, 2);
                        if (cx >= 0 && cx < LT_PV(cdim, 0) && cy >= 0 && cy < LT_PV(cdim, 1) && cz >= 0 && cz < LT_PV(cdim, 2))
                            clr = __uint_as_float(P.clear[((size_t)(int)cz * P.cny + (int)cy) * P.cnx + (int)cx].x);
                    }
                }
                R u1;
                typename HeldU<R, TABLE>::type x0, x2, x3;
                if constexpr (TABLE) {
                    const double* t = P.table + ((pid - P.photon_offset) * P.table_steps + grp) * 4;
                    x0 = (R)(1.0 - t[0]); u1 = (R)(1.0 - t[1]); x2 = (R)(1.0 - t[2]); x3 = (R)(1.0 - t[3]);
                } else {
                    x0 = HeldU<R, TABLE>::draw(&rng);
                    u1 = Mx<R>::uniform32(&rng);
                    x2 = HeldU<R, TABLE>::draw(&rng);
                    x3 = HeldU<R, TABLE>::draw(&rng);
                }
                grp++;
                const MedD<R>* Mp = LT_MED(MESH ? cur : s_lm[cur]);
                const R mu_t = Mp->mu_t;
                if (sleft == 0) sleft = HeldU<R, TABLE>::neg_log(x0, s_math);
                const R s = (mu_t > 0) ? sleft * Mp->inv_mu_t : inf;

                R tb = inf; int hit_tri = -1;
                if constexpr (!MESH) {
                    if (uz != 0) {
                        const R dz = (uz > 0 ? s_zb[cur + 1] : s_zb[cur]) - pz;
                        const R guard = sizeof(R) == 8 ? (R)(1.0 + 1e-12) : (R)(1.0 + 1e-5);
                        const bool near = !(Mx<R>::abs(dz) > s * Mx<R>::abs(uz) * guard);
                        if (__any(near)) {
                            R den = uz;
                            asm volatile("" : "+v"(den));
                            if (near) tb = dz / den;
                        }
                    }
                } else {
                    const bool query = !(s < (R)clr);
                    if (query) {
                        R o[3] = {px, py, pz}, d[3] = {ux, uy, uz}, th;
                        nearest_bvh_walk(s_tris, s_nodes, P.n_nodes, s_links, o, d, s, hit_tri, th);
                        if (hit_tri >= 0) tb = th;
                    }
                }
#endif
                const bool at_boundary = MESH ? (hit_tri >= 0) : (tb <= s);
                if (!at_boundary && !(s < inf)) {
                    atomicAdd(&s_cnt[MESH ? CW_ESC_MESH : CW_CAPPED], (double)w); alive = false;
                } else if (at_boundary) {
                    px += ux * tb; py += uy * tb; pz += uz * tb;
                    sleft -= tb * mu_t;
                    if (!(sleft > 0)) sleft = 0;
                    if constexpr (!MESH) {
                        const bool down = uz > 0;
                        const int k = down ? cur + 1 : cur, next = down ? cur + 1 : cur - 1;
                        pz = s_zb[k];
                        const IfD<R> F = s_if[k];
                        const R Nr = down ? F.nr_down : F.nr_up;
                        R ct;
                        const R Rf = boundary_planar(uz, down ? F.n_up : F.n_dn, down ? F.n_dn : F.n_up, Nr, &ct);
                        const bool refl = HeldU<R, TABLE>::get(x3) <= Rf;
                        const bool gone = !refl && (next < 0 || next >= P.n_layers);
                        if constexpr (CAPTURE) if (P.vertices)
                            record_vertex<R>(P, pid - P.photon_offset, nv, px, py, pz, ux, uy, uz, w,
                                             refl ? LT_VERTEX_REFLECTIVE : LT_VERTEX_TRANSMISSIVE, cur, step, (R)0, (R)0, down ? (R)-1 : (R)1, (R)0,
                                             gone ? (R)0 : (refl ? Rf : (R)1 - Rf));
                        if (refl) uz = -uz;
                        else if (gone) { atomicAdd(&s_cnt[next < 0 ? CW_ESC_TOP : CW_ESC_BOT], (double)w); alive = false; }
                        else { ux *= Nr; uy *= Nr; uz = down ? ct : -ct; cur = next; }
                    } else {
                    R nf[3], n1 = Mp->n, n2; int next;
                    {
                        const TriD<R>* T = &s_tris[hit_tri];
                        R tn[3] = {T->n[0], T->n[1], T->n[2]};
                        R d[3] = {ux, uy, uz};
                        R dn = dot3(d, tn);
                        R sg = dn > 0 ? (R)-1 : (R)1;
                        nf[0] = sg * tn[0]; nf[1] = sg * tn[1]; nf[2] = sg * tn[2];
                        next = dn > 0 ? T->med_front : T->med_back;
                        n2 = next >= 0 ? s_med[next].n : n1;
                    }
                    R d[3] = {ux, uy, uz}, ct, refr[3];
                    R Rf = boundary(d, nf, n1, n2, &ct, refr);
                    if constexpr (CAPTURE) if (P.vertices) {
                        const bool refl = HeldU<R, TABLE>::get(x3) <= Rf;
                        const bool leaves = !refl && next < 0;
                        record_vertex<R>(P, pid - P.photon_offset, nv, px, py, pz, ux, uy, uz, w,
                                         refl ? LT_VERTEX_REFLECTIVE : LT_VERTEX_TRANSMISSIVE, cur, step, nf[0], nf[1], nf[2], (R)0,
                                         leaves ? (R)0 : (refl ? Rf : (R)1 - Rf));
                    }
                    if (HeldU<R, TABLE>::get(x3) <= Rf) {
                        R ro[3]; reflect_walk(d, nf, ro);
                        ux = ro[0]; uy = ro[1]; uz = ro[2];
                        px += eps * nf[0]; py += eps * nf[1]; pz += eps * nf[2];
                    } else if (next < 0) {
                        atomicAdd(&s_cnt[CW_ESC_MESH], (double)w); alive = false;
                    } else {
                        ux = refr[0]; uy = refr[1]; uz = refr[2];
                        px -= eps * nf[0]; py -= eps * nf[1]; pz -= eps * nf[2];
                        cur = next;
                    }
                    }
                } else {
                    px += ux * s; py += uy * s; pz += uz * s;
                    sleft = 0;
                    const R dw = w * Mp->absorb;
                    if constexpr (CAPTURE) if (P.vertices) {
                        const R ct_c = hg_sample_walk(u1, Mp);
                        record_vertex<R>(P, pid - P.photon_offset, nv, px, py, pz, ux, uy, uz, w, LT_VERTEX_VOLUME, cur, step, (R)0, (R)0, (R)0,
                                         (R)0, (w - dw > 0) ? hg_pdf(-ct_c, Mp->g) : (R)0);
                    }
                    const R fx = (px - gx0) * ivx, fy = (py - gy0) * ivy, fz = (pz - gz0) * ivz;
                    const unsigned vx = (unsigned)(int)fx, vy = (unsigned)(int)fy, vz = (unsigned)(int)fz;
                    bool inside;
                    if constexpr (!MESH) inside = (int)(Mx<R>::sign_word(fx) | Mx<R>::sign_word(fy) | Mx<R>::sign_word(fz)) >= 0 &&
                                                  vx < (unsigned)P.nx && vy < (unsigned)P.ny && vz < (unsigned)P.nz;
                    else inside = fx >= 0 && fx < fnx && fy >= 0 && fy < fny && fz >= 0 && fz < fnz;
                    const unsigned idx = P.log_idx
                        ? (((__umul24(__umul24(vz >> kTileBZ, P.log_nty) + (vy >> kTileBY), P.log_ntx) + (vx >> kTileBX)) << kTileShift)
                           | ((vz & 15u) << 10) | ((vy & 31u) << 5) | (vx & 31u))
                        : (vz * (unsigned)P.ny + vy) * (unsigned)P.nx + vx;
                    const TV q = tally_quantum<TALLY, R>(w * Mp->dep);
                    const bool same = inside && idx == pend_idx;
                    const bool flush = inside && !same;
                    f_idx = flush ? pend_idx : kNoVoxel; f_val = pend_val;
                    pend_val = same ? pend_val + q : (flush ? q : pend_val);
                    pend_idx = flush ? idx : pend_idx;
                    acc_abs += inside ? (double)dw : 0.0;
                    acc_lost += inside ? 0.0 : (double)dw;
                    w -= dw;
                    if (!(w > 0)) alive = false;
                    else {
                        R u[3] = {ux, uy, uz};
                        spin<R, TABLE>(u, hg_sample_walk(u1, Mp), x2, s_math);
                        ux = u[0]; uy = u[1]; uz = u[2];
                        if (w < (R)1e-4) {
                            if (HeldU<R, TABLE>::get(x3) <= (R)0.1) { atomicAdd(&s_cnt[CW_ROULETTE], -9.0 * (double)w); w *= (R)10; }
                            else { atomicAdd(&s_cnt[CW_ROULETTE], (double)w); alive = false; }
                        }
                    }
                }
            }
        }
#if LT_WALK_BATCH && defined(LT_DIAG_MESH)
        dg_clk_bnd += clock64() - dg_t1;
#endif
        emit_deposit<TALLY>(P, f_idx != kNoVoxel, f_idx, f_val, lg_cur, lg_end, lg_chunk, s_hist);
    }
    emit_deposit<TALLY>(P, pend_idx != kNoVoxel, pend_idx, pend_val, lg_cur, lg_end, lg_chunk, s_hist);
    if (P.log_idx && lg_chunk < kLogExhausted && (threadIdx.x & 63) == 0) P.log_fill[lg_chunk] = lg_cur - lg_chunk * kLogChunk;

#if LT_WALK_BATCH && defined(LT_DIAG_MESH)
#if LT_WALK_BATCH == 2
    if (blockIdx.x == 7 && threadIdx.x == 0) {
        const double tot = (double)(clock64() - dg_clk_all);
        printf("[march diag] iterations %llu, cycles per iteration %.0f | alive %.1f, preparing %.1f | share of the wave's time: prepare %.3f, march round %.3f "
               "(in %.3f of iterations, %.1f lanes), drain %.3f (in %.3f of iterations, %.1f items), resolve %.3f, complete %.3f | complete %.1f lanes: "
               "boundary in %.3f of iterations (%.1f lanes), interaction in %.3f (%.1f lanes) | refills %.3f of iterations (%.1f lanes)\n",
               dg_iter, tot / dg_iter, (double)dg_alive / dg_iter, (double)dg_prep / dg_iter, dgm_clk[0] / tot, dgm_clk[1] / tot, (double)dg_trav_it / dg_iter,
               dg_trav_it ? (double)dg_trav / dg_trav_it : 0.0, dgm_clk[2] / tot, (double)dg_bvh_it / dg_iter, dg_bvh_it ? (double)dg_bvh / dg_bvh_it : 0.0,
               dgm_clk[3] / tot, dg_clk_bnd / tot, (double)dg_go / dg_iter, (double)dg_bnd_it / dg_iter, dg_bnd_it ? (double)dg_bnd / dg_bnd_it : 0.0,
               (double)dg_int_it / dg_iter, dg_int_it ? (double)dg_int / dg_int_it : 0.0, (double)dg_refill_it / dg_iter, dg_refill_it ? (double)dg_refill / dg_refill_it : 0.0);
    }
#else
    if (blockIdx.x == 7 && threadIdx.x == 0) {
        const double tot = (double)(clock64() - dg_clk_all);
        printf("[mesh diag] cycles per service %.0f; share of the wave's time: services %.3f, complete-stage %.3f; cycles per iteration %.0f\n",
               dg_trav_it ? (double)dg_clk_srv / dg_trav_it : 0.0, dg_clk_srv / tot, dg_clk_bnd / tot, tot / dg_iter);
    }
#endif
    if (blockIdx.x == 7 && threadIdx.x == 0)
        printf("[mesh diag] iterations %llu | alive %.1f/64 | prepare %.1f | waiting for a query %.1f | traversals: %.3f of iterations, %.1f lanes each | "
               "complete %.1f lanes: boundary in %.3f of iterations (%.1f lanes), interaction in %.3f (%.1f lanes) | refills: %.3f of iterations, %.1f lanes | "
               "services with BVH lanes %.3f of iterations (%.1f lanes), with 4-triangle lanes %.3f (%.1f lanes)\n",
               dg_iter, (double)dg_alive / dg_iter, (double)dg_prep / dg_iter, (double)dg_wait / dg_iter, (double)dg_trav_it / dg_iter,
               dg_trav_it ? (double)dg_trav / dg_trav_it : 0.0, (double)dg_go / dg_iter, (double)dg_bnd_it / dg_iter,
               dg_bnd_it ? (double)dg_bnd / dg_bnd_it : 0.0, (double)dg_int_it / dg_iter, dg_int_it ? (double)dg_int / dg_int_it : 0.0,
               (double)dg_refill_it / dg_iter, dg_refill_it ? (double)dg_refill / dg_refill_it : 0.0,
               (double)dg_bvh_it / dg_iter, dg_bvh_it ? (double)dg_bvh / dg_bvh_it : 0.0, (double)dg_l4_it / dg_iter, dg_l4_it ? (double)dg_l4 / dg_l4_it : 0.0);
#endif
    const double wa = wave_sum(acc_abs), wl = wave_sum(acc_lost);
    const unsigned long long ws = wave_sum(acc_steps);
    if (lane == 0) {
        atomicAdd(&s_cnt[CW_ABSORBED], wa);
        atomicAdd(&s_cnt[CW_LOST], wl);
        __hip_atomic_fetch_add(&P.counters->steps, ws, __ATOMIC_RELAXED, __HIP_MEMORY_SCOPE_AGENT);
    }
    __syncthreads();
    if (P.log_idx)
        for (unsigned t = threadIdx.x; t < P.log_n_hist; t += blockDim.x)
            if (s_hist[t]) __hip_atomic_fetch_add(&P.log_hist[t * kLogGroups + (blockIdx.x & (kLogGroups - 1))], s_hist[t],
                                                  __ATOMIC_RELAXED, __HIP_MEMORY_SCOPE_AGENT);
    if (PHASE != 2 && blockIdx.x == 0 && threadIdx.x == 8)
        __hip_atomic_fetch_add(&P.counters->photons, P.n_photons, __ATOMIC_RELAXED, __HIP_MEMORY_SCOPE_AGENT);
    if (threadIdx.x < 8)
        __hip_atomic_fetch_add(&P.counters->w[threadIdx.x], s_cnt[threadIdx.x], __ATOMIC_RELAXED,
                               __HIP_MEMORY_SCOPE_AGENT);
}
#if LT_INV_MODE == 2
#undef gx0
#undef gy0
#undef gz0
#undef ivx
#undef ivy
#undef ivz
#undef fnx
#undef fny
#undef fnz
#endif
```

Measured before the change: 89.58 billion.

## Add per-layer flattened records in LDS and hoist table loads early in slab walk

Builds a per-layer record that merges medium coefficients with the layer's z bounds, uploads it and copies it into LDS, so the slab walk reads one contiguous record instead of chasing layer->medium indirection. The log and sincos table cells and the layer coefficients are loaded at the top of each step behind a compiler barrier, so LDS latency overlaps the step arithmetic. Streams are now created with the highest priority. This adds LDS footprint and register pressure from the early-held values, which could lower occupancy.

```diff
diff --git a/include/lt.h b/include/lt.h
--- a/include/lt.h
+++ b/include/lt.h
@@ -74,6 +74,8 @@
                 int n_nodes);
 int lt_build_bvh(const double* verts, int n_tris, int split_method, int32_t* order_out, lt_bvh_node* nodes_out,
                  int max_nodes, int* n_nodes_out);
+int lt_layer_records(const lt_medium* media, int n_media, int quantity, const double* z_bounds, const int32_t* medium_idx,
+                     int n_layers, int f32, void* media_out, void* zb_out, void* rec_out);
 int lt_set_grid(lt_ctx* ctx, int nx, int ny, int nz, const double origin[3],
                 const double voxel[3], int tally_dtype);
 int lt_set_source(lt_ctx* ctx, int type, const double pos[3], const double dir[3],
diff --git a/light_transport_amd/_lib.py b/light_transport_amd/_lib.py
--- a/light_transport_amd/_lib.py
+++ b/light_transport_amd/_lib.py
@@ -24,6 +24,7 @@
     "lt_set_surface_materials", "lt_set_lights", "lt_render_surface", "lt_set_vertex_capture", "lt_read_vertices",
     "lt_set_tally_mode", "lt_last_log_stages", "lt_reserve_log", "lt_render_surface_old", "lt_set_overlap", "lt_last_log_hot_tiles",
     "lt_last_log_info", "lt_set_tally_quantity", "lt_set_tuning", "lt_mesh_accel_info", "lt_build_bvh",
+    "lt_layer_records",
 ]
 
 VERTEX_DTYPE = np.dtype([("point", "<f8", 3), ("direction", "<f8", 3), ("g_norm", "<f8", 3), ("throughput", "<f8"),
@@ -50,6 +51,19 @@
     if rc:
         raise LtError("lt_build_bvh failed (%d): needs >= 1 triangle with finite vertices and split_method 0 or 1" % rc)
     return order, nodes[:nn.value]
+
+
+def layer_records(media, z_bounds, medium_idx, quantity=0, f32=False):
+    arr = (Medium * len(media))(*[Medium(*map(float, m)) for m in media])
+    zb = _f64(z_bounds)
+    mi = np.ascontiguousarray(medium_idx, dtype=np.int32)
+    dt = np.float32 if f32 else np.float64
+    m_out, z_out, r_out = np.zeros((len(media), 12), dt), np.zeros(zb.size, dt), np.zeros((mi.size, 12), dt)
+    rc = lib().lt_layer_records(arr, C.c_int(len(media)), C.c_int(int(quantity)), _dp(zb), _ip(mi), C.c_int(mi.size), C.c_int(int(f32)),
+                                m_out.ctypes.data_as(C.c_void_p), z_out.ctypes.data_as(C.c_void_p), r_out.ctypes.data_as(C.c_void_p))
+    if rc:
+        raise LtError("lt_layer_records failed (%d): needs len(z_bounds) == len(medium_idx) + 1 and medium indices inside the media" % rc)
+    return m_out, z_out, r_out
 
 
 class Medium(C.Structure):
diff --git a/light_transport_amd/csrc/lt_api.cpp b/light_transport_amd/csrc/lt_api.cpp
--- a/light_transport_amd/csrc/lt_api.cpp
+++ b/light_transport_amd/csrc/lt_api.cpp
@@ -103,7 +103,7 @@
     uint64_t captured_photons = 0;
     int blocks_per_cu = 0, threads_per_block = 0;
 
-    DevBuf d_media[2], d_zb[2], d_if[2], d_lm, d_tris[2], d_nodes[2];
+    DevBuf d_media[2], d_zb[2], d_if[2], d_lay[2], d_lm, d_tris[2], d_nodes[2];
     DevBuf d_grid, d_counters, d_head, d_table, d_scratch_in, d_scratch_out, d_scratch_aux;
     DevBuf d_mats, d_lights, d_r0, d_r1, d_lc, d_img, d_xy, d_vtx, d_vcnt, d_clear, d_job, d_gridx[kMaxLanes - 1];
     int cn[3] = {0, 0, 0};
@@ -182,6 +182,13 @@
     return true;
 }
 
+static hipError_t create_stream(hipStream_t* s)
+{
+    int least = 0, greatest = 0;
+    hipError_t e = hipDeviceGetStreamPriorityRange(&least, &greatest);
+    return e != hipSuccess ? e : hipStreamCreateWithPriority(s, hipStreamNonBlocking, greatest);
+}
+
 #define CHECK_CTX(c) do { if (!(c)) return LT_E_INVALID; } while (0)
 #define HIP_TRY(c, call) do { hipError_t e_ = (call); if (e_ != hipSuccess) return (c)->hip(e_, #call); } while (0)
 #define BIND(c) HIP_TRY(c, hipSetDevice((c)->device))
@@ -272,6 +279,16 @@
         out[(size_t)k].n_up = up; out[(size_t)k].n_dn = dn;
         out[(size_t)k].nr_down = up / dn; out[(size_t)k].nr_up = dn / up;
     }
+}
+
+template <typename R>
+void fill_layers(const lt_ctx* c, const std::vector<MedD<R>>& media, std::vector<LayD<R>>& out)
+{
+    const std::vector<R> zb(c->z_bounds.begin(), c->z_bounds.end());
+    out.assign(c->layer_medium.size(), LayD<R>());
+    for (int32_t m : c->layer_medium)
+        if (m < 0 || (size_t)m >= media.size()) return;
+    fill_layer_records(media.data(), zb.data(), c->layer_medium.data(), (int)out.size(), out.data());
 }
 
 template <typename T>
@@ -403,6 +420,7 @@
     std::vector<MedD<double>> m64; std::vector<MedD<float>> m32;
     std::vector<double> z64; std::vector<float> z32;
     std::vector<IfD<double>> i64; std::vector<IfD<float>> i32;
+    std::vector<LayD<double>> y64; std::vector<LayD<float>> y32;
     std::vector<TriD<double>> t64; std::vector<TriD<float>> t32;
     std::vector<NodeD<double>> n64; std::vector<NodeD<float>> n32;
     std::vector<int16_t> links16;
@@ -413,6 +431,9 @@
         fill_ifaces(c, i64); fill_ifaces(c, i32);
         if ((rc = upload(c, c->d_if[0], i64))) return rc;
         if ((rc = upload(c, c->d_if[1], i32))) return rc;
+        fill_layers(c, m64, y64); fill_layers(c, m32, y32);
+        if ((rc = upload(c, c->d_lay[0], y64))) return rc;
+        if ((rc = upload(c, c->d_lay[1], y32))) return rc;
     }
     if (!c->tables_dirty) {
         HIP_TRY(c, hipStreamSynchronize(c->stream));
@@ -690,7 +711,7 @@
         const size_t gb = c->n_vox() * c->grid_elem();
         HIP_TRY(c, hipEventRecord(c->ev_fork, c->stream));
         for (int l = 1; l < plan.lanes; l++) {
-            if (!c->lanes[l].stream) HIP_TRY(c, hipStreamCreateWithFlags(&c->lanes[l].stream, hipStreamNonBlocking));
+            if (!c->lanes[l].stream) HIP_TRY(c, create_stream(&c->lanes[l].stream));
             HIP_TRY(c, hipStreamWaitEvent(c->lanes[l].stream, c->ev_fork, 0));
             HIP_TRY(c, hipMemsetAsync(c->d_gridx[l - 1].p, 0, gb, c->lanes[l].stream));
         }
@@ -748,7 +769,7 @@
             P.dump_max = c->knob.tail_split > 1 ? (uint32_t)std::min<long>(c->knob.tail_split, (long)kDumpPoolLanes) : kDumpMaxLanes;
             HIP_TRY(c, ln.pool.ensure(cap * (R.v.f32 ? sizeof(SurvD<float>) : sizeof(SurvD<double>))));
             HIP_TRY(c, ln.pool_n.ensure(4));
-            if (!ln.tail_stream) HIP_TRY(c, hipStreamCreateWithFlags(&ln.tail_stream, hipStreamNonBlocking));
+            if (!ln.tail_stream) HIP_TRY(c, create_stream(&ln.tail_stream));
             if (!ln.ev_bulk) HIP_TRY(c, hipEventCreateWithFlags(&ln.ev_bulk, hipEventDisableTiming));
             if (!ln.ev_tail) HIP_TRY(c, hipEventCreateWithFlags(&ln.ev_tail, hipEventDisableTiming));
             HIP_TRY(c, hipMemsetAsync(ln.pool_n.p, 0, 4, s));
@@ -828,6 +849,20 @@
     return visited == n.size();
 }
 
+template <typename R>
+void layer_records_out(const std::vector<lt_medium>& media, int quantity, const double* z_bounds, const int32_t* medium_idx, int n_layers,
+                       void* media_out, void* zb_out, void* rec_out)
+{
+    static_assert(sizeof(MedD<R>) == 12 * sizeof(R) && sizeof(LayD<R>) == 12 * sizeof(R), "lt_layer_records: 12 values per record");
+    std::vector<MedD<R>> m; fill_media(media, quantity, m);
+    const std::vector<R> zb(z_bounds, z_bounds + n_layers + 1);
+    std::vector<LayD<R>> y((size_t)n_layers);
+    fill_layer_records(m.data(), zb.data(), medium_idx, n_layers, y.data());
+    std::memcpy(media_out, m.data(), m.size() * sizeof(MedD<R>));
+    std::memcpy(zb_out, zb.data(), zb.size() * sizeof(R));
+    std::memcpy(rec_out, y.data(), y.size() * sizeof(LayD<R>));
+}
+
 }
 
 extern "C" {
@@ -873,7 +908,7 @@
         size_t quarter = c->prop.totalGlobalMem / 4;
         c->log_budget = c->default_log_budget = quarter < ((size_t)64 << 30) ? quarter : ((size_t)64 << 30);
     }
-    if (e == hipSuccess) e = hipStreamCreateWithFlags(&c->stream, hipStreamNonBlocking);
+    if (e == hipSuccess) e = create_stream(&c->stream);
     c->lanes[0].stream = c->stream;
     if (e == hipSuccess) e = hipEventCreate(&c->ev0);
     if (e == hipSuccess) e = hipEventCreate(&c->ev1);
@@ -897,7 +932,7 @@
     if (!c) return LT_OK;
     (void)hipSetDevice(c->device);
     if (c->stream) (void)hipStreamSynchronize(c->stream);
-    for (int i = 0; i < 2; i++) { c->d_media[i].release(); c->d_zb[i].release(); c->d_if[i].release(); c->d_tris[i].release(); c->d_nodes[i].release(); }
+    for (int i = 0; i < 2; i++) { c->d_media[i].release(); c->d_zb[i].release(); c->d_if[i].release(); c->d_lay[i].release(); c->d_tris[i].release(); c->d_nodes[i].release(); }
     c->d_lm.release(); c->d_grid.release(); c->d_counters.release(); c->d_head.release(); c->d_table.release();
     c->d_scratch_in.release(); c->d_scratch_out.release(); c->d_scratch_aux.release();
     c->d_mats.release(); c->d_lights.release(); c->d_r0.release(); c->d_r1.release(); c->d_lc.release();
@@ -936,6 +971,17 @@
     c->media.assign(media, media + n);
     c->scene_changed();
     c->tables_dirty = true;
+    return LT_OK;
+}
+
+int lt_layer_records(const lt_medium* media, int n_media, int quantity, const double* z_bounds, const int32_t* medium_idx,
+                     int n_layers, int f32, void* media_out, void* zb_out, void* rec_out)
+{
+    if (!media || n_media <= 0 || !z_bounds || !medium_idx || n_layers <= 0 || !media_out || !zb_out || !rec_out) return LT_E_INVALID;
+    for (int l = 0; l < n_layers; l++) if (medium_idx[l] < 0 || medium_idx[l] >= n_media) return LT_E_INVALID;
+    const std::vector<lt_medium> m(media, media + n_media);
+    if (f32) layer_records_out<float>(m, quantity, z_bounds, medium_idx, n_layers, media_out, zb_out, rec_out);
+    else layer_records_out<double>(m, quantity, z_bounds, medium_idx, n_layers, media_out, zb_out, rec_out);
     return LT_OK;
 }
 
@@ -1108,7 +1154,7 @@
     P.head = (unsigned long long*)c->d_head.p;
     P.n_photons = n_photons; P.photon_offset = photon_offset; P.seed = seed;
     const int pi = v.f32 ? 1 : 0;
-    P.media = c->d_media[pi].p; P.zb = c->d_zb[pi].p; P.ifaces = c->d_if[pi].p; P.layer_medium = (const int32_t*)c->d_lm.p;
+    P.media = c->d_media[pi].p; P.zb = c->d_zb[pi].p; P.ifaces = c->d_if[pi].p; P.layers = c->d_lay[pi].p; P.layer_medium = (const int32_t*)c->d_lm.p;
     P.tris = c->d_tris[pi].p; P.nodes = c->d_nodes[pi].p; P.links = c->have_mesh && c->have_links ? (const int16_t*)c->d_links.p : nullptr;
     P.n_media = n_media;
     P.n_layers = c->have_layers ? (int)c->layer_medium.size() : 0;
diff --git a/light_transport_amd/csrc/lt_internal.hpp b/light_transport_amd/csrc/lt_internal.hpp
--- a/light_transport_amd/csrc/lt_internal.hpp
+++ b/light_transport_amd/csrc/lt_internal.hpp
@@ -20,6 +20,28 @@
     R n_up, n_dn;
     R nr_down, nr_up;
 };
+
+template <typename R>
+struct alignas(16) LayD {
+    R mu_t, inv_mu_t;
+    R z_lo, z_hi;
+    R absorb, dep;
+    R two_g, one_m_g;
+    R one_m_g2, one_p_g2;
+    R inv_2g, n;
+};
+static_assert(sizeof(LayD<double>) == 96 && sizeof(LayD<float>) == 48, "LayD: a whole number of 16-byte quads");
+template <typename R>
+inline void fill_layer_records(const MedD<R>* media, const R* zb, const int32_t* layer_medium, int n_layers, LayD<R>* out)
+{
+    for (int l = 0; l < n_layers; l++) {
+        const MedD<R>& m = media[layer_medium[l]];
+        LayD<R>& r = out[l];
+        r.mu_t = m.mu_t; r.inv_mu_t = m.inv_mu_t; r.z_lo = zb[l]; r.z_hi = zb[l + 1];
+        r.absorb = m.absorb; r.dep = m.dep; r.two_g = m.two_g; r.one_m_g = m.one_m_g;
+        r.one_m_g2 = m.one_m_g2; r.one_p_g2 = m.one_p_g2; r.inv_2g = m.inv_2g; r.n = m.n;
+    }
+}
 
 template <typename R>
 struct TriD {
@@ -79,6 +101,7 @@
     const void* media;
     const void* zb;
     const void* ifaces;
+    const void* layers;
     const int32_t* layer_medium;
     const void* tris;
     const void* nodes;
diff --git a/light_transport_amd/csrc/lt_kernels.hip b/light_transport_amd/csrc/lt_kernels.hip
--- a/light_transport_amd/csrc/lt_kernels.hip
+++ b/light_transport_amd/csrc/lt_kernels.hip
@@ -207,7 +207,15 @@
     *cs = ((q + 1) & 2) ? -c1 : c1;
 }
 
-LT_DEV double neg_log_raw(unsigned k, const double* T)
+LT_DEV double2 neg_log_cell(unsigned k, const double* T)
+{
+    const unsigned n = k + 1u;
+    const unsigned nm = n << (__clz((int)n) & 31);
+    const unsigned sh = 24u + (nm >= 0xC0000000u ? 1u : 0u);
+    const unsigned j = ((nm >> (sh - 1u)) + 1u) >> 1;
+    return *reinterpret_cast<const double2*>(T + 2 * ((int)j - 96));
+}
+LT_DEV double neg_log_raw(unsigned k, const double2 Tj)
 {
     const unsigned n = k + 1u;
     const int lz = __clz((int)n);
@@ -217,7 +225,6 @@
     const unsigned j = ((nm >> (sh - 1u)) + 1u) >> 1;
     const int dint = (int)(nm - (j << sh));
     const double d = __builtin_ldexp((double)dint, -(int)sh);
-    const double2 Tj = *reinterpret_cast<const double2*>(T + 2 * ((int)j - 96));
     const double r = d * Tj.x;
     double p = 1.0 / 7.0;
     p = fma_k(p, r, -1.0 / 6.0); p = fma_k(p, r, 1.0 / 5.0); p = fma_k(p, r, -0.25); p = fma_k(p, r, 1.0 / 3.0);
@@ -227,7 +234,13 @@
     const double v = -fma_mk(de, 6.93147180369123816490e-01, fma_mk(de, 1.90821492927058770002e-10, lnm));
     return n == 0u ? 0.0 : v;
 }
-LT_DEV void sincos_turn_raw(unsigned k, const double* T, double* sn, double* cs)
+LT_DEV double neg_log_raw(unsigned k, const double* T) { return neg_log_raw(k, neg_log_cell(k, T)); }
+LT_DEV double2 sincos_turn_cell(unsigned k, const double* T)
+{
+    const unsigned iq = (((k + 1u) >> 25) + 1u) >> 1;
+    return *reinterpret_cast<const double2*>(T + 2 * (kLnTabEntries + (int)(iq & (unsigned)(kScTabEntries - 1))));
+}
+LT_DEV void sincos_turn_raw(unsigned k, const double2 Ti, double* sn, double* cs)
 {
     const unsigned n = k + 1u;
     const unsigned iq = ((n >> 25) + 1u) >> 1;
@@ -243,10 +256,10 @@
     pc = fma_k(pc, z, 4.1666666666666666667e-02);
     pc = __builtin_fma(pc, z, -0.5);
     const double cd = __builtin_fma(pc, z, 1.0);
-    const double2 Ti = *reinterpret_cast<const double2*>(T + 2 * (kLnTabEntries + (int)(iq & (unsigned)(kScTabEntries - 1))));
     *sn = __builtin_fma(Ti.x, cd, Ti.y * sd);
     *cs = __builtin_fma(Ti.y, cd, -(Ti.x * sd));
 }
+LT_DEV void sincos_turn_raw(unsigned k, const double* T, double* sn, double* cs) { sincos_turn_raw(k, sincos_turn_cell(k, T), sn, cs); }
 template <typename R> struct Mx;
 template <> struct Mx<double> {
     static LT_DEV double log(double x) { return ::log(x); }
@@ -783,6 +796,12 @@
     const R t = Mx<R>::quot(M->one_m_g2, M->two_g * xi + M->one_m_g);
     return (M->one_p_g2 - t * t) * M->inv_2g;
 }
+template <typename R> LT_DEV R hg_sample_walk(R xi, R two_g, R one_m_g, R one_m_g2, R one_p_g2, R inv_2g)
+{
+    if (two_g == 0) return (R)2 * xi - (R)1;
+    const R t = Mx<R>::quot(one_m_g2, two_g * xi + one_m_g);
+    return (one_p_g2 - t * t) * inv_2g;
+}
 
 template <typename R> LT_DEV void onb(const R* n, R* v2, R* v3)
 {
@@ -895,10 +914,9 @@
     return (R)0.5 * (rs * rs + rp * rp);
 }
 
-template <typename R, bool TABLE> LT_DEV void spin(R* u, R ct, typename HeldU<R, TABLE>::type xi_phi, const double* T)
+template <typename R> LT_DEV void spin_turn(R* u, R ct, R sp, R cp)
 {
     const R st2 = Mx<R>::max0((R)1 - ct * ct);
-    R sp, cp; HeldU<R, TABLE>::sincos_turn(xi_phi, T, &sp, &cp);
     R ux = u[0], uy = u[1], uz = u[2];
     if (Mx<R>::abs(uz) > (R)0.99999) {
         const R st = Mx<R>::sqrt_unit(st2);
@@ -913,6 +931,11 @@
         u[2] = uz * ct - sc * t2;
     }
 }
+template <typename R, bool TABLE> LT_DEV void spin(R* u, R ct, typename HeldU<R, TABLE>::type xi_phi, const double* T)
+{
+    R sp, cp; HeldU<R, TABLE>::sincos_turn(xi_phi, T, &sp, &cp);
+    spin_turn(u, ct, sp, cp);
+}
 
 LT_DEV unsigned long long mix64(unsigned long long z)
 {
@@ -955,7 +978,7 @@
 LT_DEV size_t align16(size_t x) { return (x + 15) & ~(size_t)15; }
 
 template <typename R> struct LdsLayout {
-    size_t off_cnt, off_frame, off_media, off_zb, off_if, off_lm, off_tris, off_nodes, off_links, off_hist, off_march, off_math, total;
+    size_t off_cnt, off_frame, off_media, off_zb, off_if, off_lm, off_lay, off_tris, off_nodes, off_links, off_hist, off_march, off_math, total;
     __host__ __device__ LdsLayout(int n_media, int n_layers, int n_tris, int n_nodes, unsigned n_hist = 0, size_t march_bytes = 0)
     {
         auto al = [](size_t x) { return (x + 15) & ~(size_t)15; };
@@ -966,6 +989,7 @@
         off_zb = o;    o = al(o + (size_t)(n_layers + 1) * sizeof(R));
         off_if = o;    o = al(o + (size_t)(n_layers > 0 ? n_layers + 1 : 0) * sizeof(IfD<R>));
         off_lm = o;    o = al(o + (size_t)(n_layers > 0 ? n_layers : 1) * sizeof(int32_t));
+        off_lay = o;   o = al(o + (size_t)(n_layers > 0 ? n_layers : 0) * sizeof(LayD<R>));
         off_tris = o;  o = al(o + (size_t)n_tris * sizeof(TriD<R>));
         off_nodes = o; o = al(o + (size_t)n_nodes * sizeof(NodeD<R>));
         off_links = o; o = al(o + (size_t)n_nodes * 16 * sizeof(int16_t));
diff --git a/light_transport_amd/csrc/lt_walk_kernel.inc b/light_transport_amd/csrc/lt_walk_kernel.inc
--- a/light_transport_amd/csrc/lt_walk_kernel.inc
+++ b/light_transport_amd/csrc/lt_walk_kernel.inc
@@ -1,5 +1,24 @@
 #ifndef LT_MED
 #define LT_MED(i) reinterpret_cast<const MedD<R>*>(reinterpret_cast<const unsigned char*>(s_med) + __umul24((unsigned)(i), (unsigned)sizeof(MedD<R>)))
+#define LT_LAY(i) reinterpret_cast<const LayD<R>*>(reinterpret_cast<const unsigned char*>(s_lay) + __umul24((unsigned)(i), (unsigned)sizeof(LayD<R>)))
+#endif
+#ifndef LT_LAY_LATE
+#define LT_LAY_LATE 0
+#endif
+#ifndef LT_TAB_LATE
+#define LT_TAB_LATE 0
+#endif
+#if LT_WALK_BATCH == 0
+#define LT_STEP_Y(held, field) (kLayEarly ? held : Yp->field)
+#define LT_STEP_ABSORB LT_STEP_Y(absorb, absorb)
+#define LT_STEP_DEP LT_STEP_Y(dep, dep)
+#define LT_STEP_HG(xi) hg_sample_walk(xi, LT_STEP_Y(hg_2g, two_g), LT_STEP_Y(hg_1mg, one_m_g), LT_STEP_Y(hg_1mg2, one_m_g2), LT_STEP_Y(hg_1pg2, one_p_g2), LT_STEP_Y(hg_i2g, inv_2g))
+#define LT_STEP_G (LT_MED(s_lm[cur])->g)
+#else
+#define LT_STEP_ABSORB Mp->absorb
+#define LT_STEP_DEP Mp->dep
+#define LT_STEP_HG(xi) hg_sample_walk(xi, Mp)
+#define LT_STEP_G (Mp->g)
 #endif
 #if LT_WALK_BATCH != 2
 template <typename R, int GEOM, bool TABLE, int TALLY, bool CAPTURE, int PHASE = 0>
@@ -27,6 +46,7 @@
     const MedD<R>* s_med = reinterpret_cast<const MedD<R>*>(lds_raw + L.off_media);
     const R* s_zb = reinterpret_cast<const R*>(lds_raw + L.off_zb);
     const int32_t* s_lm = reinterpret_cast<const int32_t*>(lds_raw + L.off_lm);
+    [[maybe_unused]] const LayD<R>* s_lay = reinterpret_cast<const LayD<R>*>(lds_raw + L.off_lay);
     const IfD<R>* s_if = reinterpret_cast<const IfD<R>*>(lds_raw + L.off_if);
     const TriD<R>* s_tris = GEOM == 2 ? reinterpret_cast<const TriD<R>*>(P.tris)
                                       : reinterpret_cast<const TriD<R>*>(lds_raw + L.off_tris);
@@ -58,6 +78,7 @@
         lds_copy(lds_raw + L.off_zb, P.zb, (size_t)(P.n_layers + 1) * sizeof(R));
         lds_copy(lds_raw + L.off_lm, P.layer_medium, (size_t)P.n_layers * sizeof(int32_t));
         lds_copy(lds_raw + L.off_if, P.ifaces, (size_t)(P.n_layers + 1) * sizeof(IfD<R>));
+        lds_copy(lds_raw + L.off_lay, P.layers, (size_t)P.n_layers * sizeof(LayD<R>));
     } else if constexpr (GEOM == 1) {
         lds_copy(lds_raw + L.off_tris, P.tris, (size_t)P.n_tris * sizeof(TriD<R>));
         lds_copy(lds_raw + L.off_nodes, P.nodes, (size_t)P.n_nodes * sizeof(NodeD<R>));
@@ -551,15 +572,29 @@
                     x3 = HeldU<R, TABLE>::draw(&rng);
                 }
                 grp++;
-                const MedD<R>* Mp = LT_MED(MESH ? cur : s_lm[cur]);
-                const R mu_t = Mp->mu_t;
-                if (sleft == 0) sleft = HeldU<R, TABLE>::neg_log(x0, s_math);
-                const R s = (mu_t > 0) ? sleft * Mp->inv_mu_t : inf;
+                static_assert(!MESH, "walk_kernel is the slab walk");
+                constexpr bool kLayEarly = PHASE != 2 && !CAPTURE && !LT_LAY_LATE;
+                constexpr bool kTabEarly = !TABLE && sizeof(R) == 8 && PHASE != 2 && !CAPTURE && !LT_TAB_LATE;
+                [[maybe_unused]] const MedD<R>* Mp = s_med;
+                const LayD<R>* Yp = LT_LAY(cur);
+                const R mu_t = Yp->mu_t, inv_mu_t = Yp->inv_mu_t, z_lo = Yp->z_lo, z_hi = Yp->z_hi;
+                [[maybe_unused]] R absorb = 0, dep = 0, hg_2g = 0, hg_1mg = 0, hg_1mg2 = 0, hg_1pg2 = 0, hg_i2g = 0;
+                [[maybe_unused]] double2 Tln, Tsc;
+                if constexpr (kTabEarly) { Tln = neg_log_cell(x0, s_math); Tsc = sincos_turn_cell(x2, s_math); }
+                if constexpr (kLayEarly) {
+                    absorb = Yp->absorb; dep = Yp->dep;
+                    hg_2g = Yp->two_g; hg_1mg = Yp->one_m_g; hg_1mg2 = Yp->one_m_g2; hg_1pg2 = Yp->one_p_g2; hg_i2g = Yp->inv_2g;
+                }
+                if constexpr (kLayEarly || kTabEarly) asm volatile("" ::: "memory");
+                if (sleft == 0) {
+                    if constexpr (kTabEarly) sleft = neg_log_raw(x0, Tln); else sleft = HeldU<R, TABLE>::neg_log(x0, s_math);
+                }
+                const R s = (mu_t > 0) ? sleft * inv_mu_t : inf;
 
                 R tb = inf; int hit_tri = -1;
                 if constexpr (!MESH) {
                     if (uz != 0) {
-                        const R dz = (uz > 0 ? s_zb[cur + 1] : s_zb[cur]) - pz;
+                        const R dz = (uz > 0 ? z_hi : z_lo) - pz;
                         const R guard = sizeof(R) == 8 ? (R)(1.0 + 1e-12) : (R)(1.0 + 1e-5);
                         const bool near = !(Mx<R>::abs(dz) > s * Mx<R>::abs(uz) * guard);
                         if (__any(near)) {
@@ -637,11 +672,11 @@
                 } else {
                     px += ux * s; py += uy * s; pz += uz * s;
                     sleft = 0;
-                    const R dw = w * Mp->absorb;
+                    const R dw = w * LT_STEP_ABSORB;
                     if constexpr (CAPTURE) if (P.vertices) {
-                        const R ct_c = hg_sample_walk(u1, Mp);
+                        const R ct_c = LT_STEP_HG(u1);
                         record_vertex<R>(P, pid - P.photon_offset, nv, px, py, pz, ux, uy, uz, w, LT_VERTEX_VOLUME, cur, step, (R)0, (R)0, (R)0,
-                                         (R)0, (w - dw > 0) ? hg_pdf(-ct_c, Mp->g) : (R)0);
+                                         (R)0, (w - dw > 0) ? hg_pdf(-ct_c, LT_STEP_G) : (R)0);
                     }
                     const R fx = (px - gx0) * ivx, fy = (py - gy0) * ivy, fz = (pz - gz0) * ivz;
                     const unsigned vx = (unsigned)(int)fx, vy = (unsigned)(int)fy, vz = (unsigned)(int)fz;
@@ -653,7 +688,7 @@
                         ? (((__umul24(__umul24(vz >> kTileBZ, P.log_nty) + (vy >> kTileBY), P.log_ntx) + (vx >> kTileBX)) << kTileShift)
                            | ((vz & 15u) << 10) | ((vy & 31u) << 5) | (vx & 31u))
                         : (vz * (unsigned)P.ny + vy) * (unsigned)P.nx + vx;
-                    const TV q = tally_quantum<TALLY, R>(w * Mp->dep);
+                    const TV q = tally_quantum<TALLY, R>(w * LT_STEP_DEP);
                     const bool same = inside && idx == pend_idx;
                     const bool flush = inside && !same;
                     f_idx = flush ? pend_idx : kNoVoxel; f_val = pend_val;
@@ -665,7 +700,13 @@
                     if (!(w > 0)) alive = false;
                     else {
                         R u[3] = {ux, uy, uz};
-                        spin<R, TABLE>(u, hg_sample_walk(u1, Mp), x2, s_math);
+#if LT_WALK_BATCH == 0
+                        if constexpr (kTabEarly) {
+                            R sp, cp; sincos_turn_raw(x2, Tsc, &sp, &cp);
+                            spin_turn(u, LT_STEP_HG(u1), sp, cp);
+                        } else
+#endif
+                        spin<R, TABLE>(u, LT_STEP_HG(u1), x2, s_math);
                         ux = u[0]; uy = u[1]; uz = u[2];
                         if (w < (R)1e-4) {
                             if (HeldU<R, TABLE>::get(x3) <= (R)0.1) { atomicAdd(&s_cnt[CW_ROULETTE], -9.0 * (double)w); w *= (R)10; }
@@ -730,6 +771,13 @@
         __hip_atomic_fetch_add(&P.counters->w[threadIdx.x], s_cnt[threadIdx.x], __ATOMIC_RELAXED,
                                __HIP_MEMORY_SCOPE_AGENT);
 }
+#undef LT_STEP_ABSORB
+#if LT_WALK_BATCH == 0
+#undef LT_STEP_Y
+#endif
+#undef LT_STEP_DEP
+#undef LT_STEP_HG
+#undef LT_STEP_G
 #if LT_INV_MODE == 2
 #undef gx0
 #undef gy0
```

Result: faster. 93.59 billion, median of 6 (+4.5%).
